# spawner1145/vae-tagger

Measured on AMD Instinct MI355X. Metric: images/sec encode+tag, 1024^2 bf16, higher is better.
Workload: dtype bf16

## Files before the change

include/vae_tagger_hip.h:

```cpp
#ifndef VAE_TAGGER_HIP_H
#define VAE_TAGGER_HIP_H

#include <stddef.h>
#include <stdint.h>

#ifdef __cplusplus
extern "C" {
#endif

typedef struct vt_context vt_context;

enum { VT_OK = 0, VT_ERR_INVALID = 1, VT_ERR_HIP = 2, VT_ERR_STATE = 3, VT_ERR_MISSING_WEIGHT = 4,
       VT_ERR_WORKSPACE = 5 };
enum { VT_F32 = 0, VT_BF16 = 1, VT_F16 = 2, VT_U8 = 3  };

const char* vt_version(void);
int vt_create(int device, vt_context** out);
void vt_destroy(vt_context* ctx);
const char* vt_last_error(const vt_context* ctx);

int vt_encoder_configure(vt_context* ctx, int in_channels, int latent_channels, const int* block_out_channels,
                         int n_blocks, int layers_per_block, int norm_num_groups, float scaling_factor,
                         int has_scaling_factor, float shift_factor, int has_shift_factor);
int vt_set_weight(vt_context* ctx, const char* name, const void* host_data, int dtype, const int64_t* shape,
// ... 60 lines not shown
                    uint64_t* row_stats_out , size_t row_stats_bytes, void* workspace, size_t workspace_bytes, void* stream);

typedef struct { const void* state; size_t state_bytes; long long capacity; long long n_seen; } vt_eval_source;
int vt_eval_export(vt_context* ctx, const void* state, size_t state_bytes, int N, int T, long long capacity, long long n_seen,
                   void* out_state, size_t out_bytes, long long out_capacity, void* stream);
int vt_eval_merge(vt_context* ctx, void* dst, size_t dst_bytes, int N, int T, long long dst_capacity, long long dst_n_seen,
                  const vt_eval_source* sources , int W, void* stream);

typedef struct { const void* state; size_t state_bytes; double alpha; double gamma; const double* class_weights ; } vt_loss_source;
size_t vt_loss_state_bytes(int N);
int vt_loss_reset(vt_context* ctx, void* state, size_t state_bytes, int N, double alpha, double gamma,
                  const double* class_weights , void* stream);
int vt_loss_update(vt_context* ctx, void* state, size_t state_bytes, int N, const float* logits ,
                   const void* labels , int labels_dtype , int B, void* stream);
int vt_loss_read(vt_context* ctx, const void* state, size_t state_bytes, int N, void* out, size_t out_bytes, void* stream);
int vt_loss_merge(vt_context* ctx, void* dst, size_t dst_bytes, int N, double alpha, double gamma,
                  const double* class_weights , const vt_loss_source* sources , int W, void* stream);

enum { VT_SAMPLE_GT = 0, VT_SAMPLE_GE = 1 };
size_t vt_sample_state_bytes(int T, long long capacity);
int vt_sample_reset(vt_context* ctx, void* state, size_t state_bytes, int T, const double* thresholds , int rule,
                    long long capacity, void* stream);
int vt_sample_update(vt_context* ctx, void* state, size_t state_bytes, int T, long long capacity, const float* probs ,
                     const void* labels , int labels_dtype , const uint32_t* true_extra ,
                     int B, int N, long long n_seen , void* stream);
int vt_sample_from_keys(vt_context* ctx, const void* eval_state, size_t eval_state_bytes, int N, int T_eval, long long capacity,
                        long long n_seen, const double* class_thresholds , int rule,
                        const uint32_t* true_extra , void* sample_state , size_t sample_state_bytes,
                        long long sample_capacity, void* stream);
size_t vt_sample_finish_bytes(int T);
int vt_sample_finish(vt_context* ctx, const void* state, size_t state_bytes, int T, long long capacity, long long n_seen, void* out,
                     size_t out_bytes, void* stream);
int vt_sample_read_rows(vt_context* ctx, const void* state, size_t state_bytes, int T, long long capacity, long long n_seen,
                        uint32_t* true_out , size_t true_bytes, uint32_t* rows_out , size_t rows_bytes,
                        void* stream);

double vt_encoder_flops(const vt_context* ctx, int H, int W);

enum { VT_HEAD_PARAM = 0, VT_HEAD_GRAD = 1, VT_HEAD_ADAM_M = 2, VT_HEAD_ADAM_V = 3, VT_HEAD_LOSS_RING = 4, VT_HEAD_NORM = 5 };
enum { VT_HEAD_LOSS_BCE = 0, VT_HEAD_LOSS_FOCAL = 1, VT_HEAD_LOSS_CLASS_BALANCED = 2 };
int vt_decoder_feature_dim(const vt_context* ctx);
int vt_decode_features(vt_context* ctx, const float* latent_nchw, int B, int h, int w, float* features_out , void* workspace,
                       size_t workspace_bytes, void* stream);
size_t vt_head_state_bytes(const vt_context* ctx);
size_t vt_head_workspace_bytes(const vt_context* ctx, int B);
int vt_head_init(vt_context* ctx, void* state, size_t state_bytes, void* stream);
int vt_head_forward(vt_context* ctx, const void* state, size_t state_bytes, const float* features, int B, float* logits_out, void* workspace,
                    size_t workspace_bytes, void* stream);
int vt_head_forward_backward(vt_context* ctx, void* state, size_t state_bytes, const float* features, const void* labels, int labels_dtype,
                             int B, int loss_kind, double focal_alpha, double focal_gamma, const float* class_weights, double loss_scale,
                             int train, const float* dropout_p , unsigned long long seed, unsigned long long step,
                             float* logits_out, unsigned char* masks_out, void* workspace, size_t workspace_bytes, void* stream);
int vt_head_clip(vt_context* ctx, void* state, size_t state_bytes, float max_norm, void* stream);
int vt_head_step(vt_context* ctx, void* state, size_t state_bytes, double lr, double beta1, double beta2, double eps, double weight_decay,
                 long long t, void* stream);
int vt_head_commit(vt_context* ctx, const void* state, size_t state_bytes, void* stream);
int vt_head_read(vt_context* ctx, const void* state, size_t state_bytes, int kind, const char* name, void* out, size_t out_bytes, void* stream);
int vt_head_write(vt_context* ctx, void* state, size_t state_bytes, int kind, const char* name, const void* src, size_t src_bytes,
                  void* stream);

enum { VT_FRONT_BN_MEAN = 6, VT_FRONT_BN_VAR = 7, VT_FRONT_BN_TRACKED = 8 };
size_t vt_front_state_bytes(const vt_context* ctx);
size_t vt_front_workspace_bytes(const vt_context* ctx, int B, int h, int w);
int vt_front_init(vt_context* ctx, void* state, size_t state_bytes, void* stream);
int vt_front_forward(vt_context* ctx, void* state, size_t state_bytes, const float* latent_nchw, int B, int h, int w, int train,
                     float attention_dropout, unsigned long long seed, unsigned long long step, float* features_out ,
                     unsigned char* mask_out, void* workspace, size_t workspace_bytes, void* stream);
int vt_front_backward(vt_context* ctx, void* state, size_t state_bytes, const float* latent_nchw, const float* d_features , int B,
                      int h, int w, float attention_dropout, unsigned long long seed, unsigned long long step, void* workspace,
                      size_t workspace_bytes, void* stream);
int vt_front_step(vt_context* ctx, void* state, size_t state_bytes, double lr, double beta1, double beta2, double eps, double weight_decay,
                  long long t, void* stream);
int vt_front_commit(vt_context* ctx, const void* state, size_t state_bytes, void* stream);
int vt_front_read(vt_context* ctx, const void* state, size_t state_bytes, int kind, const char* name, void* out, size_t out_bytes, void* stream);
int vt_front_write(vt_context* ctx, void* state, size_t state_bytes, int kind, const char* name, const void* src, size_t src_bytes,
                   void* stream);
int vt_head_forward_backward_dx(vt_context* ctx, void* state, size_t state_bytes, const float* features, const void* labels, int labels_dtype,
                                int B, int loss_kind, double focal_alpha, double focal_gamma, const float* class_weights, double loss_scale,
                                int train, const float* dropout_p , unsigned long long seed, unsigned long long step,
                                float* logits_out, unsigned char* masks_out, float* d_features , void* workspace,
                                size_t workspace_bytes, void* stream);
int vt_train_clip(vt_context* ctx, void* head_state, size_t head_state_bytes, void* front_state, size_t front_state_bytes, float max_norm,
                  void* stream);

size_t vt_cross_state_bytes(const vt_context* ctx);
size_t vt_cross_workspace_bytes(const vt_context* ctx, int B);
int vt_cross_init(vt_context* ctx, void* state, size_t state_bytes, void* stream);
int vt_cross_forward(vt_context* ctx, void* state, size_t state_bytes, const float* x_in , int B, float* features_out ,
                     void* workspace, size_t workspace_bytes, void* stream);
int vt_cross_backward(vt_context* ctx, void* state, size_t state_bytes, const float* x_in, const float* d_features , int B,
                      float* d_x_out , void* workspace, size_t workspace_bytes, void* stream);
int vt_cross_step(vt_context* ctx, void* state, size_t state_bytes, double lr, double beta1, double beta2, double eps, double weight_decay,
                  long long t, void* stream);
int vt_cross_commit(vt_context* ctx, const void* state, size_t state_bytes, void* stream);
int vt_cross_read(vt_context* ctx, const void* state, size_t state_bytes, int kind, const char* name, void* out, size_t out_bytes, void* stream);
int vt_cross_write(vt_context* ctx, void* state, size_t state_bytes, int kind, const char* name, const void* src, size_t src_bytes,
                   void* stream);
int vt_train_clip3(vt_context* ctx, void* head_state, size_t head_state_bytes, void* front_state, size_t front_state_bytes, void* cross_state,
                   size_t cross_state_bytes, float max_norm, void* stream);

size_t vt_head_grads_floats(const vt_context* ctx);
int vt_head_grads_export(vt_context* ctx, const void* state, size_t state_bytes, void* dst, size_t dst_bytes, void* stream);
int vt_head_grads_merge(vt_context* ctx, void* state, size_t state_bytes, const float* src, size_t stride_floats, int K, const double* weights,
                        void* stream);
size_t vt_front_grads_floats(const vt_context* ctx);
int vt_front_grads_export(vt_context* ctx, const void* state, size_t state_bytes, void* dst, size_t dst_bytes, void* stream);
int vt_front_grads_merge(vt_context* ctx, void* state, size_t state_bytes, const float* src, size_t stride_floats, int K, const double* weights,
                         void* stream);
size_t vt_cross_grads_floats(const vt_context* ctx);
int vt_cross_grads_export(vt_context* ctx, const void* state, size_t state_bytes, void* dst, size_t dst_bytes, void* stream);
int vt_cross_grads_merge(vt_context* ctx, void* state, size_t state_bytes, const float* src, size_t stride_floats, int K, const double* weights,
                         void* stream);

int vt_set_flag(vt_context* ctx, int flag, int value);

int vt_debug_trace(vt_context* ctx, int enable, unsigned long long* sums_out, int max_sums, int* n_out);
int vt_profile_num_configs(void);
int vt_profile_begin(vt_context* ctx);
int vt_profile_end(vt_context* ctx, int max_cfg, long long* launches, double* total_ms, double* total_flops,
                   const char** kernel_names);

int vt_image_decoder_configure(vt_context* ctx, int out_channels, int latent_channels, const int* block_out_channels, int n_blocks,
                               int layers_per_block, int groups, float scaling, int has_scaling, float shift, int has_shift);
int vt_image_decoder_finalize(vt_context* ctx);
size_t vt_decode_image_workspace_bytes(const vt_context* ctx, int B, int h, int w);
int vt_decode_image(vt_context* ctx, const float* z_nchw, int B, int h, int w, int unscale, float* image_out, size_t image_bytes,
                    void* workspace, size_t workspace_bytes, void* stream);

int vt_op_conv2d(vt_context* ctx, const void* x_bf16_nhwc, const void* w_bf16_ohwi, const float* bias,
                 const float* residual_f32, float* out_f32, void* out_bf16, int B, int Hin, int Win, int Cin,
                 int Cout, int ksize, int stride, int pad_lo, int pad_hi, void* stream);
int vt_op_norm_silu_conv3x3(vt_context* ctx, const void* x_nhwc, int x_dtype, const float* scale_shift,
                            const void* w_bf16_ohwi, const float* bias, const float* residual_f32, float* out_f32,
                            void* out_bf16, int B, int H, int W, int Cin, int Cout, void* stream);
size_t vt_op_conv2d_gn_workspace_bytes(int B, int Hout, int Wout, int Cout);
int vt_op_conv2d_gn(vt_context* ctx, const void* x_bf16_nhwc, const void* w_bf16_ohwi, const float* bias,
                    const float* residual_f32, float* out_f32, void* out_bf16, int B, int Hin, int Win, int Cin,
                    int Cout, int ksize, int stride, int pad_lo, int pad_hi, int groups, float eps, const float* gamma,
                    const float* beta, float* scale_shift_out, void* workspace, void* stream);
int vt_op_upsample2x_conv3x3(vt_context* ctx, const void* x_bf16_nhwc, const float* w_f32_oihw, const float* bias, float* out_f32,
                             int B, int h, int w, int C, void* stream);
int vt_op_upsample2x_conv3x3_gn(vt_context* ctx, const void* x_bf16_nhwc, const float* w_f32_oihw, const float* bias, float* out_f32,
                                int B, int h, int w, int C, int groups, float eps, const float* gamma, const float* beta,
                                float* scale_shift_out, void* stream);
size_t vt_op_conv3x3_fp8_workspace_bytes(int B, int H, int W, int Cin, int Cout);
int vt_op_conv3x3_fp8(vt_context* ctx, const float* x_f32_nhwc, const float* w_f32_oihw, const float* bias, const float* residual_f32,
                      float* out_f32, int B, int H, int W, int Cin, int Cout, int stride ,
                      void* workspace, void* stream);
int vt_op_gemm_nt(vt_context* ctx, const void* a_bf16, const void* b_bf16, const float* bias, float* out_f32,
                  void* out_bf16, int batch, int M, int N, int K, int lda, int ldb, int ldo, long long a_bs,
                  long long b_bs, long long o_bs, float alpha, int bias_per_row, void* stream);
int vt_op_conv_in(vt_context* ctx, const float* x_nchw, const float* w_oihw, const float* bias, float* out_f32,
                  void* out_bf16, int B, int H, int W, int Cout, void* workspace, void* stream);
size_t vt_op_groupnorm_workspace_bytes(int B, int HW, int C);
int vt_op_groupnorm(vt_context* ctx, const void* x, int x_dtype, int B, int HW, int C, int groups, float eps,
                    const float* gamma, const float* beta, int silu, void* y_bf16, void* workspace, void* stream);
int vt_op_softmax_rows(vt_context* ctx, const float* scores, void* probs_bf16, int rows, int n, int lds, int ldp,
                       void* stream);
size_t vt_op_attention_workspace_bytes(int B, int S, int C);
int vt_op_attention(vt_context* ctx, const void* x_bf16 , const float* residual_f32,
                    float* out_f32, int B, int S, int C, void* workspace, void* stream);

#ifdef __cplusplus
}
#endif
#endif
```

vae_tagger_amd/_lib.py:

```python
import ctypes
import os
import threading

_HERE = os.path.dirname(os.path.abspath(__file__))
LIB_PATH = os.environ.get("VAE_TAGGER_HIP_LIB") or os.path.join(_HERE, "csrc", "libvae_tagger_hip.so")

VT_F32, VT_BF16, VT_F16, VT_U8 = 0, 1, 2, 3
VT_STATUS_NONFINITE, VT_STATUS_FP8_SATURATED = 1, 2
ENCODE_MOMENTS, ENCODE_MODE, ENCODE_MODE_SCALED = 0, 1, 2
HEAD_PARAM, HEAD_GRAD, HEAD_ADAM_M, HEAD_ADAM_V, HEAD_LOSS_RING, HEAD_NORM = range(6)
FRONT_BN_MEAN, FRONT_BN_VAR, FRONT_BN_TRACKED = 6, 7, 8
HEAD_LOSS_KINDS = {"bce": 0, "focal": 1, "class_balanced": 2}
HEAD_RING = 256
VT_SAMPLE_GT, VT_SAMPLE_GE = 0, 1

_c = ctypes
_vp, _i, _f, _sz, _ll = _c.c_void_p, _c.c_int, _c.c_float, _c.c_size_t, _c.c_longlong


class ResizeItem(_c.Structure):
    _fields_ = [("src_hwc", _vp), ("src_h", _i), ("src_w", _i), ("crop_left", _i), ("crop_top", _i), ("crop_w", _i), ("crop_h", _i)]


class EvalSource(_c.Structure):
    _fields_ = [("state", _vp), ("state_bytes", _sz), ("capacity", _ll), ("n_seen", _ll)]


class LossSource(_c.Structure):
    _fields_ = [("state", _vp), ("state_bytes", _sz), ("alpha", _c.c_double), ("gamma", _c.c_double), ("class_weights", _vp)]


PROTOTYPES = {
    "vt_version": (_c.c_char_p, []),
    "vt_create": (_i, [_i, _c.POINTER(_vp)]),
    "vt_destroy": (None, [_vp]),
    "vt_last_error": (_c.c_char_p, [_vp]),
    "vt_encoder_configure": (_i, [_vp, _i, _i, _c.POINTER(_i), _i, _i, _i, _f, _i, _f, _i]),
    "vt_set_weight": (_i, [_vp, _c.c_char_p, _vp, _i, _c.POINTER(_c.c_int64), _i]),
    "vt_encoder_finalize": (_i, [_vp]),
    "vt_decoder_configure": (_i, [_vp, _i, _i, _i, _i, _i, _i, _i]),
    "vt_decoder_finalize": (_i, [_vp]),
    "vt_encode_workspace_bytes": (_sz, [_vp, _i, _i, _i]),
    "vt_encode": (_i, [_vp, _vp, _i, _i, _i, _i, _vp, _vp, _sz, _vp]),
    "vt_decode_workspace_bytes": (_sz, [_vp, _i, _i, _i]),
    "vt_decode_logits": (_i, [_vp, _vp, _i, _i, _i, _vp, _vp, _sz, _vp]),
    "vt_get_confidence": (_i, [_vp, _vp, _i, _i, _vp, _vp, _vp]),
    "vt_summarize_confidence": (_i, [_vp, _vp, _vp, _i, _i, _f, _i, _vp, _vp, _vp, _vp]),
    "vt_summarize_confidence_per_class": (_i, [_vp, _vp, _vp, _i, _i, _vp, _i, _vp, _vp, _vp, _vp]),
    "vt_status": (_i, [_vp, _i, _c.POINTER(_i), _vp]),
    "vt_status_async": (_i, [_vp, _i, _vp, _vp]),
    "vt_encode_tag_workspace_bytes": (_sz, [_vp, _i, _i, _i]),
    "vt_encode_tag": (_i, [_vp, _vp, _i, _i, _i, _vp, _vp, _vp, _sz, _vp]),
    "vt_preprocess_u8": (_i, [_vp, _vp, _i, _i, _i, _vp, _vp]),
    "vt_resize_workspace_bytes": (_sz, [_i, _i, _i, _i, _i]),
    "vt_resize_table": (_i, [_i, _i, _i, _c.POINTER(_i), _i]),
    "vt_resize_u8": (_i, [_vp, _vp, _i, _i, _i, _i, _i, _i, _vp, _i, _i, _i, _vp, _sz, _vp]),
    "vt_resize_batch_workspace_bytes": (_sz, [_c.POINTER(ResizeItem), _i, _i, _i, _i]),
    "vt_resize_normalize_batch": (_i, [_vp, _c.POINTER(ResizeItem), _i, _i, _i, _i, _vp, _sz, _vp, _sz, _vp, _sz, _vp]),
    "vt_eval_state_bytes": (_sz, [_i, _i, _ll]),
    "vt_eval_reset": (_i, [_vp, _vp, _sz, _i, _i, _c.POINTER(_c.c_double), _i, _ll, _vp]),
    "vt_eval_update": (_i, [_vp, _vp, _sz, _i, _i, _i, _ll, _vp, _vp, _i, _i, _ll, _vp]),
    "vt_eval_grow": (_i, [_vp, _vp, _sz, _ll, _vp, _sz, _ll, _i, _i, _ll, _vp]),
    "vt_eval_ap_workspace_bytes": (_sz, [_i, _ll]),
    "vt_eval_average_precision": (_i, [_vp, _vp, _sz, _i, _i, _ll, _ll, _vp, _sz, _vp, _vp, _sz, _vp]),
    "vt_eval_read_counts": (_i, [_vp, _vp, _sz, _i, _i, _ll, _vp, _sz, _vp, _sz, _vp, _sz, _vp]),
    "vt_eval_recount_workspace_bytes": (_sz, [_i, _ll]),
    "vt_eval_recount": (_i, [_vp, _vp, _sz, _i, _i, _ll, _ll, _vp, _vp, _sz, _vp, _sz, _vp, _sz, _vp]),
    "vt_eval_export": (_i, [_vp, _vp, _sz, _i, _i, _ll, _ll, _vp, _sz, _ll, _vp]),
    "vt_eval_merge": (_i, [_vp, _vp, _sz, _i, _i, _ll, _ll, _c.POINTER(EvalSource), _i, _vp]),
    "vt_loss_state_bytes": (_sz, [_i]),
    "vt_loss_reset": (_i, [_vp, _vp, _sz, _i, _c.c_double, _c.c_double, _vp, _vp]),
    "vt_loss_update": (_i, [_vp, _vp, _sz, _i, _vp, _vp, _i, _i, _vp]),
    "vt_loss_read": (_i, [_vp, _vp, _sz, _i, _vp, _sz, _vp]),
    "vt_loss_merge": (_i, [_vp, _vp, _sz, _i, _c.c_double, _c.c_double, _vp, _c.POINTER(LossSource), _i, _vp]),
    "vt_sample_state_bytes": (_sz, [_i, _ll]),
    "vt_sample_reset": (_i, [_vp, _vp, _sz, _i, _c.POINTER(_c.c_double), _i, _ll, _vp]),
    "vt_sample_update": (_i, [_vp, _vp, _sz, _i, _ll, _vp, _vp, _i, _vp, _i, _i, _ll, _vp]),
    "vt_sample_from_keys": (_i, [_vp, _vp, _sz, _i, _i, _ll, _ll, _vp, _i, _vp, _vp, _sz, _ll, _vp]),
    "vt_sample_finish_bytes": (_sz, [_i]),
    "vt_sample_finish": (_i, [_vp, _vp, _sz, _i, _ll, _ll, _vp, _sz, _vp]),
    "vt_sample_read_rows": (_i, [_vp, _vp, _sz, _i, _ll, _ll, _vp, _sz, _vp, _sz, _vp]),
    "vt_decoder_feature_dim": (_i, [_vp]),
    "vt_decode_features": (_i, [_vp, _vp, _i, _i, _i, _vp, _vp, _sz, _vp]),
    "vt_head_state_bytes": (_sz, [_vp]),
    "vt_head_workspace_bytes": (_sz, [_vp, _i]),
    "vt_head_init": (_i, [_vp, _vp, _sz, _vp]),
    "vt_head_forward": (_i, [_vp, _vp, _sz, _vp, _i, _vp, _vp, _sz, _vp]),
    "vt_head_forward_backward": (_i, [_vp, _vp, _sz, _vp, _vp, _i, _i, _i, _c.c_double, _c.c_double, _vp, _c.c_double, _i,
                                      _c.POINTER(_f), _c.c_ulonglong, _c.c_ulonglong, _vp, _vp, _vp, _sz, _vp]),
    "vt_head_clip": (_i, [_vp, _vp, _sz, _f, _vp]),
    "vt_head_step": (_i, [_vp, _vp, _sz, _c.c_double, _c.c_double, _c.c_double, _c.c_double, _c.c_double, _ll, _vp]),
    "vt_head_commit": (_i, [_vp, _vp, _sz, _vp]),
    "vt_head_read": (_i, [_vp, _vp, _sz, _i, _c.c_char_p, _vp, _sz, _vp]),
    "vt_head_write": (_i, [_vp, _vp, _sz, _i, _c.c_char_p, _vp, _sz, _vp]),
    "vt_front_state_bytes": (_sz, [_vp]),
    "vt_front_workspace_bytes": (_sz, [_vp, _i, _i, _i]),
    "vt_front_init": (_i, [_vp, _vp, _sz, _vp]),
    "vt_front_forward": (_i, [_vp, _vp, _sz, _vp, _i, _i, _i, _i, _f, _c.c_ulonglong, _c.c_ulonglong, _vp, _vp, _vp, _sz, _vp]),
    "vt_front_backward": (_i, [_vp, _vp, _sz, _vp, _vp, _i, _i, _i, _f, _c.c_ulonglong, _c.c_ulonglong, _vp, _sz, _vp]),
    "vt_front_step": (_i, [_vp, _vp, _sz, _c.c_double, _c.c_double, _c.c_double, _c.c_double, _c.c_double, _ll, _vp]),
    "vt_front_commit": (_i, [_vp, _vp, _sz, _vp]),
    "vt_front_read": (_i, [_vp, _vp, _sz, _i, _c.c_char_p, _vp, _sz, _vp]),
    "vt_front_write": (_i, [_vp, _vp, _sz, _i, _c.c_char_p, _vp, _sz, _vp]),
    "vt_head_forward_backward_dx": (_i, [_vp, _vp, _sz, _vp, _vp, _i, _i, _i, _c.c_double, _c.c_double, _vp, _c.c_double, _i,
                                         _c.POINTER(_f), _c.c_ulonglong, _c.c_ulonglong, _vp, _vp, _vp, _vp, _sz, _vp]),
    "vt_train_clip": (_i, [_vp, _vp, _sz, _vp, _sz, _f, _vp]),
    "vt_cross_state_bytes": (_sz, [_vp]),
    "vt_cross_workspace_bytes": (_sz, [_vp, _i]),
    "vt_cross_init": (_i, [_vp, _vp, _sz, _vp]),
    "vt_cross_forward": (_i, [_vp, _vp, _sz, _vp, _i, _vp, _vp, _sz, _vp]),
    "vt_cross_backward": (_i, [_vp, _vp, _sz, _vp, _vp, _i, _vp, _vp, _sz, _vp]),
    "vt_cross_step": (_i, [_vp, _vp, _sz, _c.c_double, _c.c_double, _c.c_double, _c.c_double, _c.c_double, _ll, _vp]),
    "vt_cross_commit": (_i, [_vp, _vp, _sz, _vp]),
    "vt_cross_read": (_i, [_vp, _vp, _sz, _i, _c.c_char_p, _vp, _sz, _vp]),
    "vt_cross_write": (_i, [_vp, _vp, _sz, _i, _c.c_char_p, _vp, _sz, _vp]),
    "vt_train_clip3": (_i, [_vp, _vp, _sz, _vp, _sz, _vp, _sz, _f, _vp]),
    "vt_head_grads_floats": (_sz, [_vp]),
    "vt_head_grads_export": (_i, [_vp, _vp, _sz, _vp, _sz, _vp]),
    "vt_head_grads_merge": (_i, [_vp, _vp, _sz, _vp, _sz, _i, _c.POINTER(_c.c_double), _vp]),
    "vt_front_grads_floats": (_sz, [_vp]),
    "vt_front_grads_export": (_i, [_vp, _vp, _sz, _vp, _sz, _vp]),
    "vt_front_grads_merge": (_i, [_vp, _vp, _sz, _vp, _sz, _i, _c.POINTER(_c.c_double), _vp]),
    "vt_cross_grads_floats": (_sz, [_vp]),
    "vt_cross_grads_export": (_i, [_vp, _vp, _sz, _vp, _sz, _vp]),
    "vt_cross_grads_merge": (_i, [_vp, _vp, _sz, _vp, _sz, _i, _c.POINTER(_c.c_double), _vp]),
    "vt_image_decoder_configure": (_i, [_vp, _i, _i, _c.POINTER(_i), _i, _i, _i, _f, _i, _f, _i]),
    "vt_image_decoder_finalize": (_i, [_vp]),
    "vt_decode_image_workspace_bytes": (_sz, [_vp, _i, _i, _i]),
    "vt_decode_image": (_i, [_vp, _vp, _i, _i, _i, _i, _vp, _sz, _vp, _sz, _vp]),
    "vt_encoder_flops":(_c.c_double, [_vp, _i, _i]),
    "vt_set_flag": (_i, [_vp, _i, _i]),
    "vt_debug_trace": (_i, [_vp, _i, _c.POINTER(_c.c_ulonglong), _i, _c.POINTER(_i)]),
    "vt_profile_num_configs": (_i, []),
    "vt_profile_begin": (_i, [_vp]),
    "vt_profile_end": (_i, [_vp, _i, _c.POINTER(_ll), _c.POINTER(_c.c_double), _c.POINTER(_c.c_double), _c.POINTER(_c.c_char_p)]),
    "vt_op_conv2d": (_i, [_vp, _vp, _vp, _vp, _vp, _vp, _vp, _i, _i, _i, _i, _i, _i, _i, _i, _i, _vp]),
    "vt_op_norm_silu_conv3x3": (_i, [_vp, _vp, _i, _vp, _vp, _vp, _vp, _vp, _vp, _i, _i, _i, _i, _i, _vp]),
    "vt_op_conv2d_gn_workspace_bytes": (_sz, [_i, _i, _i, _i]),
    "vt_op_conv2d_gn": (_i, [_vp, _vp, _vp, _vp, _vp, _vp, _vp, _i, _i, _i, _i, _i, _i, _i, _i, _i, _i, _f, _vp, _vp, _vp, _vp, _vp]),
    "vt_op_upsample2x_conv3x3": (_i, [_vp, _vp, _vp, _vp, _vp, _i, _i, _i, _i, _vp]),
    "vt_op_upsample2x_conv3x3_gn": (_i, [_vp, _vp, _vp, _vp, _vp, _i, _i, _i, _i, _i, _f, _vp, _vp, _vp, _vp]),
    "vt_op_conv3x3_fp8_workspace_bytes": (_sz, [_i, _i, _i, _i, _i]),
    "vt_op_conv3x3_fp8": (_i, [_vp, _vp, _vp, _vp, _vp, _vp, _i, _i, _i, _i, _i, _i, _vp, _vp]),
    "vt_op_gemm_nt": (_i, [_vp, _vp, _vp, _vp, _vp, _vp, _i, _i, _i, _i, _i, _i, _i, _ll, _ll, _ll, _f, _i, _vp]),
    "vt_op_conv_in": (_i, [_vp, _vp, _vp, _vp, _vp, _vp, _i, _i, _i, _i, _vp, _vp]),
    "vt_op_groupnorm_workspace_bytes": (_sz, [_i, _i, _i]),
    "vt_op_groupnorm": (_i, [_vp, _vp, _i, _i, _i, _i, _i, _f, _vp, _vp, _i, _vp, _vp, _vp]),
    "vt_op_softmax_rows": (_i, [_vp, _vp, _vp, _i, _i, _i, _i, _vp]),
    "vt_op_attention_workspace_bytes": (_sz, [_i, _i, _i]),
    "vt_op_attention": (_i, [_vp, _vp, _vp, _vp, _i, _i, _i, _vp, _vp]),
}

_lib = None
_lock = threading.Lock()


class VTError(RuntimeError):
    pass


def load():
    global _lib
    with _lock:
        if _lib is not None:
            return _lib
        if not os.path.exists(LIB_PATH):
            raise VTError(
                f"{LIB_PATH} not found: the HIP extension is not built. Run "
                f"`python -c 'import __graft_entry__ as g; g.build()'` or `make -C {os.path.dirname(LIB_PATH)}`. "
                "There is no CPU fallback.")
        lib = ctypes.CDLL(LIB_PATH)
        for name, (res, args) in PROTOTYPES.items():
            fn = getattr(lib, name)
            fn.restype = res
            fn.argtypes = args
        _lib = lib
        return lib


class Context:

    def __init__(self, device_index=0):
        self.lib = load()
        h = _vp()
        rc = self.lib.vt_create(int(device_index), ctypes.byref(h))
        if rc != 0 or not h.value:
            raise VTError(f"vt_create(device={device_index}) failed with code {rc} (no usable HIP device?)")
        self.handle = h
        self.device_index = int(device_index)

    def close(self):
        if getattr(self, "handle", None) is not None and self.handle.value:
            self.lib.vt_destroy(self.handle)
            self.handle = _vp()

    def __del__(self):
        try:
            self.close()
        except Exception:
            pass

    def check(self, rc, what):
        if rc != 0:
            msg = self.lib.vt_last_error(self.handle)
            raise VTError(f"{what} failed (code {rc}): {msg.decode('utf-8', 'replace') if msg else ''}")

    def call(self, name, *args):
        self.check(getattr(self.lib, name)(self.handle, *args), name)

    def status(self, clear=True, stream=None):
        v = _i(0)
        if stream is None:
            import torch
            stream = _vp(torch.cuda.current_stream(self.device_index).cuda_stream)
        self.call("vt_status", int(clear), ctypes.byref(v), stream)
        return v.value

    def set_weight(self, name, tensor):
        import torch
        t = tensor.detach().to("cpu")
        if t.dtype == torch.bfloat16:
            dt, t = VT_BF16, t.contiguous().view(torch.int16)
        elif t.dtype == torch.float16:
            dt, t = VT_F16, t.contiguous().view(torch.int16)
        else:
            dt, t = VT_F32, t.to(torch.float32).contiguous()
        shape = (ctypes.c_int64 * max(1, tensor.dim()))(*tensor.shape)
        self.call("vt_set_weight", name.encode("utf-8"), _vp(t.data_ptr()), dt, shape, tensor.dim())
```

vae_tagger_amd/csrc/capi.hip:

```cpp
#include <math.h>
#include <string.h>

#include "vt_context.h"
#include "vt_eval.h"

using namespace vt;

namespace {
__global__ void dbg_checksum_kernel(const unsigned int* __restrict__ p, long long n, unsigned long long* __restrict__ out) {
    unsigned long long acc = 0;
    for (long long i = (long long)blockIdx.x * blockDim.x + threadIdx.x; i < n; i += (long long)gridDim.x * blockDim.x) acc += (unsigned long long)p[i] * (unsigned long long)(i % 1021 + 1);
    atomicAdd(out, acc);
}
constexpr int DBG_SLOTS = 256;
}

void vt::dbg_sum(vt_context* c, const void* p, size_t bytes, hipStream_t s) {
    if (!c->dbg_on || !c->dbg || c->dbg_n >= DBG_SLOTS) return;
    hipLaunchKernelGGL(dbg_checksum_kernel, dim3(64), dim3(256), 0, s, (const unsigned int*)p, (long long)(bytes / 4), c->dbg + c->dbg_n);
    ++c->dbg_n;
}

extern "C" {

// ... 294 lines not shown
    return VT_OK;
}

size_t vt_eval_ap_workspace_bytes(int N, long long n_seen) {
    if (N <= 0 || n_seen <= 0 || (unsigned long long)N * (unsigned long long)n_seen > (unsigned long long)VT_EVAL_MICRO_LIMIT) return 0;
    return vt_eval_align((size_t)N * (size_t)n_seen * 8);
}

int vt_eval_average_precision(vt_context* c, void* state, size_t state_bytes, int N, int T, long long capacity, long long n_seen,
                              double* ap_out, size_t ap_bytes, double* micro_ap_out, void* workspace, size_t workspace_bytes, void* stream) {
    if (!c) return VT_ERR_INVALID;
    DeviceGuard guard(c);
    if (int r = eval_check_state(c, "vt_eval_average_precision", state, state_bytes, N, T, capacity)) return r;
    if (capacity <= 0) return c->fail(VT_ERR_STATE, "vt_eval_average_precision: the state keeps no keys (capacity 0)");
    if (n_seen <= 0 || n_seen > capacity) return c->fail(VT_ERR_INVALID, "vt_eval_average_precision: n_seen = %lld outside [1, capacity = %lld]", n_seen, capacity);
    if (!ap_out || ((uintptr_t)ap_out & 7)) return c->fail(VT_ERR_INVALID, "vt_eval_average_precision: ap_out is null or misaligned");
    if (ap_bytes < (size_t)N * 8) return c->fail(VT_ERR_WORKSPACE, "vt_eval_average_precision: ap_out holds %zu bytes, %zu needed", ap_bytes, (size_t)N * 8);
    if (micro_ap_out) {
        const size_t need = vt_eval_ap_workspace_bytes(N, n_seen);
        if (need == 0) return c->fail(VT_ERR_INVALID, "vt_eval_average_precision: micro AP runs on the device while n_seen * N < 2^31");
        if ((uintptr_t)micro_ap_out & 7) return c->fail(VT_ERR_INVALID, "vt_eval_average_precision: micro_ap_out is misaligned");
        if (!workspace || misaligned(workspace)) return c->fail(VT_ERR_INVALID, "vt_eval_average_precision: workspace is null or not 256-B aligned");
        if (workspace_bytes < need) return c->fail(VT_ERR_WORKSPACE, "vt_eval_average_precision: workspace holds %zu bytes, %zu needed", workspace_bytes, need);
    }
    HIPCK(c, vt_eval_launch_ap(state, vt_eval_layout(N, T, capacity), N, capacity, n_seen, ap_out, micro_ap_out, (unsigned long long*)workspace,
                               (hipStream_t)stream), "eval_average_precision");
    return VT_OK;
}

int vt_eval_read_counts(vt_context* c, const void* state, size_t state_bytes, int N, int T, long long capacity, uint32_t* counts_out,
                        size_t counts_bytes, uint32_t* support_out, size_t support_bytes, uint64_t* row_stats_out, size_t row_stats_bytes,
                        void* stream) {
    if (!c) return VT_ERR_INVALID;
    DeviceGuard guard(c);
    if (int r = eval_check_state(c, "vt_eval_read_counts", state, state_bytes, N, T, capacity)) return r;
    if (!counts_out || !support_out || !row_stats_out) return c->fail(VT_ERR_INVALID, "vt_eval_read_counts: null output");
    const size_t nc = (size_t)N * T * 2 * 4, ns = (size_t)N * 4, nr = 3 * 8;
    if (counts_bytes < nc || support_bytes < ns || row_stats_bytes < nr)
        return c->fail(VT_ERR_WORKSPACE, "vt_eval_read_counts: outputs hold %zu / %zu / %zu bytes, %zu / %zu / %zu needed", counts_bytes, support_bytes,
                       row_stats_bytes, nc, ns, nr);
    const EvalLayout l = vt_eval_layout(N, T, capacity);
    hipStream_t s = (hipStream_t)stream;
    const char* st = (const char*)state;
    HIPCK(c, hipMemcpyAsync(counts_out, st + l.counts, nc, hipMemcpyDefault, s), "eval_read counts");
    HIPCK(c, hipMemcpyAsync(support_out, st + l.support, ns, hipMemcpyDefault, s), "eval_read support");
    HIPCK(c, hipMemcpyAsync(row_stats_out, st + l.row_stats, nr, hipMemcpyDefault, s), "eval_read row_stats");
    return VT_OK;
}

size_t vt_eval_recount_workspace_bytes(int N, long long n_seen) {
    if (N <= 0 || n_seen < 0 || n_seen > VT_EVAL_MAX_N_SEEN) return 0;
    return vt_eval_recount_ws_bytes(N, n_seen);
}

int vt_eval_recount(vt_context* c, const void* state, size_t state_bytes, int N, int T, long long capacity, long long n_seen,
                    const double* class_thresholds, uint32_t* counts_out, size_t counts_bytes, uint64_t* row_stats_out,
                    size_t row_stats_bytes, void* workspace, size_t workspace_bytes, void* stream) {
    if (!c) return VT_ERR_INVALID;
    DeviceGuard guard(c);
    if (int r = eval_check_state(c, "vt_eval_recount", state, state_bytes, N, T, capacity)) return r;
    if (n_seen < 0 || n_seen > VT_EVAL_MAX_N_SEEN || n_seen > capacity)
        return c->fail(VT_ERR_INVALID, "vt_eval_recount: n_seen = %lld outside [0, capacity = %lld]%s", n_seen, capacity,
                       capacity == 0 ? " (the state keeps no keys)" : "");
    if (!class_thresholds || ((uintptr_t)class_thresholds & 7)) return c->fail(VT_ERR_INVALID, "vt_eval_recount: class_thresholds is null or misaligned");
    if (!counts_out || ((uintptr_t)counts_out & 3) || !row_stats_out || ((uintptr_t)row_stats_out & 7))
        return c->fail(VT_ERR_INVALID, "vt_eval_recount: an output is null or misaligned");
    if (!workspace || misaligned(workspace)) return c->fail(VT_ERR_INVALID, "vt_eval_recount: workspace is null or not 256-B aligned");
    const size_t nc = (size_t)N * 2 * 4, nr = 3 * 8, need = vt_eval_recount_ws_bytes(N, n_seen);
    if (counts_bytes < nc || row_stats_bytes < nr)
        return c->fail(VT_ERR_WORKSPACE, "vt_eval_recount: outputs hold %zu / %zu bytes, %zu / %zu needed", counts_bytes, row_stats_bytes, nc, nr);
    if (workspace_bytes < need) return c->fail(VT_ERR_WORKSPACE, "vt_eval_recount: workspace holds %zu bytes, %zu needed", workspace_bytes, need);
    HIPCK(c, vt_eval_launch_recount(state, vt_eval_layout(N, T, capacity), N, capacity, n_seen, class_thresholds, counts_out,
                                    (unsigned long long*)row_stats_out, workspace, (hipStream_t)stream), "eval_recount");
    return VT_OK;
}

namespace {
bool blocks_overlap(const void* a, size_t na, const void* b, size_t nb) {
    const uintptr_t pa = (uintptr_t)a, pb = (uintptr_t)b;
    return pa < pb + nb && pb < pa + na;
}
}

int vt_eval_export(vt_context* c, const void* state, size_t state_bytes, int N, int T, long long capacity, long long n_seen, void* out_state,
                   size_t out_bytes, long long out_capacity, void* stream) {
    if (!c) return VT_ERR_INVALID;
    DeviceGuard guard(c);
    if (int r = eval_check_state(c, "vt_eval_export (state)", state, state_bytes, N, T, capacity)) return r;
    if (int r = eval_check_state(c, "vt_eval_export (out)", out_state, out_bytes, N, T, out_capacity)) return r;
    if (n_seen < 0 || n_seen > VT_EVAL_MAX_N_SEEN || (capacity > 0 && n_seen > capacity))
        return c->fail(VT_ERR_INVALID, "vt_eval_export: n_seen = %lld outside [0, capacity = %lld]", n_seen, capacity);
    if (out_capacity != 0 && out_capacity < n_seen)
        return c->fail(VT_ERR_INVALID, "vt_eval_export: out_capacity = %lld is neither 0 nor >= n_seen = %lld", out_capacity, n_seen);
    if (out_capacity > 0 && capacity == 0 && n_seen > 0)
        return c->fail(VT_ERR_INVALID, "vt_eval_export: the state keeps no keys (capacity 0) but out_capacity = %lld", out_capacity);
    const EvalLayout l = vt_eval_layout(N, T, capacity), lo = vt_eval_layout(N, T, out_capacity);
    if (blocks_overlap(state, l.total, out_state, lo.total)) return c->fail(VT_ERR_INVALID, "vt_eval_export: out_state overlaps the state");
    HIPCK(c, vt_eval_launch_export(state, l, out_state, lo, N, capacity, n_seen, out_capacity, c->eval_merge_vec, (hipStream_t)stream), "eval_export");
    return VT_OK;
}

int vt_eval_merge(vt_context* c, void* dst, size_t dst_bytes, int N, int T, long long dst_capacity, long long dst_n_seen,
                  const vt_eval_source* sources, int W, void* stream) {
    if (!c) return VT_ERR_INVALID;
    DeviceGuard guard(c);
    if (int r = eval_check_state(c, "vt_eval_merge (dst)", dst, dst_bytes, N, T, dst_capacity)) return r;
    if (!sources || W < 1 || W > VT_EVAL_MAX_MERGE) return c->fail(VT_ERR_INVALID, "vt_eval_merge: null sources or W = %d outside [1, %d]", W, VT_EVAL_MAX_MERGE);
    if (dst_n_seen < 0 || dst_n_seen > VT_EVAL_MAX_N_SEEN || (dst_capacity > 0 && dst_n_seen > dst_capacity))
        return c->fail(VT_ERR_INVALID, "vt_eval_merge: dst_n_seen = %lld outside [0, capacity = %lld]", dst_n_seen, dst_capacity);
    const EvalLayout l = vt_eval_layout(N, T, dst_capacity);
    EvalMergeArg a;
    a.W = W;
    long long total = dst_n_seen;
    for (int w = 0; w < W; ++w) {
        const vt_eval_source& s = sources[w];
        if (int r = eval_check_state(c, "vt_eval_merge (source)", s.state, s.state_bytes, N, T, s.capacity)) return r;
        if (s.n_seen < 0 || s.n_seen > VT_EVAL_MAX_N_SEEN || (s.capacity > 0 && s.n_seen > s.capacity))
            return c->fail(VT_ERR_INVALID, "vt_eval_merge: source %d has n_seen = %lld outside [0, capacity = %lld]", w, s.n_seen, s.capacity);
        if (blocks_overlap(dst, l.total, s.state, vt_eval_layout(N, T, s.capacity).total))
            return c->fail(VT_ERR_INVALID, "vt_eval_merge: source %d is dst or overlaps it", w);
        if (dst_capacity > 0 && s.capacity == 0 && s.n_seen > 0)
            return c->fail(VT_ERR_INVALID, "vt_eval_merge: source %d keeps no keys (capacity 0) for its %lld samples, dst does", w, s.n_seen);
        a.src[w] = EvalMergeSrc{(const char*)s.state, s.capacity, s.n_seen, s.n_seen, total};
        total += s.n_seen;
        if (total > VT_EVAL_MAX_N_SEEN) return c->fail(VT_ERR_INVALID, "vt_eval_merge: %lld samples in all, 2^31 or more", total);
    }
    if (dst_capacity > 0 && total > dst_capacity)
        return c->fail(VT_ERR_INVALID, "vt_eval_merge: dst_n_seen + the sources' samples = %lld exceeds the capacity %lld", total, dst_capacity);
    HIPCK(c, vt_eval_launch_merge(dst, l, N, dst_capacity, a, c->eval_merge_vec, (hipStream_t)stream), "eval_merge");
    return VT_OK;
}

int vt_set_flag(vt_context* c, int flag, int value) {
    if (!c) return VT_ERR_INVALID;
    if (flag == 0) { c->use_halo_conv = value != 0; return VT_OK; }
    if (flag == 1) { c->fuse_gn_stats = value != 0; return VT_OK; }
    if (flag == 2) { c->fuse_gn_apply = value != 0; return VT_OK; }
    if (flag == 3) { c->halo_occ2 = value < 0 ? 0 : (value > 4 ? 4 : value); return VT_OK; }
    if (flag == 4) { c->res_fp16 = value != 0; return VT_OK; }
    if (flag == 5) { c->conv_in_mfma = value != 0; return VT_OK; }
    if (flag == 6) { c->gemm_short = value != 0; return VT_OK; }
    if (flag == 8) { c->fuse_shortcut = value != 0; return VT_OK; }
    if (flag == 9) { c->attn_qk_kernel = value != 0; return VT_OK; }
    if (flag == 10) { c->pv_stream = value != 0; return VT_OK; }
    if (flag == 11) { c->fp8 = value != 0; return VT_OK; }
    if (flag == 16) { if ((value & 3) == 3 || value < 0 || value > 7) return c->fail(VT_ERR_INVALID, "vt_set_flag(16): tile shape 0..2 (+4: every layer)"); c->fp8_tile = value; return VT_OK; }
    if (flag == 12) { c->attn_pv_kernel = value != 0; return VT_OK; }
    if (flag == 17) { c->attn_proj_kernel = value != 0; return VT_OK; }
    if (flag == 18) { c->f16_ops = value != 0; return VT_OK; }
    if (flag == 19) { c->s2_planar = value != 0; return VT_OK; }
    if (flag == 21) { c->eval_merge_vec = value != 0; return VT_OK; }
    if (flag == 20) { c->conv_out_halo = value != 0; return VT_OK; }
    if (flag == 22) { c->up2_literal = value != 0; return VT_OK; }
    if (flag == 13) { c->s2_halo = value != 0; return VT_OK; }
    if (flag == 14) { c->attn_fp8 = value != 0; return VT_OK; }
    if (flag == 15) { c->proj_fp8 = value != 0; return VT_OK; }
    if (flag == 7) {
        if (value < 0 || value > 2) return c->fail(VT_ERR_INVALID, "vt_set_flag(7): value %d not in 0..2", value);
        c->attn_mode = value;
        return VT_OK;
    }
    return c->fail(VT_ERR_INVALID, "vt_set_flag: unknown flag %d", flag);
}

int vt_profile_num_configs(void) { return VT_NUM_PROF_SLOTS; }

int vt_preprocess_u8(vt_context* c, const uint8_t* in_hwc, int B, int H, int W, float* out_nchw, void* stream) {
    if (!c) return VT_ERR_INVALID;
    DeviceGuard guard(c);
    HIPCK(c, vt_launch_preprocess_u8(in_hwc, out_nchw, B, H, W, (hipStream_t)stream), "vt_preprocess_u8");
    return VT_OK;
}

namespace {
constexpr int RS_BITS = 32 - 8 - 2;
double rs_filter(int kind, double x) {
    if (kind == 0) {
        if (x < 0.0) x = -x;
        return x < 1.0 ? 1.0 - x : 0.0;
    }
    if (-3.0 <= x && x < 3.0) {
        auto sinc = [](double v) { if (v == 0.0) return 1.0; v *= M_PI; return sin(v) / v; };
        return sinc(x) * sinc(x / 3);
    }
    return 0.0;
}
}
extern "C++" {
namespace vt {
int rs_ksize(int in_size, int out_size, int kind) {
    double fs = (double)in_size / out_size;
    if (fs < 1.0) fs = 1.0;
    return (int)ceil((kind == 0 ? 1.0 : 3.0) * fs) * 2 + 1;
}
void rs_table(int in_size, int out_size, int kind, int* tab) {
    const double scale = (double)in_size / out_size;
    double filterscale = scale < 1.0 ? 1.0 : scale;
    const double support = (kind == 0 ? 1.0 : 3.0) * filterscale, ss = 1.0 / filterscale;
    const int ksize = (int)ceil(support) * 2 + 1;
    std::vector<double> w(ksize);
    for (int xx = 0; xx < out_size; ++xx) {
        const double center = (xx + 0.5) * scale;
        int xmin = (int)(center - support + 0.5);
        if (xmin < 0) xmin = 0;
        int xmax = (int)(center + support + 0.5);
        if (xmax > in_size) xmax = in_size;
        xmax -= xmin;
        double ww = 0.0;
        for (int x = 0; x < xmax; ++x) { w[x] = rs_filter(kind, (x + xmin - center + 0.5) * ss); ww += w[x]; }
        int* t = tab + (size_t)xx * (2 + ksize);
        t[0] = xmin; t[1] = xmax;
        for (int x = 0; x < ksize; ++x) {
            double v = x < xmax ? w[x] : 0.0;
            if (x < xmax && ww != 0.0) v /= ww;
            t[2 + x] = v < 0 ? (int)(-0.5 + v * (1 << RS_BITS)) : (int)(0.5 + v * (1 << RS_BITS));
        }
    }
}
}
}
namespace {
struct RsPlan { int kh, kv; size_t tab_h, tab_v, tmp, total; };
RsPlan rs_plan(int crop_h, int crop_w, int dst_h, int dst_w, int kind) {
    RsPlan p{};
    const bool nh = dst_w != crop_w, nv = dst_h != crop_h;
    p.kh = nh ? rs_ksize(crop_w, dst_w, kind) : 0;
    p.kv = nv ? rs_ksize(crop_h, dst_h, kind) : 0;
    p.tab_h = nh ? (size_t)dst_w * (2 + p.kh) : 0;
    p.tab_v = nv ? (size_t)dst_h * (2 + p.kv) : 0;
    p.tmp = (nh && nv) ? (size_t)crop_h * dst_w * 3 : ((nv && !nh) ? (size_t)crop_h * crop_w * 3 : 0);
    p.total = align_up((p.tab_h + p.tab_v) * 4) + align_up(p.tmp);
    return p;
}
}

int vt_resize_table(int in_size, int out_size, int filter, int* table_out, int table_ints) {
    if (in_size <= 0 || out_size <= 0 || (filter != 0 && filter != 1)) return -1;
    const int ks = rs_ksize(in_size, out_size, filter);
    if (!table_out) return ks;
    if ((long long)table_ints < (long long)out_size * (2 + ks)) return -1;
    rs_table(in_size, out_size, filter, table_out);
    return ks;
}

size_t vt_resize_workspace_bytes(int crop_h, int crop_w, int dst_h, int dst_w, int filter) {
    if (crop_h <= 0 || crop_w <= 0 || dst_h <= 0 || dst_w <= 0 || (filter != 0 && filter != 1)) return 0;
    return rs_plan(crop_h, crop_w, dst_h, dst_w, filter).total + 256;
}

int vt_resize_u8(vt_context* c, const uint8_t* src_hwc, int src_h, int src_w, int crop_left, int crop_top, int crop_w, int crop_h,
                 uint8_t* dst_hwc, int dst_h, int dst_w, int filter, void* workspace, size_t workspace_bytes, void* stream) {
    if (!c) return VT_ERR_INVALID;
    if (!src_hwc || !dst_hwc || (filter != 0 && filter != 1) || crop_w <= 0 || crop_h <= 0 || dst_w <= 0 || dst_h <= 0 ||
        crop_left < 0 || crop_top < 0 || crop_left + crop_w > src_w || crop_top + crop_h > src_h)
        return c->fail(VT_ERR_INVALID, "vt_resize_u8: bad argument");
    DeviceGuard guard(c);
    const RsPlan p = rs_plan(crop_h, crop_w, dst_h, dst_w, filter);
    char* ws = (char*)(((uintptr_t)workspace + 255) & ~(uintptr_t)255);
    if (p.total && (!workspace || workspace_bytes < p.total + (size_t)(ws - (char*)workspace)))
        return c->fail(VT_ERR_WORKSPACE, "vt_resize_u8: workspace %zu < required %zu", workspace_bytes, p.total + 256);
    hipStream_t s = (hipStream_t)stream;
    int* tab = (int*)ws;
    const size_t ints = p.tab_h + p.tab_v;
    if (ints) {
        if (!c->rs_event) HIPCK(c, hipEventCreateWithFlags(&c->rs_event, hipEventDisableTiming), "hipEventCreate");
        else HIPCK(c, hipEventSynchronize(c->rs_event), "hipEventSynchronize");
        if (c->rs_host_ints < ints) {
            if (c->rs_host) (void)hipHostFree(c->rs_host);
            c->rs_host = nullptr; c->rs_host_ints = 0;
            HIPCK(c, hipHostMalloc((void**)&c->rs_host, ints * 4, hipHostMallocDefault), "hipHostMalloc");
            c->rs_host_ints = ints;
        }
        if (p.tab_h) rs_table(crop_w, dst_w, filter, c->rs_host);
        if (p.tab_v) rs_table(crop_h, dst_h, filter, c->rs_host + p.tab_h);
        HIPCK(c, hipMemcpyAsync(tab, c->rs_host, ints * 4, hipMemcpyHostToDevice, s), "hipMemcpyAsync(tables)");
        HIPCK(c, hipEventRecord(c->rs_event, s), "hipEventRecord");
    }
    unsigned char* tmp = p.tmp ? (unsigned char*)(ws + align_up(ints * 4)) : nullptr;
    HIPCK(c, vt_launch_resize_u8(src_hwc, src_h, src_w, crop_left, crop_top, crop_w, crop_h, dst_hwc, dst_h, dst_w,
                                 p.tab_h ? tab : nullptr, p.kh, p.tab_v ? tab + p.tab_h : nullptr, p.kv, tmp, s), "vt_resize_u8");
    return VT_OK;
}

int vt_debug_trace(vt_context* c, int enable, unsigned long long* sums_out, int max_sums, int* n_out) {
    if (!c) return VT_ERR_INVALID;
    DeviceGuard guard(c);
    if (enable) {
        if (!c->dbg) HIPCK(c, hipMalloc((void**)&c->dbg, DBG_SLOTS * 8), "hipMalloc(debug trace)");
        HIPCK(c, hipMemset(c->dbg, 0, DBG_SLOTS * 8), "hipMemset(debug trace)");
        c->dbg_n = 0; c->dbg_on = true;
        return VT_OK;
    }
    c->dbg_on = false;
    HIPCK(c, hipDeviceSynchronize(), "hipDeviceSynchronize");
    const int n = c->dbg_n < max_sums ? c->dbg_n : max_sums;
    if (sums_out && n > 0) HIPCK(c, hipMemcpy(sums_out, c->dbg, (size_t)n * 8, hipMemcpyDeviceToHost), "hipMemcpy(debug trace)");
    if (n_out) *n_out = n;
    return VT_OK;
}

int vt_profile_begin(vt_context* c) {
    if (!c) return VT_ERR_INVALID;
    c->prof.clear(); c->events_used = 0; c->profiling = true;
    return VT_OK;
}

// ... 19 lines not shown
```

vae_tagger_amd/csrc/encoder.hip:

```cpp
#include <algorithm>

#include "vt_context.h"

namespace vt {

int launch_gemm(vt_context* c, const ConvGemmArgs& a_in, hipStream_t s, const char* what) {
    ConvGemmArgs a = a_in;
    a.short_tiles = c->gemm_short;
    if (!c->profiling || a.gate) { HIPCK(c, vt_launch_conv_gemm(a, s), what); return VT_OK; }
    const int n = a.Cout < a.Wrows ? a.Cout : a.Wrows;
    return profiled(c, s, vt_conv_gemm_config(a), 2.0 * a.batch * (double)a.Hout * a.Wout * n * (double)(a.ksize * a.ksize) * a.Cin, what,
                    [&] { return vt_launch_conv_gemm(a, s); });
}

int launch_halo(vt_context* c, const Conv3x3Args& a_in, hipStream_t s, const char* what) {
    Conv3x3Args a = a_in;
    a.occ2 = c->halo_occ2;
    if (!c->profiling) { HIPCK(c, vt_launch_conv3x3_halo(a, s), what); return VT_OK; }
    return profiled(c, s, vt_conv3x3_halo_config(a), 2.0 * a.batch * (double)a.H * a.W * a.Cout * (9.0 * a.Cin + (a.scX ? a.scCin : 0)), what,
                    [&] { return vt_launch_conv3x3_halo(a, s); });
}

int launch_halo_fp8(vt_context* c, const Conv3x3Fp8Args& a, hipStream_t s, const char* what) {
    return profiled(c, s, a.Cin <= 128 ? VT_PROF_HALO_FP8_C128 : VT_PROF_HALO_FP8,
                    2.0 * a.batch * (double)a.H * a.W * a.Cout * (9.0 * a.Cin + (a.scX ? a.scCin : 0)), what, [&] { return vt_launch_conv3x3_halo_fp8(a, s); });
}


int run_gn(vt_context* c, const void* x, int xdt , int B, int HW, const NormW& n, int groups, int silu, bf16_t* y,
           GnState& g, hipStream_t s, bool out_fp8, bool out_f16 ) {
    const float o8 = out_fp8 ? FP8_ACT_SCALE : 0.f;
    int parts = g.parts;
    if (parts == 0) HIPCK(c, vt_launch_gn_stats(x, xdt, B, HW, n.c, groups, g.partial, &parts, s), "gn_stats");
    g.parts = 0;
    HIPCK(c, vt_launch_gn_finalize(g.partial, parts, B, n.c, groups, 1e-6f, n.g, n.b, g.ss, s, c->status), "gn_finalize");
    dbg_sum(c, g.partial, (size_t)B * parts * groups * 3 * 4, s);
    dbg_sum(c, g.ss, (size_t)B * n.c * 2 * 4, s);
    const double bytes = (double)B * HW * n.c * ((xdt == 1 ? 4.0 : 2.0) + (out_fp8 ? 1.0 : 2.0));
    return profiled(c, s, VT_PROF_GN_APPLY, bytes, "gn_apply", [&] { return vt_launch_gn_apply(x, xdt, g.ss, y, B, HW, n.c, silu, s, o8, c->status, out_f16); });
}

bool conv_f16(const vt_context* c, const ConvW& w, int stride, bool has_sc) {
    if (!c->f16_ops || c->fp8 || w.k != 3) return false;
    if (stride == 2) return c->s2_halo && w.wp2_16 != nullptr;
    return c->use_halo_conv && w.wp && w.wp16 && !c->fuse_gn_apply && vt_conv3x3_halo_f16_supported(w.cout, c->halo_occ2, has_sc ? 1 : 0);
}

namespace {

struct ConvCall {
    const ConvW& w; const bf16_t* x; int B, Hin, Win, stride, pad, Hout, Wout; bf16_t* o16; hipStream_t s; const ConvOpts& o;
    const float* res32; const f16_t* res16; float* o32; f16_t* oh16;
    int cpg; bool fuse;
    double flops() const { return 2.0 * B * (double)Hout * Wout * w.cout * 9.0 * w.cin; }
};

int conv_s2_fp8(vt_context* c, const ConvCall& k) {
    const ConvW& w = k.w;
    Conv3x3S2Fp8Args h{};
    h.X = (const unsigned char*)k.x; h.Wp = w.wp8s2; h.mult = w.mult8g; h.bias = w.b; h.res = k.res32;
    h.out_f32 = k.o32; h.out_f16 = k.oh16; h.out_bf16 = k.o16; h.zeros = c->zeros;
    h.batch = k.B; h.H = k.Hin; h.W = k.Win; h.Cin = w.cin; h.Cout = w.cout; h.x_planar = k.o.planar;
    if (k.fuse) { h.gn_partial = k.o.gn->partial; h.gn_cpg = k.cpg; k.o.gn->parts = vt_conv3x3_s2_fp8_tiles(k.Hout, k.Wout); }
    return profiled(c, k.s, VT_PROF_S2_HALO_FP8, k.flops(), "conv3x3_s2_fp8", [&] { return vt_launch_conv3x3_s2_fp8(h, k.s); });
}

int conv_gemm_fp8(vt_context* c, const ConvCall& k) {
    const ConvW& w = k.w;
    ConvGemmArgs a{};
    a.X = k.x; a.W = (const bf16_t*)w.w8g; a.f8 = 1; a.col_scale = w.mult8g;
    a.bias = w.b; a.res = k.res32; a.res_f16 = k.res16; a.out_f32 = k.o32; a.out_f16 = k.oh16; a.out_bf16 = k.o16; a.zeros = c->zeros;
    a.Hin = k.Hin; a.Win = k.Win; a.Hout = k.Hout; a.Wout = k.Wout; a.Cin = w.cin; a.Cout = w.cout; a.Wrows = w.cout;
    a.ksize = 3; a.stride = 2; a.pad = k.pad;
    a.ldx = w.cin; a.ldw = 9 * w.cin; a.ldo = w.cout; a.ldr = w.cout;
    a.x_bs = (long long)k.Hin * k.Win * w.cin; a.w_bs = 0; a.o_bs = (long long)k.Hout * k.Wout * w.cout; a.r_bs = a.o_bs;
    a.batch = k.B; a.alpha = 1.f; a.bias_mode = 1; a.out_mode = 0; a.short_tiles = c->gemm_short;
    if (k.fuse && w.cout > 32 && (w.cout % (w.cout <= 128 ? 128 : 256)) == 0) {
        a.gn_partial = k.o.gn->partial; a.gn_cpg = k.cpg; k.o.gn->parts = vt_conv_gemm_ptiles_of(a);
    }
    return profiled(c, k.s, VT_PROF_GEMM_FP8, k.flops(), "conv_gemm_fp8", [&] { return vt_launch_conv_gemm(a, k.s); });
}

int conv_halo_fp8(vt_context* c, const ConvCall& k) {
    const ConvW& w = k.w; const ScFuse* sc = k.o.sc;
    Conv3x3Fp8Args h{};
    h.X = (const unsigned char*)k.x; h.Wp = w.wp8; h.mult = w.mult8; h.bias = w.b; h.res = k.res32; h.res_f16 = k.res16;
    h.out_f32 = k.o32; h.out_f16 = k.oh16; h.out_bf16 = k.o.o16_e4m3 ? nullptr : k.o16; h.zeros = c->zeros;
    if (k.o.o16_e4m3) { h.out_e4m3 = (unsigned char*)k.o16; h.out_e4m3_scale = FP8_RES_SCALE; h.status = c->status; h.out8_planar = k.o.planar; }
    else if (k.o.planar) return c->fail(VT_ERR_STATE, "internal: planar bf16 copy requested from the fp8 conv");
    h.batch = k.B; h.H = k.Hin; h.W = k.Win; h.Cin = w.cin; h.Cout = w.cout;
    if (sc) { h.scX = sc->x; h.scW = sc->wp8; h.scCin = sc->cin; h.bias = sc->bias; }
    h.shape = (w.cin <= 128 || (c->fp8_tile & 4)) ? (c->fp8_tile & 3) : 0;
    if (k.fuse) { h.gn_partial = k.o.gn->partial; h.gn_cpg = k.cpg; k.o.gn->parts = vt_conv3x3_halo_fp8_tiles_shape(k.Hin, k.Win, h.shape); }
    return launch_halo_fp8(c, h, k.s, "conv3x3_halo_fp8");
}

int conv_s2(vt_context* c, const ConvCall& k) {
    const ConvW& w = k.w;
    Conv3x3S2Args h{};
    h.X = k.x; h.Wp = k.o.x_f16 ? w.wp2_16 : w.wp2; h.bias = w.b; h.res = k.res32; h.out_f32 = k.o32; h.out_f16 = k.oh16; h.out_bf16 = k.o16; h.zeros = c->zeros;
    h.batch = k.B; h.H = k.Hin; h.W = k.Win; h.Cin = w.cin; h.Cout = w.cout; h.f16 = k.o.x_f16; h.out16_f16 = k.o.o16_f16; h.x_planar = k.o.planar;
    if (k.fuse) { h.gn_partial = k.o.gn->partial; h.gn_cpg = k.cpg; k.o.gn->parts = vt_conv3x3_s2_tiles(k.Hout, k.Wout); }
    return profiled(c, k.s, VT_PROF_S2_HALO, k.flops(), "conv3x3_s2", [&] { return vt_launch_conv3x3_s2(h, k.s); });
}

int conv_halo(vt_context* c, const ConvCall& k) {
    const ConvW& w = k.w; const ConvOpts& o = k.o;
    Conv3x3Args h{};
    h.X = o.xnorm_f32 ? nullptr : k.x; h.Xf32 = o.xnorm_f32; h.scale_shift = o.ss;
    h.Wp = o.x_f16 ? w.wp16 : w.wp; h.bias = w.b; h.res = k.res32; h.res_f16 = k.res16; h.out_f32 = k.o32; h.out_f16 = k.oh16; h.out_bf16 = k.o16; h.zeros = c->zeros;
    h.batch = k.B; h.H = k.Hin; h.W = k.Win; h.Cin = w.cin; h.Cout = w.cout; h.f16 = o.x_f16; h.out16_f16 = o.o16_f16; h.out16_planar = o.planar;
    if (o.sc) { h.scX = o.sc->x; h.scW = o.x_f16 ? o.sc->wp16 : o.sc->wp; h.scCin = o.sc->cin; h.bias = o.sc->bias; }
    if (k.fuse) { h.gn_partial = o.gn->partial; h.gn_cpg = k.cpg; o.gn->parts = vt_conv3x3_halo_tiles(k.Hin, k.Win, w.cout, o.ss ? (o.xnorm_f32 ? 1 : 2) : 0, c->halo_occ2, o.sc != nullptr); }
    VTCK(launch_halo(c, h, k.s, "conv3x3_halo"));
    if (c->dbg_on) {
        const size_t ne = (size_t)k.B * k.Hin * k.Win * w.cout;
        if (k.oh16) dbg_sum(c, k.oh16, ne * 2, k.s); else if (k.o32) dbg_sum(c, k.o32, ne * 4, k.s); else if (k.o16) dbg_sum(c, k.o16, ne * 2, k.s);
    }
    return VT_OK;
}

int conv_gemm(vt_context* c, const ConvCall& k) {
    const ConvW& w = k.w;
    ConvGemmArgs a{};
    a.X = k.x; a.W = w.w; a.bias = w.b; a.res = k.res32; a.res_f16 = k.res16; a.out_f32 = k.o32; a.out_f16 = k.oh16; a.out_bf16 = k.o16; a.zeros = c->zeros;
    a.Hin = k.Hin; a.Win = k.Win; a.Hout = k.Hout; a.Wout = k.Wout; a.Cin = w.cin; a.Cout = w.cout; a.Wrows = w.cout;
    a.ksize = w.k; a.stride = k.stride; a.pad = k.pad;
    a.ldx = w.cin; a.ldw = w.k * w.k * w.cin; a.ldo = w.cout; a.ldr = w.cout;
    a.x_bs = (long long)k.Hin * k.Win * w.cin; a.w_bs = 0; a.o_bs = (long long)k.Hout * k.Wout * w.cout; a.r_bs = a.o_bs;
    a.batch = k.B; a.alpha = 1.f; a.bias_mode = 1; a.out_mode = 0;
    if (k.fuse && w.cout > 32 && (w.cout % (w.cout <= 128 ? 128 : 256)) == 0) {
        a.short_tiles = c->gemm_short;
        a.gn_partial = k.o.gn->partial; a.gn_cpg = k.cpg; k.o.gn->parts = vt_conv_gemm_ptiles_of(a);
    }
    return launch_gemm(c, a, k.s, "conv_gemm");
}

}

int run_conv(vt_context* c, const ConvW& w, const bf16_t* x, int B, int Hin, int Win, int stride, int pad, int Hout, int Wout,
             const void* res, void* oh, bf16_t* o16, hipStream_t s, const ConvOpts& o) {
    const int cpg = w.cout / o.groups;
    const ConvCall k{w, x, B, Hin, Win, stride, pad, Hout, Wout, o16, s, o,
                     o.rdt == 1 ? (const float*)res : nullptr, o.rdt == 2 ? (const f16_t*)res : nullptr, o.rdt == 1 ? (float*)oh : nullptr, o.rdt == 2 ? (f16_t*)oh : nullptr,
                     cpg, o.gn && c->fuse_gn_stats && (cpg == 4 || cpg == 8 || cpg == 16)};
    if (o.gn) o.gn->parts = 0;
    if (o.x_fp8 && stride == 2) {
        if (!w.w8g || w.k != 3 || o.ss || o.sc || o.o16_e4m3) return c->fail(VT_ERR_STATE, "internal: fp8 operands requested for a conv the fp8 GEMM cannot run");
        if (c->s2_halo && w.wp8s2 && pad == 0 && Hout == Hin / 2 && Wout == Win / 2 && !k.res16) return conv_s2_fp8(c, k);
        return conv_gemm_fp8(c, k);
    }
    if (o.x_fp8) {
        if (!w.wp8 || w.k != 3 || stride != 1 || pad != 1 || o.ss || (o.sc && !o.sc->wp8)) return c->fail(VT_ERR_STATE, "internal: fp8 operands requested for a conv the fp8 kernel cannot run");
        return conv_halo_fp8(c, k);
    }
    if (c->s2_halo && w.wp2 && w.k == 3 && stride == 2 && pad == 0 && Hout == Hin / 2 && Wout == Win / 2 && !k.res16 && !o.ss && !o.sc && !o.xnorm_f32) return conv_s2(c, k);
    if (c->use_halo_conv && w.wp && w.k == 3 && stride == 1 && pad == 1 && Hout == Hin && Wout == Win) return conv_halo(c, k);
    if (o.ss || o.sc) return c->fail(VT_ERR_STATE, "internal: fused norm / shortcut requested for a conv the halo kernel cannot run");
    if (o.x_f16 || o.o16_f16 || o.planar) return c->fail(VT_ERR_STATE, "internal: fp16 operands / a planar layout requested for a conv on the generic GEMM");
    return conv_gemm(c, k);
}

static bool norm_conv_fusable(const vt_context* c, const ConvW& w, int cin) {
    return c->fuse_gn_apply && c->use_halo_conv && w.wp && w.k == 3 && cin * 8 <= 8192;
}

int run_norm_conv(vt_context* c, const NormW& n, const ConvW& w, const void* x, int xdt, int B, int H, int W,
                  int groups, bf16_t* act, const void* res, void* oh, bf16_t* o16, GnState& gn, bool want_stats,
                  hipStream_t s, int rdt, const NormConvOpts& nc) {
    const ScFuse* sc = nc.sc;
    const bool f8 = c->fp8 && w.wp8 && w.k == 3 && (!sc || sc->wp8);
    if (nc.o16_e4m3 && !f8) return c->fail(VT_ERR_STATE, "internal: e4m3 output requested from a bf16 conv");
    ConvOpts o;
    o.gn = want_stats ? &gn : nullptr; o.groups = groups; o.rdt = rdt;
    if (f8 || xdt == 2 || !norm_conv_fusable(c, w, n.c)) {
        const bool h16 = !f8 && conv_f16(c, w, 1, sc != nullptr) && (!sc || sc->x_f16);
        if (sc && sc->x_f16 && !h16) return c->fail(VT_ERR_STATE, "internal: fp16 shortcut input for a bf16 conv");
        VTCK(run_gn(c, x, xdt, B, H * W, n, groups, 1, act, gn, s, f8, h16));
        o.sc = sc; o.x_fp8 = f8; o.o16_e4m3 = nc.o16_e4m3; o.x_f16 = h16; o.o16_f16 = nc.o16_f16; o.planar = nc.o16_planar;
        return run_conv(c, w, act, B, H, W, 1, 1, H, W, res, oh, o16, s, o);
    }
    if (nc.o16_planar) return c->fail(VT_ERR_STATE, "internal: planar copy requested from the fused-norm staging path");
    if (sc) return c->fail(VT_ERR_STATE, "internal: fused shortcut with the fused-norm staging");
    int parts = gn.parts;
    if (parts == 0) HIPCK(c, vt_launch_gn_stats(x, xdt, B, H * W, n.c, groups, gn.partial, &parts, s), "gn_stats");
    gn.parts = 0;
    HIPCK(c, vt_launch_gn_finalize(gn.partial, parts, B, n.c, groups, 1e-6f, n.g, n.b, gn.ss, s, c->status), "gn_finalize");
    o.xnorm_f32 = xdt == 1 ? (const float*)x : nullptr; o.ss = gn.ss;
    return run_conv(c, w, xdt == 0 ? (const bf16_t*)x : nullptr, B, H, W, 1, 1, H, W, res, oh, o16, s, o);
}

namespace {

struct EncPlan {
    size_t max_elems = 0;
    int max_c = 0;
    int max_chunks = 0;
    int hl = 0, wl = 0;
    size_t total = 0;
};
constexpr size_t SLACK = 4096;

EncPlan plan_encoder(const EncoderW& e, int B, int H, int W) {
    EncPlan p;
    int h = H, w = W;
    auto note = [&](int hh, int ww, int ch) {
        p.max_elems = std::max(p.max_elems, (size_t)hh * ww * ch);
        p.max_c = std::max(p.max_c, ch);
        p.max_chunks = std::max({p.max_chunks, vt_gn_max_chunks(hh * ww, ch), vt_conv_gemm_ptiles(hh * ww, ch), vt_conv3x3_halo_tiles_max(hh, ww),
                                 vt_conv_in_parts(hh, ww), vt_conv_in_mfma_parts(hh, ww), vt_conv3x3_halo_fp8_tiles(hh, ww),
                                 vt_conv3x3_s2_tiles(hh, ww), vt_conv3x3_s2_fp8_tiles(hh, ww)});
    };
    note(h, w, e.block_out[0]);
    for (size_t i = 0; i < e.block_out.size(); ++i) {
        note(h, w, e.block_out[i]);
        if (i + 1 < e.block_out.size()) { h /= 2; w /= 2; note(h, w, e.block_out[i]); }
    }
    p.hl = h; p.wl = w;
    const int S = h * w, C = e.block_out.back();
    p.max_chunks = std::max(p.max_chunks, vt_attn_linear_parts(S));
    p.total = 3 * align_up(p.max_elems * B * 4 + SLACK) + 3 * align_up(p.max_elems * B * 2 + SLACK) +
              align_up((size_t)B * p.max_chunks * e.groups * 3 * 4) + align_up((size_t)B * p.max_c * 2 * 4) +
              attn_scratch_bytes(B, S, C) + ALIGN;
    return p;
}

struct BlockOut {
    bool only16 = false;
    bool e4m3 = false;
    bool f16 = false, planar = false;
};

struct EncRun {
    vt_context* c; const EncoderW& e; int B; hipStream_t s;
    int rdt;
    void* f32[3]; bf16_t* b16[3];
    GnState gn; AttnScratch as;
    int cur = 0;
    bf16_t *act, *tmid, *hb;
    int h, w;
    const bf16_t* h16 = nullptr;
    bool h16_is_f16 = false;

    EncRun(vt_context* c_, const EncPlan& p, int B_, int H, int W, void* ws, hipStream_t s_)
        : c(c_), e(c_->enc), B(B_), s(s_), rdt(c_->res_fp16 ? 2 : 1), h(H), w(W) {
        char* q = (char*)ws;
        for (int i = 0; i < 3; ++i) { f32[i] = (void*)q; q += align_up(p.max_elems * B * 4 + SLACK); }
        for (int i = 0; i < 3; ++i) { b16[i] = (bf16_t*)q; q += align_up(p.max_elems * B * 2 + SLACK); }
        gn.partial = (float*)q; q += align_up((size_t)B * p.max_chunks * e.groups * 3 * 4);
        gn.ss = (float*)q; q += align_up((size_t)B * p.max_c * 2 * 4);
        as = carve_attn(q, B, p.hl * p.wl, e.block_out.back());
        act = b16[0]; tmid = b16[1]; hb = b16[2];
    }

    int conv_in(const float* x) {
        const int cpg0 = e.block_out[0] / e.groups;
        const bool fuse0 = c->fuse_gn_stats && (cpg0 % 4) == 0;
        int parts = 0;
        float* o32 = rdt == 1 ? (float*)f32[cur] : nullptr;
        f16_t* oh = rdt == 2 ? (f16_t*)f32[cur] : nullptr;
        if (c->conv_in_mfma && e.conv_in_wpk) {
            HIPCK(c, vt_launch_conv_in_mfma(x, e.conv_in_wpk, e.conv_in_b, o32, nullptr, oh, fuse0 ? gn.partial : nullptr, &parts,
                                            B, h, w, s), "conv_in_mfma");
        } else {
            HIPCK(c, vt_launch_conv_in(x, e.conv_in_w, e.conv_in_b, o32, nullptr, oh, fuse0 ? gn.partial : nullptr, cpg0, &parts,
                                       B, h, w, e.block_out[0], s), "conv_in");
        }
        gn.parts = fuse0 ? parts : 0;
        return VT_OK;
    }

    bool fuse_sc(const ResnetW& rw) const {
        return c->fuse_shortcut && rw.sc_wp && c->use_halo_conv && rw.c2.wp && !c->fuse_gn_apply && (!(c->fp8 && rw.c2.wp8) || rw.sc_wp8);
    }

    int resnet(const ResnetW& rw, const bf16_t* h16_for_shortcut, const BlockOut& out = BlockOut()) {
        const int nxt = (cur + 1) % 3, scb = (cur + 2) % 3;
        const void* res = f32[cur];
        const ScFuse scf{h16_for_shortcut, rw.sc_wp, rw.b_c2sc, rw.cin, rw.sc_wp8, rw.sc_wp16, h16_is_f16};
        NormConvOpts c2;
        if (rw.has_sc) {
            if (fuse_sc(rw)) {
                c2.sc = &scf; res = nullptr;
            } else {
                ConvOpts o; o.rdt = rdt;
                VTCK(run_conv(c, rw.sc, h16_for_shortcut, B, h, w, 1, 0, h, w, nullptr, f32[scb], nullptr, s, o));
                res = f32[scb];
            }
        }
        const bool c1h = rdt == 2;
        const int c1dt = c1h ? 2 : 0;
        VTCK(run_norm_conv(c, rw.n1, rw.c1, f32[cur], rdt, B, h, w, e.groups, act, nullptr, c1h ? (void*)tmid : nullptr,
                           c1h ? nullptr : tmid, gn, true, s, rdt));
        if (out.only16) {
            c2.o16_e4m3 = out.e4m3; c2.o16_f16 = out.f16; c2.o16_planar = out.planar;
            return run_norm_conv(c, rw.n2, rw.c2, tmid, c1dt, B, h, w, e.groups, act, res, nullptr, hb, gn, false, s, rdt, c2);
        }
        VTCK(run_norm_conv(c, rw.n2, rw.c2, tmid, c1dt, B, h, w, e.groups, act, res, f32[nxt], nullptr, gn, true, s, rdt, c2));
        cur = nxt;
        return VT_OK;
    }

    int stage(size_t i) {
        const StageW& st = e.stages[i];
        BlockOut hbo;
        for (size_t j = 0; j < st.res.size(); ++j) {
            const ResnetW& rw = st.res[j];
            const bool last = j + 1 == st.res.size();
            if (rw.has_sc && !h16) return c->fail(VT_ERR_STATE, "internal: shortcut conv without a bf16 input");
            BlockOut out;
            out.only16 = last && st.has_down;
            out.e4m3 = out.only16 && c->fp8 && st.down.w8g && rw.c2.wp8 && !rw.has_sc;
            out.f16 = out.only16 && !out.e4m3 && conv_f16(c, st.down, 2, false);
            out.planar = out.only16 && c->s2_planar && c->s2_halo && !c->fuse_gn_apply &&
                         (out.e4m3 ? st.down.wp8s2 != nullptr : (st.down.wp2 != nullptr && c->use_halo_conv && rw.c2.wp && !(c->fp8 && rw.c2.wp8)));
            VTCK(resnet(rw, h16, out));
            if (last) hbo = out;
            h16 = out.only16 ? hb : nullptr; h16_is_f16 = false;
        }
        if (!st.has_down) return VT_OK;
        const int ho = h / 2, wo = w / 2;
        const int nxt = (cur + 1) % 3;
        const ResnetW* next = (i + 1 < e.stages.size() && e.stages[i + 1].res[0].has_sc) ? &e.stages[i + 1].res[0] : nullptr;
        bf16_t* copy = !next ? nullptr : (fuse_sc(*next) ? (bf16_t*)f32[(nxt + 2) % 3] : tmid);
        const bool copy16 = copy && fuse_sc(*next) && conv_f16(c, next->c2, 1, true) && c->s2_halo && st.down.wp2 && !hbo.e4m3;
        ConvOpts o;
        o.gn = &gn; o.groups = e.groups; o.rdt = rdt; o.x_fp8 = hbo.e4m3; o.x_f16 = hbo.f16; o.o16_f16 = copy16; o.planar = hbo.planar;
        VTCK(run_conv(c, st.down, hb, B, h, w, 2, 0, ho, wo, nullptr, f32[nxt], copy, s, o));
        h16 = copy; h16_is_f16 = copy16;
        cur = nxt; h = ho; w = wo;
        return VT_OK;
    }

    int mid_attention() {
        const int S = h * w, nxt = (cur + 1) % 3;
        const bool tok8 = attn_proj_is_fp8(c, e.attn, S, e.attn.c);
        VTCK(run_gn(c, f32[cur], rdt, B, S, e.attn.gn, e.groups, 0, act, gn, s, tok8));
        VTCK(run_attention(c, e.attn, act, f32[cur], f32[nxt], B, S, as, s, &gn, e.groups, rdt, tok8));
        cur = nxt;
        return VT_OK;
    }

    int conv_out(int mode, float* latent) {
        const ConvW& cw = e.conv_out;
        const bool out16 = cw.cout <= 32 && cw.w16 && c->f16_ops && !c->fp8;
        VTCK(run_gn(c, f32[cur], rdt, B, h * w, e.norm_out, e.groups, 1, act, gn, s, false, out16));
        const int keep = mode == 0 ? 2 * e.latent : e.latent;
        const float post_scale = (mode == 2 && e.has_scaling) ? e.scaling : 1.f, post_shift = (mode == 2 && e.has_shift) ? e.shift : 0.f;
        if (c->conv_out_halo && cw.wpo && cw.k == 3 && keep <= cw.cout) {
            ConvOutArgs o{};
            o.X = act; o.Wp = out16 ? cw.wpo16 : cw.wpo; o.f16 = out16; o.bias = cw.b; o.out = latent; o.zeros = c->zeros;
            o.batch = B; o.H = h; o.W = w; o.Cin = cw.cin; o.Cout = cw.cout; o.keep = keep;
            o.post_scale = post_scale; o.post_shift = post_shift;
            return profiled(c, s, VT_PROF_CONV_OUT, 2.0 * B * (double)h * w * cw.cout * 9.0 * cw.cin, "conv_out_halo", [&] { return vt_launch_conv_out_halo(o, s); });
        }
        ConvGemmArgs a{};
        a.X = act; a.W = out16 ? cw.w16 : cw.w; a.f16 = out16; a.bias = cw.b; a.out_f32 = latent; a.zeros = c->zeros;
        a.Hin = a.Hout = h; a.Win = a.Wout = w; a.Cin = cw.cin; a.Cout = cw.cout; a.Wrows = cw.cout;
        a.ksize = 3; a.stride = 1; a.pad = 1; a.ldx = cw.cin; a.ldw = 9 * cw.cin; a.ldo = cw.cout;
        a.cout_keep = keep;
        a.x_bs = (long long)h * w * cw.cin; a.o_bs = (long long)a.cout_keep * h * w; a.batch = B; a.alpha = 1.f;
        a.bias_mode = 1; a.out_mode = 1;
        a.post_scale = post_scale; a.post_shift = post_shift;
        return launch_gemm(c, a, s, "conv_out");
    }
};

}
}

using namespace vt;

extern "C" {

int vt_encoder_configure(vt_context* c, int in_ch, int latent, const int* block_out, int n_blocks, int layers,
                         int groups, float scaling, int has_scaling, float shift, int has_shift) {
    if (!c) return VT_ERR_INVALID;
    if (in_ch != 3) return c->fail(VT_ERR_INVALID, "in_channels must be 3 (got %d)", in_ch);
    if (!block_out || n_blocks < 1 || n_blocks > 8 || layers < 1 || layers > 8 || latent < 1 || groups < 1)
        return c->fail(VT_ERR_INVALID, "bad encoder configuration");
    EncoderW& e = c->enc;
    { DeviceGuard guard(c); c->free_allocs(c->enc_allocs); }
    e = EncoderW();
    e.in_ch = in_ch; e.latent = latent; e.layers = layers; e.groups = groups;
    e.block_out.assign(block_out, block_out + n_blocks);
    for (int ch : e.block_out) {
        if (ch % groups || ch % 64 || ch > 2048) return c->fail(VT_ERR_INVALID, "block_out_channels entries must be multiples of 64 and of norm_num_groups (got %d)", ch);
        const int cpg = ch / groups;
        if (cpg < 2 || (cpg & (cpg - 1)) || (256 % (ch / 8))) return c->fail(VT_ERR_INVALID, "unsupported channels/groups combination %d/%d", ch, groups);
    }
    if (2 * latent > 32 || (2 * latent) % 4) return c->fail(VT_ERR_INVALID, "latent_channels must be <= 16 and even");
    e.scaling = scaling; e.has_scaling = has_scaling != 0; e.shift = shift; e.has_shift = has_shift != 0;
    e.configured = true;
    return VT_OK;
}

size_t vt_encode_workspace_bytes(const vt_context* c, int B, int H, int W) {
    if (!c || !c->enc.configured || B <= 0 || H < 8 || W < 8) return 0;
    return plan_encoder(c->enc, B, H, W).total;
}

double vt_encoder_flops(const vt_context* c, int H, int W) {
    if (!c || !c->enc.configured) return 0.0;
    const EncoderW& e = c->enc;
    double f = 2.0 * H * W * 27 * e.block_out[0];
    int h = H, w = W, ci = e.block_out[0];
    for (size_t i = 0; i < e.block_out.size(); ++i) {
        const int co = e.block_out[i];
        for (int j = 0; j < e.layers; ++j) {
            f += 2.0 * h * w * 9 * ci * co + 2.0 * h * w * 9 * co * co;
            if (ci != co) f += 2.0 * h * w * ci * co;
            ci = co;
        }
        if (i + 1 < e.block_out.size()) { h /= 2; w /= 2; f += 2.0 * h * w * 9 * co * co; }
    }
    const double s = (double)h * w, C = ci;
    f += 4 * (2.0 * s * 9 * C * C) + 4 * (2.0 * s * C * C) + 2 * (2.0 * s * s * C) + 2.0 * s * 9 * C * 2 * e.latent;
    return f;
}

int vt_encode(vt_context* c, const float* x, int B, int H, int W, int mode, float* latent, void* ws, size_t ws_bytes,
              void* stream) {
    if (!c) return VT_ERR_INVALID;
    DeviceGuard guard(c);
    const EncoderW& e = c->enc;
    if (!e.finalized) return c->fail(VT_ERR_STATE, "encoder weights not finalized");
    if (!x || !latent || !ws || B <= 0) return c->fail(VT_ERR_INVALID, "vt_encode: null buffer or B <= 0");
    if (mode < 0 || mode > 2) return c->fail(VT_ERR_INVALID, "vt_encode: mode must be 0 (moments), 1 (mode) or 2 (mode*scale+shift)");
    const int nd = (int)e.block_out.size() - 1;
    if ((H >> nd) < 1 || (W >> nd) < 1) return c->fail(VT_ERR_INVALID, "vt_encode: image %dx%d too small", H, W);
    const EncPlan p = plan_encoder(e, B, H, W);
    if (ws_bytes < p.total) return c->fail(VT_ERR_WORKSPACE, "vt_encode: workspace %zu < required %zu", ws_bytes, p.total);
    if (((uintptr_t)ws) % ALIGN) return c->fail(VT_ERR_INVALID, "vt_encode: workspace must be 256-B aligned");
    EncRun run(c, p, B, H, W, ws, (hipStream_t)stream);
    VTCK(run.conv_in(x));
    for (size_t i = 0; i < e.stages.size(); ++i) VTCK(run.stage(i));
    VTCK(run.resnet(e.mid0, nullptr));
    VTCK(run.mid_attention());
    VTCK(run.resnet(e.mid1, nullptr));
    return run.conv_out(mode, latent);
}

size_t vt_encode_tag_workspace_bytes(const vt_context* c, int B, int H, int W) {
    if (!c || !c->enc.configured || !c->dec_configured || B <= 0 || H < 8 || W < 8) return 0;
    const EncPlan p = plan_encoder(c->enc, B, H, W);
    const size_t lat_bytes = align_up((size_t)B * c->enc.latent * p.hl * p.wl * 4);
// ... 21 lines not shown
```

vae_tagger_amd/csrc/misc_kernels.hip:

```cpp
#include <type_traits>

#include "vt_common.h"
#include "vt_kernels.h"

namespace {

constexpr int CI_PIX = 64, CI_ROWS = 16;
__global__ __launch_bounds__(256) VT_NO_PACKED_F32 void conv_in_kernel(const float* __restrict__ x, const float* __restrict__ wp,
                                                      const float* __restrict__ bias, float* __restrict__ o32,
                                                      bf16_t* __restrict__ o16, f16_t* __restrict__ oh,
                                                      float* __restrict__ gn_partial,
                                                      int gn_cpg, int H, int W, int Cout) {
    extern __shared__ __attribute__((aligned(16))) float sm[];
    constexpr int RW = CI_PIX + 2, RH = CI_ROWS + 2;
    float* sw = sm;
    float* sin = sm + 27 * Cout;
    float* red = sin + 3 * RH * RW;
    const int tid = threadIdx.x;
    const int b = blockIdx.z, y0 = blockIdx.y * CI_ROWS, x0 = blockIdx.x * CI_PIX;
    for (int i = tid; i < 27 * Cout; i += 256) sw[i] = wp[i];
    for (int i = tid; i < 3 * RH * RW; i += 256) {
        const int c = i / (RH * RW), r = (i / RW) % RH, xx = i % RW;
        const int iy = y0 - 1 + r, ix = x0 - 1 + xx;
        float v = 0.f;
        if (iy >= 0 && iy < H && ix >= 0 && ix < W) v = x[(((long long)b * 3 + c) * H + iy) * W + ix];
        sin[i] = v;
    }
    __syncthreads();
    const int cgi = tid & 15, ps = tid >> 4;
    for (int cg = cgi; cg * 8 < Cout; cg += 16) {
        const f32x4 b0 = *(const f32x4*)(bias + cg * 8), b1 = *(const f32x4*)(bias + cg * 8 + 4);
        float s0 = 0.f, ss0 = 0.f, s1 = 0.f, ss1 = 0.f;
        int cnt = 0;
        for (int row = 0; row < CI_ROWS; ++row) {
            const int y = y0 + row;
            if (y >= H) break;
            float acc[4][8];
#pragma unroll
            for (int p = 0; p < 4; ++p) {
                acc[p][0] = b0[0]; acc[p][1] = b0[1]; acc[p][2] = b0[2]; acc[p][3] = b0[3];
                acc[p][4] = b1[0]; acc[p][5] = b1[1]; acc[p][6] = b1[2]; acc[p][7] = b1[3];
            }
#pragma unroll
            for (int c = 0; c < 3; ++c)
#pragma unroll
                for (int ky = 0; ky < 3; ++ky) {
                    float in6[6];
#pragma unroll
                    for (int i = 0; i < 6; ++i) in6[i] = sin[(c * RH + row + ky) * RW + ps * 4 + i];
#pragma unroll
                    for (int kx = 0; kx < 3; ++kx) {
                        const float* wr = sw + (c * 9 + ky * 3 + kx) * Cout + cg * 8;
                        const f32x4 w0 = *(const f32x4*)wr, w1 = *(const f32x4*)(wr + 4);
#pragma unroll
                        for (int p = 0; p < 4; ++p) {
                            const float v = in6[p + kx];
                            acc[p][0] = fmaf(v, w0[0], acc[p][0]); acc[p][1] = fmaf(v, w0[1], acc[p][1]);
                            acc[p][2] = fmaf(v, w0[2], acc[p][2]); acc[p][3] = fmaf(v, w0[3], acc[p][3]);
                            acc[p][4] = fmaf(v, w1[0], acc[p][4]); acc[p][5] = fmaf(v, w1[1], acc[p][5]);
                            acc[p][6] = fmaf(v, w1[2], acc[p][6]); acc[p][7] = fmaf(v, w1[3], acc[p][7]);
                        }
                    }
                }
#pragma unroll
            for (int p = 0; p < 4; ++p) {
                const int px = x0 + ps * 4 + p;
                if (px >= W) continue;
                const long long o = (((long long)b * H + y) * W + px) * Cout + cg * 8;
                if (o32) {
                    *(f32x4*)(o32 + o) = f32x4{acc[p][0], acc[p][1], acc[p][2], acc[p][3]};
                    *(f32x4*)(o32 + o + 4) = f32x4{acc[p][4], acc[p][5], acc[p][6], acc[p][7]};
                }
                if (o16) {
                    bf16x8 h;
#pragma unroll
                    for (int i = 0; i < 8; ++i) h[i] = (bf16_t)acc[p][i];
                    *(bf16x8*)(o16 + o) = h;
                }
                if (oh) {
                    typedef _Float16 f16x8 __attribute__((ext_vector_type(8)));
                    f16x8 h;
#pragma unroll
                    for (int i = 0; i < 8; ++i) h[i] = (f16_t)acc[p][i];
                    *(f16x8*)(oh + o) = h;
                }
#pragma unroll
                for (int i = 0; i < 4; ++i) {
                    const float d0 = acc[p][i] - b0[0], d1 = acc[p][4 + i] - b1[0];
                    s0 += d0; ss0 = fmaf(d0, d0, ss0); s1 += d1; ss1 = fmaf(d1, d1, ss1);
                }
                ++cnt;
            }
        }
        if (gn_partial) {
            const float n = 4.0f * (float)cnt;
            float* r0 = red + ((cg * 2 + 0) * 16 + ps) * 3;
            float* r1 = red + ((cg * 2 + 1) * 16 + ps) * 3;
            const float m0 = cnt ? s0 / n : 0.f, m1 = cnt ? s1 / n : 0.f;
            r0[0] = n; r0[1] = b0[0] + m0; r0[2] = cnt ? fmaxf(ss0 - s0 * m0, 0.f) : 0.f;
            r1[0] = n; r1[1] = b1[0] + m1; r1[2] = cnt ? fmaxf(ss1 - s1 * m1, 0.f) : 0.f;
        }
    }
    if (gn_partial) {
        __syncthreads();
        const int G = Cout / gn_cpg, hpg = gn_cpg >> 2;
        if (tid < G) {
            float n = 0.f, mean = 0.f, m2 = 0.f;
            for (int hh = 0; hh < hpg; ++hh)
                for (int q = 0; q < 16; ++q) {
                    const float* r = red + ((tid * hpg + hh) * 16 + q) * 3;
                    vt_chan_merge(n, mean, m2, r[0], r[1], r[2]);
                }
            const int part = blockIdx.y * gridDim.x + blockIdx.x, nparts = gridDim.x * gridDim.y;
            float* o = gn_partial + (((long long)b * nparts + part) * G + tid) * 3;
            o[0] = n; o[1] = mean; o[2] = m2;
        }
    }
}

constexpr int CM_ROWS = 8, CM_PIX = 64;
#ifndef CONV_IN_OCC
#define CONV_IN_OCC 3
#endif
#ifndef CONV_IN_UNROLL
#define CONV_IN_UNROLL 1
#endif
__global__ __launch_bounds__(256, CONV_IN_OCC) void conv_in_mfma_kernel(const float* __restrict__ x, const bf16_t* __restrict__ wpk,
                                                           const float* __restrict__ bias, float* __restrict__ o32,
                                                           bf16_t* __restrict__ o16, f16_t* __restrict__ oh,
                                                           float* __restrict__ gn_partial, int H, int W) {
    constexpr int RW = CM_PIX + 2, RH = CM_ROWS + 2, C = 128;
    __shared__ __attribute__((aligned(16))) float sin[3 * RH * RW];
    __shared__ __attribute__((aligned(16))) char stgbuf[4 * 4096];
    __shared__ __attribute__((aligned(16))) char wlds[128 * 64];
    float (*red)[32][3] = (float (*)[32][3])sin;
    const int tid = threadIdx.x, lane = tid & 63, wave = tid >> 6;
    const int b = blockIdx.z, y0 = blockIdx.y * CM_ROWS, x0 = blockIdx.x * CM_PIX;
    for (int i = tid; i < 3 * RH * RW; i += 256) {
        const int c = i / (RH * RW), r = (i / RW) % RH, xx = i % RW;
        const int iy = y0 - 1 + r, ix = x0 - 1 + xx;
        float v = 0.f;
        if (iy >= 0 && iy < H && ix >= 0 && ix < W) v = x[(((long long)b * 3 + c) * H + iy) * W + ix];
        sin[i] = v;
    }
    for (int q = tid; q < 512; q += 256) {
        const int row = q >> 2, ch = q & 3;
        *(bf16x8*)(wlds + row * 64 + ((ch ^ ((row >> 2) & 3)) << 4)) = *(const bf16x8*)(wpk + C * 32 + row * 32 + ch * 8);
    }
    const int fr = lane & 15, fq = lane >> 4;
    int offb[8];
#pragma unroll
    for (int r = 0; r < 8; ++r) {
        const int k = fq * 8 + r, kk = k < 27 ? k : 0;
        const int ci = kk / 9, ky = (kk - ci * 9) / 3, kx = kk - ci * 9 - ky * 3;
        offb[r] = ((ci * RH + ky) * RW + kx) * 4;
    }
    bf16x8 wh[8];
#pragma unroll
    for (int i = 0; i < 8; ++i) wh[i] = *(const bf16x8*)(wpk + (i * 16 + fr) * 32 + fq * 8);
    const char* const wlp = wlds + fr * 64 + ((fq ^ ((fr >> 2) & 3)) << 4);
    float piv[8];
#pragma unroll
    for (int i = 0; i < 8; ++i) piv[i] = bias[64 * (i >> 2) + 16 * fq + 4 * (i & 3)];
    float gs[8], gss[8];
#pragma unroll
    for (int i = 0; i < 8; ++i) gs[i] = gss[i] = 0.f;
    int cnt = 0;
    __syncthreads();
    typedef unsigned u32x4 __attribute__((ext_vector_type(4)));
    typedef _Float16 f16x8 __attribute__((ext_vector_type(8)));
    char* const stg = stgbuf + wave * 4096;
    const f32x4 zero4 = {0.f, 0.f, 0.f, 0.f};
#pragma unroll CONV_IN_UNROLL
    for (int t = 0; t < 8; ++t) {
        const int p = wave * 128 + t * 16 + fr;
        const char* pb = (const char*)sin + ((p >> 6) * RW + (p & 63)) * 4;
        float v[8];
#pragma unroll
        for (int r = 0; r < 8; ++r) v[r] = *(const float*)(pb + offb[r]);
        if (fq == 3) { v[3] = v[4] = v[5] = 1.f; v[6] = v[7] = 0.f; }
        bf16x8 xh, xl;
#pragma unroll
        for (int r = 0; r < 8; ++r) {
            xh[r] = (bf16_t)v[r];
            xl[r] = (bf16_t)(v[r] - (float)xh[r]);
        }
        const int y = y0 + (p >> 6), xx = x0 + (p & 63);
        const bool ok = y < H && xx < W;
        const long long o = (((long long)b * H + y) * W + xx) * C + 16 * fq;
        f32x4 acc[8];
#pragma unroll
        for (int i = 0; i < 8; ++i) acc[i] = __builtin_amdgcn_mfma_f32_16x16x32_bf16(wh[i], xl, zero4, 0, 0, 0);
#pragma unroll
        for (int i = 0; i < 8; ++i) acc[i] = __builtin_amdgcn_mfma_f32_16x16x32_bf16(wh[i], xh, acc[i], 0, 0, 0);
#pragma unroll
        for (int i = 0; i < 8; ++i)
            acc[i] = __builtin_amdgcn_mfma_f32_16x16x32_bf16(*(const bf16x8*)(wlp + i * 1024), xh, acc[i], 0, 0, 0);
        if (ok && o32) {
#pragma unroll
            for (int hh = 0; hh < 2; ++hh)
#pragma unroll
                for (int i = 0; i < 4; ++i) *(f32x4*)(o32 + o + 64 * hh + 4 * i) = acc[hh * 4 + i];
        }
#pragma unroll
        for (int pass = 0; pass < 2; ++pass) {
            char* outp = pass == 0 ? (char*)oh : (char*)o16;
            if (!outp) continue;
#pragma unroll
            for (int hh = 0; hh < 2; ++hh)
#pragma unroll
                for (int i = 0; i < 4; i += 2) {
                    char* d = stg + fr * 256 + (((hh * 8 + fq * 2 + (i >> 1)) ^ fr) << 4);
                    if (pass == 0) {
                        f16x8 h;
#pragma unroll
                        for (int r = 0; r < 4; ++r) { h[r] = (f16_t)acc[hh * 4 + i][r]; h[4 + r] = (f16_t)acc[hh * 4 + i + 1][r]; }
                        *(f16x8*)d = h;
                    } else {
                        bf16x8 h;
#pragma unroll
                        for (int r = 0; r < 4; ++r) { h[r] = (bf16_t)acc[hh * 4 + i][r]; h[4 + r] = (bf16_t)acc[hh * 4 + i + 1][r]; }
                        *(bf16x8*)d = h;
                    }
                }
            asm volatile("" ::: "memory");
            const int p0 = wave * 128 + t * 16;
            const int ty = y0 + (p0 >> 6), tx = x0 + (p0 & 63);
#pragma unroll
            for (int q = 0; q < 4; ++q) {
                const int px = q * 4 + (lane >> 4), ch = lane & 15;
                const u32x4 v4 = *(const u32x4*)(stg + px * 256 + ((ch ^ px) << 4));
                if (ty < H && tx + px < W) {
#ifdef CONV_IN_NT
                    __builtin_nontemporal_store(v4, (u32x4*)(outp + ((((long long)b * H + ty) * W + tx + px) * C) * 2 + ch * 16));
#else
                    *(u32x4*)(outp + ((((long long)b * H + ty) * W + tx + px) * C) * 2 + ch * 16) = v4;
#endif
                }
            }
            asm volatile("" ::: "memory");
        }
        if (ok) {
#pragma unroll
            for (int i = 0; i < 8; ++i)
#pragma unroll
                for (int r = 0; r < 4; ++r) { const float d = acc[i][r] - piv[i]; gs[i] += d; gss[i] = fmaf(d, d, gss[i]); }
            ++cnt;
        }
    }
    if (gn_partial) {
        __syncthreads();
        const float n = vt_row16_sum(4.0f * (float)cnt);
#pragma unroll
        for (int i = 0; i < 8; ++i) {
            const float s1 = vt_row16_sum(gs[i]), s2 = vt_row16_sum(gss[i]);
            if (fr == 0) {
                const int g = 16 * (i >> 2) + 4 * fq + (i & 3);
                const float ms = n > 0.f ? s1 / n : 0.f;
                red[wave][g][0] = n; red[wave][g][1] = piv[i] + ms; red[wave][g][2] = n > 0.f ? fmaxf(s2 - s1 * ms, 0.f) : 0.f;
            }
        }
        __syncthreads();
        if (tid < 32) {
            float nn = 0.f, mean = 0.f, m2 = 0.f;
            for (int w = 0; w < 4; ++w) vt_chan_merge(nn, mean, m2, red[w][tid][0], red[w][tid][1], red[w][tid][2]);
            const int part = blockIdx.y * gridDim.x + blockIdx.x, nparts = gridDim.x * gridDim.y;
            float* o = gn_partial + (((long long)b * nparts + part) * 32 + tid) * 3;
            o[0] = nn; o[1] = mean; o[2] = m2;
        }
    }
}

template <typename T> __device__ __forceinline__ float sm_ld(const T* p, long long i) { return (float)p[i]; }

template <typename T>
__global__ __launch_bounds__(256) void softmax_rows_kernel(const T* __restrict__ s, bf16_t* __restrict__ p, int n,
                                                           int lds, int ldp) {
    __shared__ float red[8];
    const long long row = blockIdx.x;
    const T* sr = s + row * lds;
    bf16_t* pr = p + row * ldp;
    const int tid = threadIdx.x, lane = tid & 63, wv = tid >> 6;
    float m = -INFINITY;
    for (int i = tid; i < n; i += 256) m = fmaxf(m, sm_ld(sr, i));
    m = wave_max(m);
    if (lane == 0) red[wv] = m;
    __syncthreads();
    m = fmaxf(fmaxf(red[0], red[1]), fmaxf(red[2], red[3]));
    float sum = 0.f;
    for (int i = tid; i < n; i += 256) sum += __expf(sm_ld(sr, i) - m);
    sum = wave_sum(sum);
    if (lane == 0) red[4 + wv] = sum;
    __syncthreads();
    sum = (red[4] + red[5]) + (red[6] + red[7]);
    const float inv = 1.0f / sum;
    for (int i = tid; i < ldp; i += 256) pr[i] = (bf16_t)(i < n ? __expf(sm_ld(sr, i) - m) * inv : 0.f);
}

template <typename T, int NV>
__global__ __launch_bounds__(256) void softmax_rows_cached_kernel(const T* __restrict__ s, bf16_t* __restrict__ p,
                                                                  int n, int lds, int ldp) {
    __shared__ float red[8];
    const long long row = blockIdx.x;
    const T* sr = s + row * lds;
    bf16_t* pr = p + row * ldp;
    const int tid = threadIdx.x, lane = tid & 63, wv = tid >> 6;
    f32x4 v[NV];
    float m = -INFINITY;
#pragma unroll
    for (int k = 0; k < NV; ++k) {
        const int i = (k * 256 + tid) * 4;
        if (i + 3 < n) {
            if constexpr (sizeof(T) == 4) v[k] = *(const f32x4*)(sr + i);
            else { const f16x4 h = *(const f16x4*)(sr + i); v[k] = f32x4{(float)h[0], (float)h[1], (float)h[2], (float)h[3]}; }
        } else {
#pragma unroll
            for (int r = 0; r < 4; ++r) v[k][r] = (i + r < n) ? sm_ld(sr, i + r) : -INFINITY;
        }
        m = fmaxf(m, fmaxf(fmaxf(v[k][0], v[k][1]), fmaxf(v[k][2], v[k][3])));
    }
    m = wave_max(m);
    if (lane == 0) red[wv] = m;
    __syncthreads();
    m = fmaxf(fmaxf(red[0], red[1]), fmaxf(red[2], red[3]));
    float sum = 0.f;
#pragma unroll
    for (int k = 0; k < NV; ++k) {
#pragma unroll
        for (int r = 0; r < 4; ++r) { v[k][r] = __expf(v[k][r] - m); sum += v[k][r]; }
    }
    sum = wave_sum(sum);
    if (lane == 0) red[4 + wv] = sum;
    __syncthreads();
    sum = (red[4] + red[5]) + (red[6] + red[7]);
    const float inv = 1.0f / sum;
#pragma unroll
    for (int k = 0; k < NV; ++k) {
        const int i = (k * 256 + tid) * 4;
        if (i < ldp) {
            bf16x4 h;
#pragma unroll
            for (int r = 0; r < 4; ++r) h[r] = (bf16_t)(v[k][r] * inv);
            *(bf16x4*)(pr + i) = h;
        }
    }
}

__global__ __launch_bounds__(256) void preprocess_u8_kernel(const unsigned char* __restrict__ in, float* __restrict__ out,
                                                            long long HW) {
    const int b = blockIdx.y;
    const long long p = (long long)blockIdx.x * 256 + threadIdx.x;
    if (p >= HW) return;
    const unsigned char* src = in + ((long long)b * HW + p) * 3;
#pragma unroll
    for (int c = 0; c < 3; ++c) {
        const float v = __fdiv_rn((float)src[c], 255.0f);
        out[((long long)b * 3 + c) * HW + p] = (v - 0.5f) / 0.5f;
    }
}

constexpr int RS_PRECISION_BITS = 32 - 8 - 2;
__device__ __forceinline__ unsigned char rs_clip8(int v) {
    v >>= RS_PRECISION_BITS;
    return (unsigned char)(v < 0 ? 0 : (v > 255 ? 255 : v));
}
__global__ __launch_bounds__(256) void resize_h_kernel(const unsigned char* __restrict__ src, int src_w, int left, int top,
                                                       const int* __restrict__ tab, int ksize, unsigned char* __restrict__ out,
                                                       int rows, int out_w) {
    const int xx = blockIdx.x * 256 + threadIdx.x, y = blockIdx.y;
    if (xx >= out_w || y >= rows) return;
    const int* t = tab + (long long)xx * (2 + ksize);
    const int x0 = t[0], n = t[1];
    const unsigned char* p = src + ((long long)(top + y) * src_w + left + x0) * 3;
    int a0 = 1 << (RS_PRECISION_BITS - 1), a1 = a0, a2 = a0;
    for (int k = 0; k < n; ++k) {
        const int c = t[2 + k];
        a0 += p[3 * k] * c; a1 += p[3 * k + 1] * c; a2 += p[3 * k + 2] * c;
    }
    unsigned char* o = out + ((long long)y * out_w + xx) * 3;
    o[0] = rs_clip8(a0); o[1] = rs_clip8(a1); o[2] = rs_clip8(a2);
}
__global__ __launch_bounds__(256) void resize_v_kernel(const unsigned char* __restrict__ in, const int* __restrict__ tab, int ksize,
                                                       unsigned char* __restrict__ out, int w, int out_h) {
    const int xx = blockIdx.x * 256 + threadIdx.x, yy = blockIdx.y;
    if (xx >= w || yy >= out_h) return;
    const int* t = tab + (long long)yy * (2 + ksize);
    const int y0 = t[0], n = t[1];
    const unsigned char* p = in + ((long long)y0 * w + xx) * 3;
    int a0 = 1 << (RS_PRECISION_BITS - 1), a1 = a0, a2 = a0;
    for (int k = 0; k < n; ++k) {
        const int c = t[2 + k];
        const unsigned char* q = p + (long long)k * w * 3;
        a0 += q[0] * c; a1 += q[1] * c; a2 += q[2] * c;
    }
    unsigned char* o = out + ((long long)yy * w + xx) * 3;
    o[0] = rs_clip8(a0); o[1] = rs_clip8(a1); o[2] = rs_clip8(a2);
}
__global__ __launch_bounds__(256) void crop_copy_kernel(const unsigned char* __restrict__ src, int src_w, int left, int top,
                                                        unsigned char* __restrict__ out, int rows, int w) {
    const int i = blockIdx.x * 256 + threadIdx.x, y = blockIdx.y;
    if (i >= w * 3 || y >= rows) return;
    out[(long long)y * w * 3 + i] = src[((long long)(top + y) * src_w + left) * 3 + i];
}

}

hipError_t vt_launch_preprocess_u8(const unsigned char* in_hwc, float* out_nchw, int B, int H, int W, hipStream_t s) {
    if (!in_hwc || !out_nchw || B <= 0 || H <= 0 || W <= 0) return hipErrorInvalidValue;
    const long long HW = (long long)H * W;
    hipLaunchKernelGGL(preprocess_u8_kernel, dim3((unsigned)((HW + 255) / 256), B), dim3(256), 0, s, in_hwc, out_nchw, HW);
    return hipGetLastError();
}

hipError_t vt_launch_resize_u8(const unsigned char* src, int src_h, int src_w, int left, int top, int crop_w, int crop_h,
                               unsigned char* dst, int dst_h, int dst_w, const int* tab_h, int ksize_h, const int* tab_v,
                               int ksize_v, unsigned char* tmp, hipStream_t s) {
    if (!src || !dst || left < 0 || top < 0 || crop_w <= 0 || crop_h <= 0 || left + crop_w > src_w || top + crop_h > src_h ||
        dst_h <= 0 || dst_w <= 0 || dst_h > 65535 || crop_h > 65535)
        return hipErrorInvalidValue;
    const bool need_h = dst_w != crop_w, need_v = dst_h != crop_h;
    if ((need_h && !tab_h) || (need_v && !tab_v) || (need_h && need_v && !tmp)) return hipErrorInvalidValue;
    if (!need_h && !need_v) {
        hipLaunchKernelGGL(crop_copy_kernel, dim3((crop_w * 3 + 255) / 256, crop_h), dim3(256), 0, s, src, src_w, left, top, dst, crop_h, crop_w);
        return hipGetLastError();
    }
    if (need_h) {
        unsigned char* o = need_v ? tmp : dst;
        hipLaunchKernelGGL(resize_h_kernel, dim3((dst_w + 255) / 256, crop_h), dim3(256), 0, s, src, src_w, left, top, tab_h, ksize_h, o, crop_h, dst_w);
        if (need_v) hipLaunchKernelGGL(resize_v_kernel, dim3((dst_w + 255) / 256, dst_h), dim3(256), 0, s, tmp, tab_v, ksize_v, dst, dst_w, dst_h);
    } else {
        if (!tmp) return hipErrorInvalidValue;
        hipLaunchKernelGGL(crop_copy_kernel, dim3((crop_w * 3 + 255) / 256, crop_h), dim3(256), 0, s, src, src_w, left, top, tmp, crop_h, crop_w);
        hipLaunchKernelGGL(resize_v_kernel, dim3((dst_w + 255) / 256, dst_h), dim3(256), 0, s, tmp, tab_v, ksize_v, dst, dst_w, dst_h);
    }
    return hipGetLastError();
}

hipError_t vt_launch_conv_in(const float* x, const float* wp, const float* bias, float* o32, bf16_t* o16, f16_t* oh,
                             float* gn_partial, int gn_cpg, int* gn_parts, int B, int H, int W, int Cout, hipStream_t s) {
    if (!x || !wp || !bias || (!o32 && !o16 && !oh) || B <= 0 || H <= 0 || W <= 0 || Cout <= 0 || (Cout % 8))
        return hipErrorInvalidValue;
    if (gn_partial && ((gn_cpg % 4) || gn_cpg <= 0 || (Cout % gn_cpg) || Cout / gn_cpg > 256)) return hipErrorInvalidValue;
    const size_t smem = (size_t)(27 * Cout + 3 * (CI_ROWS + 2) * (CI_PIX + 2) + (Cout / 4) * 16 * 3) * sizeof(float);
    if (smem > 64 * 1024) return hipErrorInvalidValue;
    dim3 grid((W + CI_PIX - 1) / CI_PIX, (H + CI_ROWS - 1) / CI_ROWS, B);
    if (gn_parts) *gn_parts = grid.x * grid.y;
    hipLaunchKernelGGL(conv_in_kernel, grid, dim3(256), smem, s, x, wp, bias, o32, o16, oh, gn_partial, gn_cpg, H, W, Cout);
    return hipGetLastError();
}

hipError_t vt_launch_conv_in_mfma(const float* x, const bf16_t* wpk, const float* bias, float* o32, bf16_t* o16, f16_t* oh,
                                  float* gn_partial, int* gn_parts, int B, int H, int W, hipStream_t s) {
    if (!x || !wpk || !bias || (!o32 && !o16 && !oh) || B <= 0 || H <= 0 || W <= 0) return hipErrorInvalidValue;
    dim3 grid((W + CM_PIX - 1) / CM_PIX, (H + CM_ROWS - 1) / CM_ROWS, B);
    if (gn_parts) *gn_parts = grid.x * grid.y;
    hipLaunchKernelGGL(conv_in_mfma_kernel, grid, dim3(256), 0, s, x, wpk, bias, o32, o16, oh, gn_partial, H, W);
    return hipGetLastError();
}
int vt_conv_in_mfma_parts(int H, int W) { return ((W + CM_PIX - 1) / CM_PIX) * ((H + CM_ROWS - 1) / CM_ROWS); }

int vt_conv_in_parts(int H, int W) { return ((W + CI_PIX - 1) / CI_PIX) * ((H + CI_ROWS - 1) / CI_ROWS); }

template <int NV>
__global__ __launch_bounds__(256) void softmax_rows_f16x8_kernel(const f16_t* __restrict__ s, bf16_t* __restrict__ p,
                                                                 int n, int lds, int ldp) {
    typedef _Float16 f16x8 __attribute__((ext_vector_type(8)));
    __shared__ float red[8];
    const long long row = blockIdx.x;
    const f16_t* sr = s + row * lds;
    bf16_t* pr = p + row * ldp;
    const int tid = threadIdx.x, lane = tid & 63, wv = tid >> 6;
    float v[NV][8];
    float m = -INFINITY;
#pragma unroll
    for (int k = 0; k < NV; ++k) {
        const int i = (k * 256 + tid) * 8;
        if (i + 7 < n) {
            const f16x8 h = *(const f16x8*)(sr + i);
#pragma unroll
            for (int r = 0; r < 8; ++r) v[k][r] = (float)h[r];
        } else {
#pragma unroll
            for (int r = 0; r < 8; ++r) v[k][r] = (i + r < n) ? (float)sr[i + r] : -INFINITY;
        }
#pragma unroll
        for (int r = 0; r < 8; ++r) m = fmaxf(m, v[k][r]);
    }
    m = wave_max(m);
    if (lane == 0) red[wv] = m;
    __syncthreads();
    m = fmaxf(fmaxf(red[0], red[1]), fmaxf(red[2], red[3]));
    float sum = 0.f;
#pragma unroll
    for (int k = 0; k < NV; ++k)
#pragma unroll
        for (int r = 0; r < 8; ++r) { v[k][r] = __expf(v[k][r] - m); sum += v[k][r]; }
    sum = wave_sum(sum);
    if (lane == 0) red[4 + wv] = sum;
    __syncthreads();
    sum = (red[4] + red[5]) + (red[6] + red[7]);
    const float inv = 1.0f / sum;
#pragma unroll
    for (int k = 0; k < NV; ++k) {
        const int i = (k * 256 + tid) * 8;
        if (i < ldp) {
            bf16x8 h;
#pragma unroll
            for (int r = 0; r < 8; ++r) h[r] = (bf16_t)(v[k][r] * inv);
            *(bf16x8*)(pr + i) = h;
        }
    }
}

template <typename T>
static hipError_t softmax_dispatch(const T* scores, bf16_t* probs, long long rows, int n, int lds, int ldp, hipStream_t s) {
    const bool vec = (lds % 4 == 0) && (ldp % 4 == 0) && (((uintptr_t)scores) % 16 == 0) && (((uintptr_t)probs) % 8 == 0);
    const int need = (ldp + 1023) / 1024;
    const dim3 grid((unsigned)rows);
#define SMX(NV) hipLaunchKernelGGL((softmax_rows_cached_kernel<T, NV>), grid, dim3(256), 0, s, scores, probs, n, lds, ldp)
    if (vec && need <= 1) SMX(1);
    else if (vec && need <= 2) SMX(2);
    else if (vec && need <= 4) SMX(4);
    else if (vec && need <= 8) SMX(8);
    else if (vec && need <= 16) SMX(16);
    else hipLaunchKernelGGL((softmax_rows_kernel<T>), grid, dim3(256), 0, s, scores, probs, n, lds, ldp);
#undef SMX
    return hipGetLastError();
}

hipError_t vt_launch_softmax_rows(const void* scores, int scores_f16, bf16_t* probs, long long rows, int n, int lds, int ldp,
                                  hipStream_t s) {
    if (!scores || !probs || rows <= 0 || rows > 0x7fffffffLL || n <= 0 || lds < n || ldp < n) return hipErrorInvalidValue;
    if (scores_f16 && (lds % 8 == 0) && (ldp % 8 == 0) && (((uintptr_t)scores) % 16 == 0) && (((uintptr_t)probs) % 16 == 0) &&
        ldp <= 8 * 2048) {
        const int need = (ldp + 2047) / 2048;
        const dim3 grid((unsigned)rows);
#define SMH(NV) hipLaunchKernelGGL((softmax_rows_f16x8_kernel<NV>), grid, dim3(256), 0, s, (const f16_t*)scores, probs, n, lds, ldp)
        if (need <= 1) SMH(1); else if (need <= 2) SMH(2); else if (need <= 4) SMH(4); else SMH(8);
#undef SMH
        return hipGetLastError();
    }
    return scores_f16 ? softmax_dispatch((const f16_t*)scores, probs, rows, n, lds, ldp, s)
                      : softmax_dispatch((const float*)scores, probs, rows, n, lds, ldp, s);
}

namespace {

__global__ __launch_bounds__(256) void attn_row_norms_kernel(const bf16_t* __restrict__ qk, long long rows, int C,
                                                             float* __restrict__ qn, float* __restrict__ kn, float* __restrict__ sd) {
    const long long row = (long long)blockIdx.x * 4 + (threadIdx.x >> 6);
    if (row >= rows) return;
    const int lane = threadIdx.x & 63;
    const bf16_t* q = qk + row * 2 * C;
    float a = 0.f, b = 0.f, d = 0.f;
    for (int c = lane * 8; c < C; c += 512) {
        const bf16x8 qv = *(const bf16x8*)(q + c), kv = *(const bf16x8*)(q + C + c);
#pragma unroll
        for (int r = 0; r < 8; ++r) {
            const float x = (float)qv[r], y = (float)kv[r];
            a += x * x; b += y * y; d += x * y;
        }
    }
#pragma unroll
    for (int o = 32; o > 0; o >>= 1) { a += __shfl_xor(a, o); b += __shfl_xor(b, o); d += __shfl_xor(d, o); }
    if (lane == 0) { qn[row] = a; kn[row] = b; sd[row] = d; }
}

__global__ __launch_bounds__(256) VT_NO_PACKED_F32 void attn_row_norms_fp8_kernel(const bf16_t* __restrict__ qk, long long rows, int C, float scale,
                                                                 unsigned char* __restrict__ qk8, float* __restrict__ qn,
                                                                 float* __restrict__ kn, float* __restrict__ sd, int* __restrict__ status) {
    const long long row = (long long)blockIdx.x * 4 + (threadIdx.x >> 6);
    if (row >= rows) return;
    const int lane = threadIdx.x & 63;
    const bf16_t* q = qk + row * 2 * C;
    unsigned char* o = qk8 + row * 2 * C;
    const float inv = 1.0f / scale;
    float a = 0.f, b = 0.f, d = 0.f, amax = 0.f;
    typedef float f32x2 __attribute__((ext_vector_type(2)));
    for (int c = lane * 8; c < C; c += 512) {
        const bf16x8 qv = *(const bf16x8*)(q + c), kv = *(const bf16x8*)(q + C + c);
        int qw[2] = {0, 0}, kw[2] = {0, 0};
        auto pair = [&](auto p_tag) {
            constexpr int P = decltype(p_tag)::value;
            constexpr bool HI = (P & 1) != 0;
            float x0 = (float)qv[2 * P] * scale, x1 = (float)qv[2 * P + 1] * scale, y0 = (float)kv[2 * P] * scale, y1 = (float)kv[2 * P + 1] * scale;
            amax = fmaxf(fmaxf(fabsf(x0), fabsf(x1)), fmaxf(fmaxf(fabsf(y0), fabsf(y1)), amax));
            x0 = __builtin_amdgcn_fmed3f(x0, -448.f, 448.f); x1 = __builtin_amdgcn_fmed3f(x1, -448.f, 448.f);
            y0 = __builtin_amdgcn_fmed3f(y0, -448.f, 448.f); y1 = __builtin_amdgcn_fmed3f(y1, -448.f, 448.f);
            qw[P >> 1] = __builtin_amdgcn_cvt_pk_fp8_f32(x0, x1, qw[P >> 1], HI);
            kw[P >> 1] = __builtin_amdgcn_cvt_pk_fp8_f32(y0, y1, kw[P >> 1], HI);
            const f32x2 xq = __builtin_amdgcn_cvt_pk_f32_fp8(qw[P >> 1], HI), yq = __builtin_amdgcn_cvt_pk_f32_fp8(kw[P >> 1], HI);
            const float u0 = xq[0] * inv, u1 = xq[1] * inv, w0 = yq[0] * inv, w1 = yq[1] * inv;
            a += u0 * u0 + u1 * u1; b += w0 * w0 + w1 * w1; d += u0 * w0 + u1 * w1;
        };
        pair(std::integral_constant<int, 0>{}); pair(std::integral_constant<int, 1>{});
        pair(std::integral_constant<int, 2>{}); pair(std::integral_constant<int, 3>{});
        *(int2*)(o + c) = make_int2(qw[0], qw[1]);
        *(int2*)(o + C + c) = make_int2(kw[0], kw[1]);
    }
#pragma unroll
    for (int off = 32; off > 0; off >>= 1) { a += __shfl_xor(a, off); b += __shfl_xor(b, off); d += __shfl_xor(d, off); }
    if (lane == 0) { qn[row] = a; kn[row] = b; sd[row] = d; }
    if (status && amax > 448.f) atomicOr(status, 2);
}

__global__ __launch_bounds__(1024) void attn_shift_kernel(const float* __restrict__ qn, const float* __restrict__ kn,
                                                          const float* __restrict__ sd, int S, float alpha, float max_gap,
                                                          float* __restrict__ shift, int* __restrict__ flags, int group) {
    __shared__ float red[16];
// ... 69 lines not shown
```

vae_tagger_amd/csrc/ops.hip:

```cpp
#include <algorithm>

#include "vt_context.h"

using namespace vt;

namespace {

int ensure_op_scratch(vt_context* c, size_t bytes) {
    if (c->op_scratch_bytes >= bytes) return VT_OK;
    if (c->op_scratch) (void)hipFree(c->op_scratch);
    c->op_scratch = nullptr; c->op_scratch_bytes = 0;
    HIPCK(c, hipMalloc(&c->op_scratch, bytes), "hipMalloc(op scratch)");
    c->op_scratch_bytes = bytes;
    return VT_OK;
}

template <class V>
hipError_t to_device(void* dst, const std::vector<V>& v) { return hipMemcpy(dst, v.data(), v.size() * sizeof(V), hipMemcpyHostToDevice); }

}

extern "C" {

int vt_op_conv2d(vt_context* c, const void* x, const void* w, const float* bias, const float* res, float* o32, void* o16,
// ... 68 lines not shown
    if (c->use_halo_conv && ksize == 3 && stride == 1 && pad_lo == 1 && pad_hi == 1 && vt_conv3x3_halo_supported(Cin, Cout)) {
        VTCK(ensure_op_scratch(c, (size_t)Cout * 9 * Cin * 2));
        HIPCK(c, vt_launch_repack_ohwi_to_halo(cw.w, (bf16_t*)c->op_scratch, Cin, Cout, s), "repack");
        cw.wp = (const bf16_t*)c->op_scratch;
    }
    if (!bias) return c->fail(VT_ERR_INVALID, "vt_op_conv2d_gn: bias required");
    GnState gn; gn.partial = (float*)ws;
    ConvOpts o; o.gn = &gn; o.groups = groups;
    const int saved = c->fuse_gn_stats; c->fuse_gn_stats = 1;
    int r = run_conv(c, cw, (const bf16_t*)x, B, Hin, Win, stride, pad_lo, Hout, Wout, res, o32, (bf16_t*)o16, s, o);
    c->fuse_gn_stats = saved;
    if (r) return r;
    if (gn.parts == 0) return c->fail(VT_ERR_INVALID, "vt_op_conv2d_gn: this shape has no stats epilogue");
    HIPCK(c, vt_launch_gn_finalize(gn.partial, gn.parts, B, Cout, groups, eps, gamma, beta, scale_shift, s), "gn_finalize");
    return VT_OK;
}

static int op_upsample2x_conv3x3(vt_context* c, const void* x, const float* w, const float* bias, float* o32, int B, int h, int wd, int C,
                                 int groups, float eps, const float* gamma, const float* beta, float* scale_shift, hipStream_t s) {
    if (!x || !w || !o32) return c->fail(VT_ERR_INVALID, "vt_op_upsample2x_conv3x3: null buffer");
    if (B <= 0 || h <= 0 || wd <= 0 || C < 8 || (C % 8)) return c->fail(VT_ERR_INVALID, "vt_op_upsample2x_conv3x3: bad shape");
    if ((long long)B * h * wd * C >= (1LL << 29)) return c->fail(VT_ERR_INVALID, "vt_op_upsample2x_conv3x3: tensor too large for the operator entry");
    const bool f16 = c->f16_ops != 0;
    const bool want_gn = scale_shift != nullptr;
    const bool folded = !c->up2_literal && vt_conv3x3_up2_supported(C, C);
    const int cpg = want_gn ? C / groups : 0;
    const int parts_max = std::max({vt_conv3x3_up2_tiles(h, wd), vt_conv3x3_halo_tiles_max(2 * h, 2 * wd), vt_conv_gemm_ptiles(4 * h * wd, C)});
    const size_t gn_bytes = want_gn ? align_up((size_t)B * parts_max * groups * 3 * 4) : 0;
    const size_t w_bytes = align_up((size_t)C * C * 16 * 2), up_bytes = align_up((size_t)B * 4 * h * wd * C * 2);
    VTCK(ensure_op_scratch(c, gn_bytes + w_bytes + (folded ? 0 : up_bytes)));
    char* p = (char*)c->op_scratch;
    GnState gn; gn.partial = (float*)p; p += gn_bytes;
    bf16_t* wp = (bf16_t*)p; p += w_bytes;
    if (folded) {
        HIPCK(c, vt_launch_pack_up2(w, f16 ? nullptr : wp, f16 ? (f16_t*)wp : nullptr, C, C, s), "pack_up2");
        ConvUp2Args a{};
        a.X = (const bf16_t*)x; a.Wp = wp; a.bias = bias; a.out_f32 = o32; a.zeros = c->zeros; a.batch = B; a.H = h; a.W = wd; a.Cin = C; a.Cout = C; a.f16 = f16;
        if (want_gn) { a.gn_partial = gn.partial; a.gn_cpg = cpg; gn.parts = vt_conv3x3_up2_tiles(h, wd); }
        HIPCK(c, vt_launch_conv3x3_up2(a, s), "conv3x3_up2");
    } else {
        bf16_t* up = (bf16_t*)p;
        const bool halo = c->use_halo_conv && vt_conv3x3_halo_supported(C, C);
        if (f16 && !(halo && vt_conv3x3_halo_f16_supported(C, c->halo_occ2, 0)))
            return c->fail(VT_ERR_INVALID, "vt_op_upsample2x_conv3x3: the literal route has no fp16-operand kernel for %d channels", C);
        HIPCK(c, vt_launch_upsample2x_nhwc16(x, up, B, h, wd, C, s), "upsample2x");
        HIPCK(c, vt_launch_pack_f32_oihw(w, wp, C, C, halo ? 1 : 0, f16, s), "pack_f32_oihw");
        ConvW cw; cw.cin = C; cw.cout = C; cw.k = 3; cw.b = bias;
        if (halo) { cw.wp = wp; cw.wp16 = wp; } else cw.w = wp;
        ConvOpts o; o.x_f16 = f16; o.groups = want_gn ? groups : 32; o.gn = want_gn ? &gn : nullptr;
        const int saved = c->fuse_gn_stats; c->fuse_gn_stats = 1;
        const int r = run_conv(c, cw, up, B, 2 * h, 2 * wd, 1, 1, 2 * h, 2 * wd, nullptr, o32, nullptr, s, o);
        c->fuse_gn_stats = saved;
        if (r) return r;
    }
    if (want_gn) {
        if (gn.parts == 0) return c->fail(VT_ERR_INVALID, "vt_op_upsample2x_conv3x3_gn: this shape has no stats epilogue");
        HIPCK(c, vt_launch_gn_finalize(gn.partial, gn.parts, B, C, groups, eps, gamma, beta, scale_shift, s), "gn_finalize");
    }
    return VT_OK;
}

int vt_op_upsample2x_conv3x3(vt_context* c, const void* x, const float* w_oihw, const float* bias, float* o32, int B, int h, int w, int C,
                             void* stream) {
    if (!c) return VT_ERR_INVALID;
    DeviceGuard guard(c);
    return op_upsample2x_conv3x3(c, x, w_oihw, bias, o32, B, h, w, C, 0, 0.f, nullptr, nullptr, nullptr, (hipStream_t)stream);
}

int vt_op_upsample2x_conv3x3_gn(vt_context* c, const void* x, const float* w_oihw, const float* bias, float* o32, int B, int h, int w, int C,
                                int groups, float eps, const float* gamma, const float* beta, float* scale_shift, void* stream) {
    if (!c) return VT_ERR_INVALID;
    DeviceGuard guard(c);
    if (!gamma || !beta || !scale_shift || !bias || groups < 1 || groups > 64 || C % groups) return c->fail(VT_ERR_INVALID, "vt_op_upsample2x_conv3x3_gn: bad argument");
    const int cpg = C / groups;
    if (cpg != 4 && cpg != 8 && cpg != 16) return c->fail(VT_ERR_INVALID, "vt_op_upsample2x_conv3x3_gn: channels per group must be 4, 8 or 16");
    return op_upsample2x_conv3x3(c, x, w_oihw, bias, o32, B, h, w, C, groups, eps, gamma, beta, scale_shift, (hipStream_t)stream);
}

size_t vt_op_conv3x3_fp8_workspace_bytes(int B, int H, int W, int Cin, int Cout) {
    if (B <= 0 || H <= 0 || W <= 0 || !vt_conv3x3_halo_fp8_supported(Cin, Cout)) return 0;
    return align_up((size_t)B * H * W * Cin) + align_up((size_t)B * Cin * 8) + align_up((size_t)Cout * 9 * Cin) + align_up((size_t)Cout * 4) + ALIGN;
}

int vt_op_conv3x3_fp8(vt_context* c, const float* x_nhwc, const float* w_oihw, const float* bias, const float* res, float* o32,
                      int B, int H, int W, int Cin, int Cout, int stride, void* ws, void* stream) {
    if (!c) return VT_ERR_INVALID;
    DeviceGuard guard(c);
    if (!x_nhwc || !w_oihw || !o32 || !ws || ((uintptr_t)ws % ALIGN)) return c->fail(VT_ERR_INVALID, "vt_op_conv3x3_fp8: bad buffer");
    if (vt_op_conv3x3_fp8_workspace_bytes(B, H, W, Cin, Cout) == 0 || (stride != 1 && stride != 2)) return c->fail(VT_ERR_INVALID, "vt_op_conv3x3_fp8: unsupported shape");
    hipStream_t s = (hipStream_t)stream;
    char* p = (char*)ws;
    unsigned char* x8 = (unsigned char*)p; p += align_up((size_t)B * H * W * Cin);
    float* ss = (float*)p; p += align_up((size_t)B * Cin * 8);
    unsigned char* w8 = (unsigned char*)p; p += align_up((size_t)Cout * 9 * Cin);
    float* mult = (float*)p;
    std::vector<float> hw((size_t)Cout * 9 * Cin), hss((size_t)B * Cin * 2);
    HIPCK(c, hipMemcpy(hw.data(), w_oihw, hw.size() * 4, hipMemcpyDeviceToHost), "vt_op_conv3x3_fp8 copy");
    const bool s2_kernel = stride == 2 && c->s2_halo && vt_conv3x3_s2_fp8_supported(Cin, Cout);
    const ConvE4m3 pk = pack_conv_e4m3(hw.data(), Cout, Cin, s2_kernel);
    for (size_t i = 0; i < hss.size(); i += 2) { hss[i] = 1.f; hss[i + 1] = 0.f; }
    HIPCK(c, to_device(ss, hss), "vt_op_conv3x3_fp8 copy");
    if (stride == 2) {
        HIPCK(c, to_device(w8, s2_kernel ? pk.wp8s2 : pk.w8g), "vt_op_conv3x3_fp8 copy");
        HIPCK(c, to_device(mult, pk.mult8g), "vt_op_conv3x3_fp8 copy");
        HIPCK(c, vt_launch_gn_apply(x_nhwc, 1, ss, x8, B, H * W, Cin, 0, s, FP8_RES_SCALE), "vt_op_conv3x3_fp8 quantise");
        ConvW cw; cw.cin = Cin; cw.cout = Cout; cw.k = 3; cw.w8g = w8; cw.mult8g = mult; cw.b = bias;
        if (s2_kernel) cw.wp8s2 = w8;
        ConvOpts o; o.x_fp8 = true;
        return run_conv(c, cw, (const bf16_t*)x8, B, H, W, 2, 0, H / 2, W / 2, res, o32, nullptr, s, o);
    }
    HIPCK(c, to_device(w8, pk.wp8), "vt_op_conv3x3_fp8 copy");
    HIPCK(c, to_device(mult, pk.mult8), "vt_op_conv3x3_fp8 copy");
    HIPCK(c, vt_launch_gn_apply(x_nhwc, 1, ss, x8, B, H * W, Cin, 0, s, FP8_ACT_SCALE), "vt_op_conv3x3_fp8 quantise");
    Conv3x3Fp8Args h{};
    h.X = x8; h.Wp = w8; h.mult = mult; h.bias = bias; h.res = res; h.out_f32 = o32; h.zeros = c->zeros;
    h.batch = B; h.H = H; h.W = W; h.Cin = Cin; h.Cout = Cout;
    h.shape = (Cin <= 128 || (c->fp8_tile & 4)) ? (c->fp8_tile & 3) : 0;
    return launch_halo_fp8(c, h, s, "vt_op_conv3x3_fp8");
}

int vt_op_gemm_nt(vt_context* c, const void* A, const void* Bm, const float* bias, float* o32, void* o16, int batch, int M,
                  int N, int K, int lda, int ldb, int ldo, long long a_bs, long long b_bs, long long o_bs, float alpha,
                  int bias_per_row, void* stream) {
    if (!c) return VT_ERR_INVALID;
    DeviceGuard guard(c);
    if (!A || !Bm || (!o32 && !o16)) return c->fail(VT_ERR_INVALID, "vt_op_gemm_nt: null buffer");
    ConvGemmArgs a{};
    a.X = (const bf16_t*)A; a.W = (const bf16_t*)Bm; a.bias = bias; a.out_f32 = o32; a.out_bf16 = (bf16_t*)o16; a.zeros = c->zeros;
    a.Hin = a.Hout = 1; a.Win = a.Wout = M; a.Cin = K; a.Cout = N; a.Wrows = N; a.ksize = 1; a.stride = 1; a.pad = 0;
    a.ldx = lda; a.ldw = ldb; a.ldo = ldo; a.x_bs = a_bs; a.w_bs = b_bs; a.o_bs = o_bs; a.batch = batch; a.alpha = alpha;
    a.bias_mode = bias ? (bias_per_row ? 2 : 1) : 0;
    return launch_gemm(c, a, (hipStream_t)stream, "vt_op_gemm_nt");
}

int vt_op_conv_in(vt_context* c, const float* x, const float* w_oihw, const float* bias, float* o32, void* o16, int B,
                  int H, int W, int Cout, void* ws, void* stream) {
    if (!c) return VT_ERR_INVALID;
    DeviceGuard guard(c);
    if (!x || !w_oihw || !bias || !ws) return c->fail(VT_ERR_INVALID, "vt_op_conv_in: null buffer");
    std::vector<float> hw((size_t)Cout * 27);
    HIPCK(c, hipMemcpy(hw.data(), w_oihw, hw.size() * 4, hipMemcpyDeviceToHost), "vt_op_conv_in copy");
    if (Cout == 128 && c->conv_in_mfma) {
        std::vector<float> hb(128);
        HIPCK(c, hipMemcpy(hb.data(), bias, 128 * 4, hipMemcpyDeviceToHost), "vt_op_conv_in copy");
        HIPCK(c, to_device(ws, pack_conv_in_mfma(hw.data(), hb.data())), "vt_op_conv_in copy");
        HIPCK(c, vt_launch_conv_in_mfma(x, (const bf16_t*)ws, bias, o32, (bf16_t*)o16, nullptr, nullptr, nullptr, B, H, W, (hipStream_t)stream), "vt_op_conv_in");
        return VT_OK;
    }
    HIPCK(c, to_device(ws, pack_conv_in(hw.data(), Cout)), "vt_op_conv_in copy");
    HIPCK(c, vt_launch_conv_in(x, (const float*)ws, bias, o32, (bf16_t*)o16, nullptr, nullptr, 0, nullptr, B, H, W, Cout, (hipStream_t)stream), "vt_op_conv_in");
    return VT_OK;
}

size_t vt_op_groupnorm_workspace_bytes(int B, int HW, int C) {
    if (B <= 0 || HW <= 0 || C < 8 || (C % 8)) return 0;
    return align_up((size_t)B * vt_gn_max_chunks(HW, C) * 64 * 3 * 4) + align_up((size_t)B * C * 2 * 4);
}

int vt_op_groupnorm(vt_context* c, const void* x, int x_dtype, int B, int HW, int C, int groups, float eps,
                    const float* gamma, const float* beta, int silu, void* y, void* ws, void* stream) {
    if (!c) return VT_ERR_INVALID;
    DeviceGuard guard(c);
    if (!x || !gamma || !beta || !y || !ws) return c->fail(VT_ERR_INVALID, "vt_op_groupnorm: null buffer");
    if (x_dtype != VT_F32 && x_dtype != VT_BF16 && x_dtype != VT_F16) return c->fail(VT_ERR_INVALID, "vt_op_groupnorm: dtype must be f32, bf16 or f16");
    if (groups > 64) return c->fail(VT_ERR_INVALID, "vt_op_groupnorm: groups > 64");
    hipStream_t s = (hipStream_t)stream;
    float* partial = (float*)ws;
    float* ss = (float*)((char*)ws + align_up((size_t)B * vt_gn_max_chunks(HW, C) * 64 * 3 * 4));
    int nchunks = 0;
    const int f = x_dtype == VT_F32 ? 1 : (x_dtype == VT_F16 ? 2 : 0);
    HIPCK(c, vt_launch_gn_stats(x, f, B, HW, C, groups, partial, &nchunks, s), "gn_stats");
    HIPCK(c, vt_launch_gn_finalize(partial, nchunks, B, C, groups, eps, gamma, beta, ss, s), "gn_finalize");
    HIPCK(c, vt_launch_gn_apply(x, f, ss, (bf16_t*)y, B, HW, C, silu, s), "gn_apply");
    return VT_OK;
}

int vt_op_softmax_rows(vt_context* c, const float* scores, void* probs, int rows, int n, int lds, int ldp, void* stream) {
    if (!c) return VT_ERR_INVALID;
    DeviceGuard guard(c);
    HIPCK(c, vt_launch_softmax_rows(scores, 0, (bf16_t*)probs, rows, n, lds, ldp, (hipStream_t)stream), "vt_op_softmax_rows");
    return VT_OK;
}

}
```

vae_tagger_amd/csrc/vt_context.h:

```cpp
#pragma once
#include <hip/hip_runtime.h>
#include <stdarg.h>
#include <stdio.h>

#include <array>
#include <map>
#include <string>
#include <vector>

#include "../../include/vae_tagger_hip.h"
#include "vt_decoder.h"
#include "vt_kernels.h"

namespace vt {

struct HostTensor {
    std::vector<float> v;
    std::vector<int64_t> shape;
    int64_t numel() const { int64_t n = 1; for (auto d : shape) n *= d; return n; }
};

struct ConvW {
    const bf16_t* w = nullptr; const bf16_t* wp = nullptr; const float* b = nullptr; int cin = 0, cout = 0, k = 0;
    const bf16_t* wp2 = nullptr;
    const bf16_t* wpo = nullptr; const bf16_t* wpo16 = nullptr;
    const bf16_t* w16 = nullptr; const bf16_t* wp16 = nullptr; const bf16_t* wp2_16 = nullptr;
    const unsigned char* wp8 = nullptr; const float* mult8 = nullptr;
    const unsigned char* w8g = nullptr; const float* mult8g = nullptr;
    const unsigned char* wp8s2 = nullptr;
};
struct NormW { const float* g = nullptr; const float* b = nullptr; int c = 0; };
struct ResnetW {
    NormW n1, n2; ConvW c1, c2, sc; bool has_sc = false; int cin = 0, cout = 0;
    const bf16_t* sc_wp = nullptr; const float* b_c2sc = nullptr;
    const bf16_t* sc_wp16 = nullptr;
    const bf16_t* sc_wp8 = nullptr;
};
struct AttnW { NormW gn; const bf16_t *wqk = nullptr, *wv = nullptr, *wo = nullptr; const float *bqk = nullptr, *bv = nullptr, *bo = nullptr; int c = 0;
               const unsigned char *wqk8 = nullptr, *wv8 = nullptr; float sqk = 1.f, sv = 1.f; };
struct StageW { std::vector<ResnetW> res; bool has_down = false; ConvW down; };

struct EncoderW {
    bool configured = false, finalized = false;
    int in_ch = 3, latent = 16, layers = 2, groups = 32;
    std::vector<int> block_out;
    float scaling = 1.f, shift = 0.f;
    bool has_scaling = false, has_shift = false;
    const bf16_t* conv_in_wpk = nullptr;
    const float* conv_in_w = nullptr;
    const float* conv_in_b = nullptr;
    std::vector<StageW> stages;
    ResnetW mid0, mid1;
    AttnW attn;
    NormW norm_out;
    ConvW conv_out;
};

struct UpBlockW {
    std::vector<ResnetW> res; bool has_up = false;
    ConvW up;
    const bf16_t* up_wp = nullptr; const bf16_t* up_wp16 = nullptr;
};
struct ImageDecoderW {
    bool configured = false, finalized = false;
    int out_ch = 3, latent = 16, layers = 2, groups = 32;
    std::vector<int> block_out;
    float scaling = 1.f, shift = 0.f;
    bool has_scaling = false, has_shift = false;
    ConvW conv_in;
    int conv_in_cin() const { return (latent + 31) / 32 * 32; }
    ResnetW mid0, mid1;
    AttnW attn;
    std::vector<UpBlockW> ups;
    NormW norm_out;
    ConvW conv_out;
};

constexpr float FP8_ACT_SCALE = 8.0f;
constexpr float FP8_RES_SCALE = 1.0f;

constexpr size_t ALIGN = 256;
inline size_t align_up(size_t x) { return (x + ALIGN - 1) / ALIGN * ALIGN; }

}

struct vt_context {
    int device = 0;
    std::string err;
    std::map<std::string, vt::HostTensor> weights;
    std::vector<void*> enc_allocs, dec_allocs, imgdec_allocs;
    vt::ImageDecoderW imgdec;
    std::vector<void*>* cur_allocs = &enc_allocs;
    bool pack_fp8 = true;
    void* zeros = nullptr;
    int* status = nullptr;
    vt::EncoderW enc;
    DecoderWeights dec;
    bool dec_configured = false, dec_finalized = false;
    int use_halo_conv = 1;
    int fuse_gn_stats = 1;
    int fuse_gn_apply = 0;
    int res_fp16 = 1;
    int attn_mode = 0;
    int fuse_shortcut = 1;
    int pv_stream = 1;
    int attn_qk_kernel = 1;
    int attn_pv_kernel = 1;
    int fp8 = 0;
    int halo_occ2 = 3;
    int gemm_short = 1;
    int proj_fp8 = 1;
    int attn_fp8 = 1;
    unsigned long long* dbg = nullptr; int dbg_n = 0; bool dbg_on = false;
    int conv_out_halo = 1;
    int s2_planar = 1;
    int eval_merge_vec = 1;
    int f16_ops = 0;
    int attn_proj_kernel = 1;
    int fp8_tile = 0;
    int up2_literal = 0;
    int s2_halo = 1;
    int* rs_host = nullptr; size_t rs_host_ints = 0; hipEvent_t rs_event = nullptr;
    struct RsRingSlot { void* host = nullptr; size_t bytes = 0; hipEvent_t ev = nullptr; bool used = false; };
    static constexpr int RS_RING = 4;
    RsRingSlot rs_ring[RS_RING];
    unsigned rs_ring_next = 0;
    std::map<std::array<int, 4>, std::vector<int>> rs_tables;
    int conv_in_mfma = 1;
    void* op_scratch = nullptr; size_t op_scratch_bytes = 0;

    struct ProfRec { hipEvent_t e0, e1; double flops; int cfg; };
    bool profiling = false;
    std::vector<ProfRec> prof;
    std::vector<hipEvent_t> event_pool;
    size_t events_used = 0;
    hipEvent_t next_event() {
        if (events_used == event_pool.size()) {
            hipEvent_t e = nullptr;
            if (hipEventCreate(&e) != hipSuccess) return nullptr;
            event_pool.push_back(e);
        }
        return event_pool[events_used++];
    }

    int fail(int code, const char* fmt, ...) {
        char buf[512];
        va_list ap; va_start(ap, fmt); vsnprintf(buf, sizeof buf, fmt, ap); va_end(ap);
        err = buf;
        return code;
    }
    int hipfail(hipError_t e, const char* what) { return fail(VT_ERR_HIP, "%s: %s", what, hipGetErrorString(e)); }

    void* upload(const void* host, size_t bytes) {
        void* d = nullptr;
        if (hipMalloc(&d, bytes ? bytes : 16) != hipSuccess) return nullptr;
        cur_allocs->push_back(d);
        if (bytes && hipMemcpy(d, host, bytes, hipMemcpyHostToDevice) != hipSuccess) return nullptr;
        return d;
    }
    void free_allocs(std::vector<void*>& v) {
        for (void* p : v) (void)hipFree(p);
        v.clear();
    }
    const vt::HostTensor* find(const std::string& k) const {
        auto it = weights.find(k);
        return it == weights.end() ? nullptr : &it->second;
    }
};

namespace vt {

struct DeviceGuard {
    int prev = -1, dev;
    explicit DeviceGuard(const vt_context* c) : dev(c->device) {
        if (hipGetDevice(&prev) != hipSuccess) prev = -1;
        if (prev != dev) (void)hipSetDevice(dev);
    }
    ~DeviceGuard() { if (prev >= 0 && prev != dev) (void)hipSetDevice(prev); }
};

#define HIPCK(ctx, e, what) do { hipError_t _e = (e); if (_e != hipSuccess) return (ctx)->hipfail(_e, what); } while (0)
#define VTCK(e) do { const int _r = (e); if (_r) return _r; } while (0)

template <class Launch>
int profiled(vt_context* c, hipStream_t s, int slot, double count, const char* what, Launch&& launch) {
    if (!c->profiling) { HIPCK(c, launch(), what); return VT_OK; }
    vt_context::ProfRec r;
    r.e0 = c->next_event(); r.e1 = c->next_event();
    if (!r.e0 || !r.e1) return c->fail(VT_ERR_HIP, "event pool exhausted");
    r.flops = count; r.cfg = slot;
    HIPCK(c, hipEventRecord(r.e0, s), "hipEventRecord");
    HIPCK(c, launch(), what);
    HIPCK(c, hipEventRecord(r.e1, s), "hipEventRecord");
    c->prof.push_back(r);
    return VT_OK;
}

float bf2f(uint16_t h);
float h2f(uint16_t h);
std::vector<float> pack_conv_in(const float* w_o27, int cout);
std::vector<uint16_t> pack_conv_in_mfma(const float* w_o27, const float* bias);
struct ConvE4m3 {
    std::vector<uint8_t> wp8;  std::vector<float> mult8;
    std::vector<uint8_t> w8g;  std::vector<float> mult8g;
    std::vector<uint8_t> wp8s2;
};
ConvE4m3 pack_conv_e4m3(const float* w_oihw, int cout, int cin, bool s2_layout);

int rs_ksize(int in_size, int out_size, int kind);
void rs_table(int in_size, int out_size, int kind, int* tab);

void dbg_sum(vt_context* c, const void* p, size_t bytes, hipStream_t s);

struct GnState {
    float* partial = nullptr; float* ss = nullptr;
    int parts = 0;
};
struct ScFuse { const bf16_t* x; const bf16_t* wp; const float* bias; int cin; const bf16_t* wp8; const bf16_t* wp16;
                bool x_f16;
};
struct ConvOpts {
    GnState* gn = nullptr;
    int groups = 32;
    const float* xnorm_f32 = nullptr; const float* ss = nullptr;
    int rdt = 1;
    const ScFuse* sc = nullptr;
    bool x_fp8 = false, o16_e4m3 = false;
    bool x_f16 = false;
    bool o16_f16 = false;
    bool planar = false;
};
int launch_gemm(vt_context* c, const ConvGemmArgs& a, hipStream_t s, const char* what);
int launch_halo(vt_context* c, const Conv3x3Args& a, hipStream_t s, const char* what);
int launch_halo_fp8(vt_context* c, const Conv3x3Fp8Args& a, hipStream_t s, const char* what);
int run_conv(vt_context* c, const ConvW& w, const bf16_t* x, int B, int Hin, int Win, int stride, int pad, int Hout, int Wout,
             const void* res, void* oh, bf16_t* o16, hipStream_t s, const ConvOpts& o = ConvOpts());
int run_gn(vt_context* c, const void* x, int xdt, int B, int HW, const NormW& n, int groups, int silu, bf16_t* y, GnState& g, hipStream_t s,
           bool out_fp8 = false, bool out_f16 = false);
bool conv_f16(const vt_context* c, const ConvW& w, int stride, bool has_sc);
struct NormConvOpts { const ScFuse* sc = nullptr; bool o16_e4m3 = false, o16_f16 = false, o16_planar = false; };
int run_norm_conv(vt_context* c, const NormW& n, const ConvW& w, const void* x, int xdt, int B, int H, int W, int groups, bf16_t* act,
                  const void* res, void* oh, bf16_t* o16, GnState& gn, bool want_stats, hipStream_t s, int rdt, const NormConvOpts& nc = NormConvOpts());

struct AttnScratch {
    bf16_t* qk; bf16_t* vt; f16_t* scores; bf16_t* probs; bf16_t* o;
    unsigned char* qk8; unsigned char* vt8;
    unsigned char* x8; float* ident;
    float* qn; float* kn; float* sd; float* shift; float* rinv; float* part; int* flags;
    int group;
};
size_t attn_scratch_bytes(int B, int S, int C);
AttnScratch carve_attn(char* p, int B, int S, int C);
bool attn_proj_is_fp8(const vt_context* c, const AttnW& w, int S, int C);
int run_attention(vt_context* c, const AttnW& w, const bf16_t* x16, const void* res, void* out, int B, int S, const AttnScratch& sc,
                  hipStream_t s, GnState* gn = nullptr, int groups = 32, int rdt = 1, bool x_e4m3 = false);

}
```

vae_tagger_amd/csrc/vt_kernels.h:

```cpp
#pragma once
#include <hip/hip_runtime.h>
#include "vt_common.h"

struct ConvGemmArgs {
    const bf16_t* X;
    const bf16_t* W;
    const float* bias;
    const float* res;
    const f16_t* res_f16;
    float* out_f32;
    bf16_t* out_bf16;
    f16_t* out_f16;
    const void* zeros;
    float* gn_partial;
    int Hin, Win, Hout, Wout;
    int Cin, Cout;
    int Wrows;
    int ksize, stride, pad;
    int ldx, ldw, ldo, ldr;
    long long x_bs, w_bs, o_bs, r_bs;
    int batch;
    float alpha;
    int bias_mode;
    int out_mode;
// ... 100 lines not shown
struct AttnPv8Args {
    const unsigned char* P8; long long p_bs;
    const unsigned char* vt8; int ldv; long long vt_bs;
    int kext;
    bf16_t* o; int ldo; long long o_bs;
    float out_scale;
    const int* gate; int gate_expect;
    int S, C, batch;
    const void* zeros;
};
bool vt_attn_fp8_supported(int S, int C);
__host__ __device__ inline long long vt_attn_p8_slab_stride(int S) { return (long long)((S + 127) / 128) * 4096 + 2304; }
long long vt_attn_p8_bytes(int S);
hipError_t vt_launch_attn_qk_fp8(const AttnQk8Args& a, hipStream_t s);
hipError_t vt_launch_attn_pv_fp8(const AttnPv8Args& a, hipStream_t s);
hipError_t vt_launch_attn_vt_to_fp8(const bf16_t* vt, long long vt_bs, int ldv, unsigned char* v8, long long v8_bs, int ld8, int S, int kext,
                                    int C, int batch, float scale, int* status, hipStream_t s);
hipError_t vt_launch_attn_row_norms_fp8(const bf16_t* qk, long long rows, int C, float scale, unsigned char* qk8, float* qn, float* kn, float* sd,
                                        int* status, hipStream_t s);

struct Conv3x3Args {
    const bf16_t* X;
    const float* Xf32;
    const float* scale_shift;
    const bf16_t* Wp;
    const float* bias;
    const float* res;
    const f16_t* res_f16;
    float* out_f32;
    bf16_t* out_bf16;
    f16_t* out_f16;
    const void* zeros;
    float* gn_partial;
    int gn_cpg;
    int batch, H, W, Cin, Cout;
    const bf16_t* scX;
    const bf16_t* scW;
    int scCin;
    int occ2;
    int f16;
    int out16_f16;
    int out16_planar;
    int tiles_x, ctiles, per_img, ptiles;
    unsigned long long m_per_img, m_ctiles, m_tiles_x;
};
int vt_conv3x3_halo_tiles(int H, int W, int Cout, int xt, int occ2, int has_sc);
int vt_conv3x3_halo_tiles_max(int H, int W);
int vt_conv_gemm_ptiles(int HWo, int Cout);
int vt_conv_gemm_ptiles_of(const ConvGemmArgs& a);
bool vt_conv3x3_halo_supported(int Cin, int Cout);
bool vt_conv3x3_halo_f16_supported(int Cout, int occ2, int has_sc);
int vt_conv3x3_halo_config(const Conv3x3Args& a);
hipError_t vt_launch_conv3x3_halo(const Conv3x3Args& a, hipStream_t s);
hipError_t vt_launch_repack_ohwi_to_halo(const bf16_t* w_ohwi, bf16_t* wp, int Cin, int Cout, hipStream_t s);

struct ConvUp2Args {
    const bf16_t* X;
    const bf16_t* Wp;
    const float* bias;
    float* out_f32; f16_t* out_f16;
    bf16_t* out_16; int out16_f16;
    const void* zeros;
    float* gn_partial; int gn_cpg;
    int batch, H, W, Cin, Cout;
    int f16;
    int tiles_x, ptiles, ctiles;
};
bool vt_conv3x3_up2_supported(int Cin, int Cout);
int vt_conv3x3_up2_tiles(int H, int W);
hipError_t vt_launch_conv3x3_up2(const ConvUp2Args& a, hipStream_t s);
hipError_t vt_launch_pack_up2(const float* w_oihw, bf16_t* wp_bf16, f16_t* wp_f16, int Cin, int Cout, hipStream_t s);
hipError_t vt_launch_pack_f32_oihw(const float* w_oihw, bf16_t* dst, int Cin, int Cout, int layout, int f16, hipStream_t s);
hipError_t vt_launch_upsample2x_nhwc16(const void* x, void* y, int B, int H, int W, int C, hipStream_t s);

struct Conv3x3S2Args {
    const bf16_t* X;
    const bf16_t* Wp;
    const float* bias;
    const float* res;
    float* out_f32; bf16_t* out_bf16; f16_t* out_f16;
    const void* zeros;
    float* gn_partial; int gn_cpg;
    int batch, H, W, Cin, Cout;
    int f16, out16_f16;
    int x_planar;
    int Ho, Wo, tiles_x, ctiles, per_img, ptiles;
    unsigned long long m_per_img, m_ctiles, m_tiles_x;
};
bool vt_conv3x3_s2_supported(int Cin, int Cout);
int vt_conv3x3_s2_tiles(int Ho, int Wo);
hipError_t vt_launch_conv3x3_s2(const Conv3x3S2Args& a, hipStream_t s);
hipError_t vt_launch_repack_ohwi_to_s2(const bf16_t* w_ohwi, bf16_t* wp, int Cin, int Cout, hipStream_t s);

struct Conv3x3S2Fp8Args {
    const unsigned char* X;
    const unsigned char* Wp;
    const float* mult;
    const float* bias;
    const float* res;
    float* out_f32; bf16_t* out_bf16; f16_t* out_f16;
    const void* zeros;
    float* gn_partial; int gn_cpg;
    int batch, H, W, Cin, Cout;
    int x_planar;
    int Ho, Wo, tiles_x, ctiles, per_img, ptiles;
    unsigned long long m_per_img, m_ctiles, m_tiles_x;
};
bool vt_conv3x3_s2_fp8_supported(int Cin, int Cout);
int vt_conv3x3_s2_fp8_tiles(int Ho, int Wo);
hipError_t vt_launch_conv3x3_s2_fp8(const Conv3x3S2Fp8Args& a, hipStream_t s);

struct Conv3x3Fp8Args {
    const unsigned char* X;
    const unsigned char* Wp;
    const float* mult;
    const float* bias;
    const float* res; const f16_t* res_f16;
    float* out_f32; bf16_t* out_bf16; f16_t* out_f16;
    unsigned char* out_e4m3; float out_e4m3_scale;
    int out8_planar;
    int* status;
    const void* zeros;
    float* gn_partial; int gn_cpg;
    int batch, H, W, Cin, Cout;
    const bf16_t* scX; const bf16_t* scW; int scCin;
    int shape;
    int tiles_x, ctiles, per_img, ptiles;
    unsigned long long m_per_img, m_ctiles, m_tiles_x;
};
bool vt_conv3x3_halo_fp8_supported(int Cin, int Cout);
int vt_conv3x3_halo_fp8_tiles(int H, int W);
int vt_conv3x3_halo_fp8_tiles_shape(int H, int W, int shape);
int vt_halo_fp8_row_of_cout(int cout_local );
hipError_t vt_launch_conv3x3_halo_fp8(const Conv3x3Fp8Args& a, hipStream_t s);

struct ConvOutArgs {
    const bf16_t* X;
    const bf16_t* Wp;
    const float* bias;
    float* out;
    const void* zeros;
    int batch, H, W, Cin, Cout, keep;
    float post_scale, post_shift;
    int f16;
};
bool vt_conv_out_halo_supported(int Cin, int Cout);
hipError_t vt_launch_conv_out_halo(const ConvOutArgs& a, hipStream_t s);

hipError_t vt_launch_conv_in(const float* x_nchw, const float* w_packed , const float* bias,
                             float* out_f32, bf16_t* out_bf16, f16_t* out_f16, float* gn_partial, int gn_cpg, int* gn_parts,
                             int B, int H, int W, int Cout, hipStream_t s);
int vt_conv_in_parts(int H, int W);
hipError_t vt_launch_conv_in_mfma(const float* x_nchw, const bf16_t* wpk, const float* bias, float* out_f32, bf16_t* out_bf16,
                                  f16_t* out_f16, float* gn_partial, int* gn_parts, int B, int H, int W, hipStream_t s);
int vt_conv_in_mfma_parts(int H, int W);

hipError_t vt_launch_gn_stats(const void* x, int x_dtype, int B, int HW, int C, int groups,
                              float* partial, int* nchunks_out, hipStream_t s);
hipError_t vt_launch_gn_finalize(const float* partial , int nparts, int B, int C, int groups,
                                 float eps, const float* gamma, const float* beta, float* scale_shift ,
                                 hipStream_t s, int* status = nullptr );
int vt_gn_max_chunks(int HW, int C);
hipError_t vt_launch_gn_apply(const void* x, int x_dtype, const float* scale_shift, void* y, int B, int HW,
                              int C, int silu, hipStream_t s, float out_fp8_scale = 0.f,
                              int* status = nullptr ,
                              int out_f16 = 0 );

hipError_t vt_launch_preprocess_u8(const unsigned char* in_hwc, float* out_nchw, int B, int H, int W, hipStream_t s);
hipError_t vt_launch_resize_u8(const unsigned char* src, int src_h, int src_w, int left, int top, int crop_w, int crop_h,
                               unsigned char* dst, int dst_h, int dst_w, const int* tab_h, int ksize_h, const int* tab_v,
                               int ksize_v, unsigned char* tmp, hipStream_t s);

hipError_t vt_launch_attn_row_norms(const bf16_t* qk, long long rows, int C, float* qn, float* kn, float* sd, hipStream_t s);
hipError_t vt_launch_attn_shift(const float* qn, const float* kn, const float* sd, int images, int S, float alpha, float max_gap,
                                float* shift, int* flags, int group, hipStream_t s);
hipError_t vt_launch_attn_row_reduce(const float* part, int slots, long long row_bs, int S, int batch, int op, float* out,
                                     const int* gate, int gate_expect, hipStream_t s);
hipError_t vt_launch_softmax_rows(const void* scores, int scores_f16, bf16_t* probs, long long rows, int n, int lds,
                                  int ldp, hipStream_t s);

struct DecoderWeights;
```

Measured before the change: 217.5.

## Fuse conv_in with first GroupNorm+SiLU via stats-only pass and recompute-apply pass

Runs the 3-channel conv_in twice: once computing only GroupNorm statistics with no output store, then again emitting both the raw fp16 residual and the normalized SiLU activation directly. This drops the separate gn_apply pass over the full-resolution 128-channel activation, and with it the read-back of that tensor. The conv_in kernel is also restructured to process horizontal strips of tiles with double-buffered, vectorized halo loads. The cost is recomputing the cheap conv and higher LDS use per block. Adds an op entry point and a flag to toggle the path.

```diff
diff --git a/include/vae_tagger_hip.h b/include/vae_tagger_hip.h
--- a/include/vae_tagger_hip.h
+++ b/include/vae_tagger_hip.h
@@ -236,6 +236,10 @@
                   long long b_bs, long long o_bs, float alpha, int bias_per_row, void* stream);
 int vt_op_conv_in(vt_context* ctx, const float* x_nchw, const float* w_oihw, const float* bias, float* out_f32,
                   void* out_bf16, int B, int H, int W, int Cout, void* workspace, void* stream);
+size_t vt_op_conv_in_norm_workspace_bytes(int B, int H, int W);
+int vt_op_conv_in_norm(vt_context* ctx, const float* x_nchw, const float* w_oihw, const float* bias, const float* gamma, const float* beta,
+                       int groups, float eps, int fused, void* x0_out_f16, void* a1_out_16, int a1_is_f16, int B, int H, int W,
+                       void* workspace, size_t workspace_bytes, void* stream);
 size_t vt_op_groupnorm_workspace_bytes(int B, int HW, int C);
 int vt_op_groupnorm(vt_context* ctx, const void* x, int x_dtype, int B, int HW, int C, int groups, float eps,
                     const float* gamma, const float* beta, int silu, void* y_bf16, void* workspace, void* stream);
diff --git a/vae_tagger_amd/_lib.py b/vae_tagger_amd/_lib.py
--- a/vae_tagger_amd/_lib.py
+++ b/vae_tagger_amd/_lib.py
@@ -144,6 +144,8 @@
     "vt_op_conv3x3_fp8": (_i, [_vp, _vp, _vp, _vp, _vp, _vp, _i, _i, _i, _i, _i, _i, _vp, _vp]),
     "vt_op_gemm_nt": (_i, [_vp, _vp, _vp, _vp, _vp, _vp, _i, _i, _i, _i, _i, _i, _i, _ll, _ll, _ll, _f, _i, _vp]),
     "vt_op_conv_in": (_i, [_vp, _vp, _vp, _vp, _vp, _vp, _i, _i, _i, _i, _vp, _vp]),
+    "vt_op_conv_in_norm_workspace_bytes": (_sz, [_i, _i, _i]),
+    "vt_op_conv_in_norm": (_i, [_vp, _vp, _vp, _vp, _vp, _vp, _i, _f, _i, _vp, _vp, _i, _i, _i, _i, _vp, _sz, _vp]),
     "vt_op_groupnorm_workspace_bytes": (_sz, [_i, _i, _i]),
     "vt_op_groupnorm": (_i, [_vp, _vp, _i, _i, _i, _i, _i, _f, _vp, _vp, _i, _vp, _vp, _vp]),
     "vt_op_softmax_rows": (_i, [_vp, _vp, _vp, _i, _i, _i, _i, _vp]),
diff --git a/vae_tagger_amd/csrc/capi.hip b/vae_tagger_amd/csrc/capi.hip
--- a/vae_tagger_amd/csrc/capi.hip
+++ b/vae_tagger_amd/csrc/capi.hip
@@ -470,6 +470,7 @@
     if (flag == 21) { c->eval_merge_vec = value != 0; return VT_OK; }
     if (flag == 20) { c->conv_out_halo = value != 0; return VT_OK; }
     if (flag == 22) { c->up2_literal = value != 0; return VT_OK; }
+    if (flag == 23) { c->conv_in_norm = value != 0; return VT_OK; }
     if (flag == 13) { c->s2_halo = value != 0; return VT_OK; }
     if (flag == 14) { c->attn_fp8 = value != 0; return VT_OK; }
     if (flag == 15) { c->proj_fp8 = value != 0; return VT_OK; }
diff --git a/vae_tagger_amd/csrc/encoder.hip b/vae_tagger_amd/csrc/encoder.hip
--- a/vae_tagger_amd/csrc/encoder.hip
+++ b/vae_tagger_amd/csrc/encoder.hip
@@ -173,10 +173,11 @@
     if (nc.o16_e4m3 && !f8) return c->fail(VT_ERR_STATE, "internal: e4m3 output requested from a bf16 conv");
     ConvOpts o;
     o.gn = want_stats ? &gn : nullptr; o.groups = groups; o.rdt = rdt;
+    if (nc.act_ready && (f8 || xdt != 2)) return c->fail(VT_ERR_STATE, "internal: a ready-made operand for a conv that wants another one");
     if (f8 || xdt == 2 || !norm_conv_fusable(c, w, n.c)) {
         const bool h16 = !f8 && conv_f16(c, w, 1, sc != nullptr) && (!sc || sc->x_f16);
         if (sc && sc->x_f16 && !h16) return c->fail(VT_ERR_STATE, "internal: fp16 shortcut input for a bf16 conv");
-        VTCK(run_gn(c, x, xdt, B, H * W, n, groups, 1, act, gn, s, f8, h16));
+        if (!nc.act_ready) VTCK(run_gn(c, x, xdt, B, H * W, n, groups, 1, act, gn, s, f8, h16));
         o.sc = sc; o.x_fp8 = f8; o.o16_e4m3 = nc.o16_e4m3; o.x_f16 = h16; o.o16_f16 = nc.o16_f16; o.planar = nc.o16_planar;
         return run_conv(c, w, act, B, H, W, 1, 1, H, W, res, oh, o16, s, o);
     }
@@ -239,6 +240,7 @@
     int cur = 0;
     bf16_t *act, *tmid, *hb;
     int h, w;
+    bool act_ready = false;
     const bf16_t* h16 = nullptr;
     bool h16_is_f16 = false;
 
@@ -259,6 +261,21 @@
         int parts = 0;
         float* o32 = rdt == 1 ? (float*)f32[cur] : nullptr;
         f16_t* oh = rdt == 2 ? (f16_t*)f32[cur] : nullptr;
+        const ResnetW& r0 = e.stages[0].res[0];
+        if (c->conv_in_norm && c->conv_in_mfma && e.conv_in_wpk && fuse0 && rdt == 2 && !c->fp8 && !c->fuse_gn_apply && !r0.has_sc &&
+            r0.n1.c == 128 && e.groups == 32) {
+            const NormW& n = r0.n1;
+            HIPCK(c, vt_launch_conv_in_mfma(x, e.conv_in_wpk, e.conv_in_b, nullptr, nullptr, nullptr, gn.partial, &parts, B, h, w, s), "conv_in_mfma (statistics)");
+            HIPCK(c, vt_launch_gn_finalize(gn.partial, parts, B, n.c, e.groups, 1e-6f, n.g, n.b, gn.ss, s, c->status), "gn_finalize");
+            dbg_sum(c, gn.partial, (size_t)B * parts * e.groups * 3 * 4, s);
+            dbg_sum(c, gn.ss, (size_t)B * n.c * 2 * 4, s);
+            const int apply = conv_f16(c, r0.c1, 1, false) ? 2 : 1;
+            const double bytes = (double)B * h * w * (3 * 4.0 + n.c * (2.0 + 2.0));
+            VTCK(profiled(c, s, VT_PROF_GN_APPLY, bytes, "conv_in_norm",
+                          [&] { return vt_launch_conv_in_mfma(x, e.conv_in_wpk, e.conv_in_b, nullptr, act, oh, nullptr, nullptr, B, h, w, s, gn.ss, apply); }));
+            gn.parts = 0; act_ready = true;
+            return VT_OK;
+        }
         if (c->conv_in_mfma && e.conv_in_wpk) {
             HIPCK(c, vt_launch_conv_in_mfma(x, e.conv_in_wpk, e.conv_in_b, o32, nullptr, oh, fuse0 ? gn.partial : nullptr, &parts,
                                             B, h, w, s), "conv_in_mfma");
@@ -290,8 +307,10 @@
         }
         const bool c1h = rdt == 2;
         const int c1dt = c1h ? 2 : 0;
+        NormConvOpts c1;
+        c1.act_ready = act_ready; act_ready = false;
         VTCK(run_norm_conv(c, rw.n1, rw.c1, f32[cur], rdt, B, h, w, e.groups, act, nullptr, c1h ? (void*)tmid : nullptr,
-                           c1h ? nullptr : tmid, gn, true, s, rdt));
+                           c1h ? nullptr : tmid, gn, true, s, rdt, c1));
         if (out.only16) {
             c2.o16_e4m3 = out.e4m3; c2.o16_f16 = out.f16; c2.o16_planar = out.planar;
             return run_norm_conv(c, rw.n2, rw.c2, tmid, c1dt, B, h, w, e.groups, act, res, nullptr, hb, gn, false, s, rdt, c2);
diff --git a/vae_tagger_amd/csrc/misc_kernels.hip b/vae_tagger_amd/csrc/misc_kernels.hip
--- a/vae_tagger_amd/csrc/misc_kernels.hip
+++ b/vae_tagger_amd/csrc/misc_kernels.hip
@@ -119,30 +119,75 @@
 }
 
 constexpr int CM_ROWS = 8, CM_PIX = 64;
+constexpr int CM_RW = 72, CM_RH = CM_ROWS + 2, CM_COL0 = 3;
 #ifndef CONV_IN_OCC
 #define CONV_IN_OCC 3
 #endif
 #ifndef CONV_IN_UNROLL
 #define CONV_IN_UNROLL 1
 #endif
+#ifndef CONV_IN_STRIP
+#define CONV_IN_STRIP 4
+#endif
+template <bool STORE, int APPLY, bool STATS>
 __global__ __launch_bounds__(256, CONV_IN_OCC) void conv_in_mfma_kernel(const float* __restrict__ x, const bf16_t* __restrict__ wpk,
                                                            const float* __restrict__ bias, float* __restrict__ o32,
-                                                           bf16_t* __restrict__ o16, f16_t* __restrict__ oh,
-                                                           float* __restrict__ gn_partial, int H, int W) {
-    constexpr int RW = CM_PIX + 2, RH = CM_ROWS + 2, C = 128;
-    __shared__ __attribute__((aligned(16))) float sin[3 * RH * RW];
-    __shared__ __attribute__((aligned(16))) char stgbuf[4 * 4096];
+                                                           void* __restrict__ o16, f16_t* __restrict__ oh,
+                                                           float* __restrict__ gn_partial, const float* __restrict__ scale_shift,
+                                                           int H, int W, int tiles_x, int strip) {
+    constexpr int RW = CM_RW, RH = CM_RH, C = 128, HALO = 3 * RH * RW, NSEG = 3 * RH * 16, NEDGE = 3 * RH * 2;
+    static_assert(STORE || APPLY == 0, "the applied output is a store");
+    __shared__ __attribute__((aligned(16))) float sin[2 * HALO];
+    __shared__ __attribute__((aligned(16))) char stgbuf[STORE ? 4 * 4096 : 16];
     __shared__ __attribute__((aligned(16))) char wlds[128 * 64];
-    float (*red)[32][3] = (float (*)[32][3])sin;
+    __shared__ float red[STATS ? 2 : 1][4][32][3];
     const int tid = threadIdx.x, lane = tid & 63, wave = tid >> 6;
-    const int b = blockIdx.z, y0 = blockIdx.y * CM_ROWS, x0 = blockIdx.x * CM_PIX;
-    for (int i = tid; i < 3 * RH * RW; i += 256) {
-        const int c = i / (RH * RW), r = (i / RW) % RH, xx = i % RW;
-        const int iy = y0 - 1 + r, ix = x0 - 1 + xx;
-        float v = 0.f;
-        if (iy >= 0 && iy < H && ix >= 0 && ix < W) v = x[(((long long)b * 3 + c) * H + iy) * W + ix];
-        sin[i] = v;
-    }
+    const int b = blockIdx.z, y0 = blockIdx.y * CM_ROWS;
+    const int t0 = blockIdx.x * strip, ntile = min(strip, tiles_x - t0);
+    const bool vec = (W & 3) == 0 && (((uintptr_t)x) & 15) == 0;
+    const float* const xb = x + (long long)b * 3 * H * W;
+    int rowo[2]; bool rowok[2]; int segx[2], ldso[2];
+#pragma unroll
+    for (int j = 0; j < 2; ++j) {
+        const int sl = min(tid + 256 * j, NSEG - 1), row = sl >> 4, ch = row / RH, r = row - ch * RH, iy = y0 - 1 + r;
+        rowok[j] = tid + 256 * j < NSEG && iy >= 0 && iy < H;
+        rowo[j] = (ch * H + (rowok[j] ? iy : 0)) * W;
+        segx[j] = (sl & 15) * 4;
+        ldso[j] = row * RW + CM_COL0 + 1 + segx[j];
+    }
+    const int erow = min(tid, NEDGE - 1) >> 1, ech = erow / RH, eiy = y0 - 1 + (erow - ech * RH), edx = (tid & 1) ? CM_PIX : -1;
+    const bool erowok = tid < NEDGE && eiy >= 0 && eiy < H;
+    const int erowo = (ech * H + (erowok ? eiy : 0)) * W;
+    const int eldso = erow * RW + CM_COL0 + 1 + edx;
+    f32x4 pv[2]; float pe;
+    auto fetch = [&](int tx0) {
+#pragma unroll
+        for (int j = 0; j < 2; ++j) {
+            const int ix = tx0 + segx[j];
+            if (vec) {
+                const bool ok = rowok[j] && ix < W;
+                const f32x4 q = *(const f32x4*)(xb + (ok ? rowo[j] + ix : 0));
+                pv[j] = ok ? q : f32x4{0.f, 0.f, 0.f, 0.f};
+            } else {
+#pragma unroll
+                for (int e = 0; e < 4; ++e) {
+                    const bool ok = rowok[j] && ix + e < W;
+                    const float q = xb[ok ? rowo[j] + ix + e : 0];
+                    pv[j][e] = ok ? q : 0.f;
+                }
+            }
+        }
+        const int ex = tx0 + edx;
+        const bool eok = erowok && ex >= 0 && ex < W;
+        const float q = xb[eok ? erowo + ex : 0];
+        pe = eok ? q : 0.f;
+    };
+    auto put = [&](float* buf) {
+        *(f32x4*)(buf + ldso[0]) = pv[0];
+        if (tid < NSEG - 256) *(f32x4*)(buf + ldso[1]) = pv[1];
+        if (tid < NEDGE) buf[eldso] = pe;
+    };
+    fetch(t0 * CM_PIX);
     for (int q = tid; q < 512; q += 256) {
         const int row = q >> 2, ch = q & 3;
         *(bf16x8*)(wlds + row * 64 + ((ch ^ ((row >> 2) & 3)) << 4)) = *(const bf16x8*)(wpk + C * 32 + row * 32 + ch * 8);
@@ -153,120 +198,162 @@
     for (int r = 0; r < 8; ++r) {
         const int k = fq * 8 + r, kk = k < 27 ? k : 0;
         const int ci = kk / 9, ky = (kk - ci * 9) / 3, kx = kk - ci * 9 - ky * 3;
-        offb[r] = ((ci * RH + ky) * RW + kx) * 4;
+        offb[r] = ((ci * RH + ky) * RW + kx + CM_COL0) * 4;
     }
     bf16x8 wh[8];
 #pragma unroll
     for (int i = 0; i < 8; ++i) wh[i] = *(const bf16x8*)(wpk + (i * 16 + fr) * 32 + fq * 8);
     const char* const wlp = wlds + fr * 64 + ((fq ^ ((fr >> 2) & 3)) << 4);
     float piv[8];
-#pragma unroll
-    for (int i = 0; i < 8; ++i) piv[i] = bias[64 * (i >> 2) + 16 * fq + 4 * (i & 3)];
-    float gs[8], gss[8];
-#pragma unroll
-    for (int i = 0; i < 8; ++i) gs[i] = gss[i] = 0.f;
-    int cnt = 0;
+    if constexpr (STATS) {
+#pragma unroll
+        for (int i = 0; i < 8; ++i) piv[i] = bias[64 * (i >> 2) + 16 * fq + 4 * (i & 3)];
+    }
+    float sc[8], sh[8];
+    if constexpr (APPLY != 0) {
+        const float* ssb = scale_shift + ((long long)b * C + (lane & 15) * 8) * 2;
+#pragma unroll
+        for (int i = 0; i < 4; ++i) {
+            const f32x4 q = *(const f32x4*)(ssb + i * 4);
+            sc[2 * i] = q[0]; sh[2 * i] = q[1]; sc[2 * i + 1] = q[2]; sh[2 * i + 1] = q[3];
+        }
+    }
+    put(sin);
     __syncthreads();
     typedef unsigned u32x4 __attribute__((ext_vector_type(4)));
     typedef _Float16 f16x8 __attribute__((ext_vector_type(8)));
-    char* const stg = stgbuf + wave * 4096;
+    char* const stg = stgbuf + (STORE ? wave * 4096 : 0);
     const f32x4 zero4 = {0.f, 0.f, 0.f, 0.f};
+    for (int tk = 0; tk < ntile; ++tk) {
+        const int x0 = (t0 + tk) * CM_PIX, cur = tk & 1;
+        const bool more = tk + 1 < ntile;
+        if (more) fetch(x0 + CM_PIX);
+        const char* const hb = (const char*)(sin + cur * HALO);
+        float gs[8], gss[8];
+#pragma unroll
+        for (int i = 0; i < 8; ++i) gs[i] = gss[i] = 0.f;
+        int cnt = 0;
 #pragma unroll CONV_IN_UNROLL
-    for (int t = 0; t < 8; ++t) {
-        const int p = wave * 128 + t * 16 + fr;
-        const char* pb = (const char*)sin + ((p >> 6) * RW + (p & 63)) * 4;
-        float v[8];
-#pragma unroll
-        for (int r = 0; r < 8; ++r) v[r] = *(const float*)(pb + offb[r]);
-        if (fq == 3) { v[3] = v[4] = v[5] = 1.f; v[6] = v[7] = 0.f; }
-        bf16x8 xh, xl;
-#pragma unroll
-        for (int r = 0; r < 8; ++r) {
-            xh[r] = (bf16_t)v[r];
-            xl[r] = (bf16_t)(v[r] - (float)xh[r]);
-        }
-        const int y = y0 + (p >> 6), xx = x0 + (p & 63);
-        const bool ok = y < H && xx < W;
-        const long long o = (((long long)b * H + y) * W + xx) * C + 16 * fq;
-        f32x4 acc[8];
-#pragma unroll
-        for (int i = 0; i < 8; ++i) acc[i] = __builtin_amdgcn_mfma_f32_16x16x32_bf16(wh[i], xl, zero4, 0, 0, 0);
-#pragma unroll
-        for (int i = 0; i < 8; ++i) acc[i] = __builtin_amdgcn_mfma_f32_16x16x32_bf16(wh[i], xh, acc[i], 0, 0, 0);
-#pragma unroll
-        for (int i = 0; i < 8; ++i)
-            acc[i] = __builtin_amdgcn_mfma_f32_16x16x32_bf16(*(const bf16x8*)(wlp + i * 1024), xh, acc[i], 0, 0, 0);
-        if (ok && o32) {
-#pragma unroll
-            for (int hh = 0; hh < 2; ++hh)
-#pragma unroll
-                for (int i = 0; i < 4; ++i) *(f32x4*)(o32 + o + 64 * hh + 4 * i) = acc[hh * 4 + i];
-        }
-#pragma unroll
-        for (int pass = 0; pass < 2; ++pass) {
-            char* outp = pass == 0 ? (char*)oh : (char*)o16;
-            if (!outp) continue;
-#pragma unroll
-            for (int hh = 0; hh < 2; ++hh)
-#pragma unroll
-                for (int i = 0; i < 4; i += 2) {
-                    char* d = stg + fr * 256 + (((hh * 8 + fq * 2 + (i >> 1)) ^ fr) << 4);
-                    if (pass == 0) {
-                        f16x8 h;
-#pragma unroll
-                        for (int r = 0; r < 4; ++r) { h[r] = (f16_t)acc[hh * 4 + i][r]; h[4 + r] = (f16_t)acc[hh * 4 + i + 1][r]; }
-                        *(f16x8*)d = h;
-                    } else {
-                        bf16x8 h;
-#pragma unroll
-                        for (int r = 0; r < 4; ++r) { h[r] = (bf16_t)acc[hh * 4 + i][r]; h[4 + r] = (bf16_t)acc[hh * 4 + i + 1][r]; }
-                        *(bf16x8*)d = h;
+        for (int t = 0; t < 8; ++t) {
+            const int p = wave * 128 + t * 16 + fr;
+            const char* pb = hb + ((p >> 6) * RW + (p & 63)) * 4;
+            float v[8];
+#pragma unroll
+            for (int r = 0; r < 8; ++r) v[r] = *(const float*)(pb + offb[r]);
+            if (fq == 3) { v[3] = v[4] = v[5] = 1.f; v[6] = v[7] = 0.f; }
+            bf16x8 xh, xl;
+#pragma unroll
+            for (int r = 0; r < 8; ++r) {
+                xh[r] = (bf16_t)v[r];
+                xl[r] = (bf16_t)(v[r] - (float)xh[r]);
+            }
+            const int y = y0 + (p >> 6), xx = x0 + (p & 63);
+            const bool ok = y < H && xx < W;
+            f32x4 acc[8];
+#pragma unroll
+            for (int i = 0; i < 8; ++i) acc[i] = __builtin_amdgcn_mfma_f32_16x16x32_bf16(wh[i], xl, zero4, 0, 0, 0);
+#pragma unroll
+            for (int i = 0; i < 8; ++i) acc[i] = __builtin_amdgcn_mfma_f32_16x16x32_bf16(wh[i], xh, acc[i], 0, 0, 0);
+#pragma unroll
+            for (int i = 0; i < 8; ++i)
+                acc[i] = __builtin_amdgcn_mfma_f32_16x16x32_bf16(*(const bf16x8*)(wlp + i * 1024), xh, acc[i], 0, 0, 0);
+            if constexpr (STORE) {
+                if (ok && o32) {
+                    const long long o = (((long long)b * H + y) * W + xx) * C + 16 * fq;
+#pragma unroll
+                    for (int hh = 0; hh < 2; ++hh)
+#pragma unroll
+                        for (int i = 0; i < 4; ++i) *(f32x4*)(o32 + o + 64 * hh + 4 * i) = acc[hh * 4 + i];
+                }
+                const int p0 = wave * 128 + t * 16;
+                const int ty = y0 + (p0 >> 6), tx = x0 + (p0 & 63);
+#pragma unroll
+                for (int pass = 0; pass < (APPLY != 0 ? 1 : 2); ++pass) {
+                    char* outp = pass == 0 ? (char*)oh : (char*)o16;
+                    if (!outp) continue;
+#pragma unroll
+                    for (int hh = 0; hh < 2; ++hh)
+#pragma unroll
+                        for (int i = 0; i < 4; i += 2) {
+                            char* d = stg + fr * 256 + (((hh * 8 + fq * 2 + (i >> 1)) ^ fr) << 4);
+                            if (pass == 0) {
+                                f16x8 h;
+#pragma unroll
+                                for (int r = 0; r < 4; ++r) { h[r] = (f16_t)acc[hh * 4 + i][r]; h[4 + r] = (f16_t)acc[hh * 4 + i + 1][r]; }
+                                *(f16x8*)d = h;
+                            } else {
+                                bf16x8 h;
+#pragma unroll
+                                for (int r = 0; r < 4; ++r) { h[r] = (bf16_t)acc[hh * 4 + i][r]; h[4 + r] = (bf16_t)acc[hh * 4 + i + 1][r]; }
+                                *(bf16x8*)d = h;
+                            }
+                        }
+                    asm volatile("" ::: "memory");
+#pragma unroll
+                    for (int q = 0; q < 4; ++q) {
+                        const int px = q * 4 + (lane >> 4), ch = lane & 15;
+                        const u32x4 v4 = *(const u32x4*)(stg + px * 256 + ((ch ^ px) << 4));
+                        if (ty < H && tx + px < W) {
+                            const long long ob = ((((long long)b * H + ty) * W + tx + px) * C) * 2 + ch * 16;
+                            if constexpr (APPLY != 0) {
+                                __builtin_nontemporal_store(v4, (u32x4*)(outp + ob));
+                                const f16x8 hx = __builtin_bit_cast(f16x8, v4);
+                                float a[8];
+#pragma unroll
+                                for (int i = 0; i < 8; ++i) a[i] = vt_silu(fmaf((float)hx[i], sc[i], sh[i]));
+                                if constexpr (APPLY == 2) {
+                                    f16x8 oa;
+#pragma unroll
+                                    for (int i = 0; i < 8; ++i) oa[i] = (f16_t)a[i];
+                                    __builtin_nontemporal_store(oa, (f16x8*)((char*)o16 + ob));
+                                } else {
+                                    bf16x8 oa;
+#pragma unroll
+                                    for (int i = 0; i < 8; ++i) oa[i] = (bf16_t)a[i];
+                                    __builtin_nontemporal_store(oa, (bf16x8*)((char*)o16 + ob));
+                                }
+                            } else {
+#ifdef CONV_IN_NT
+                                __builtin_nontemporal_store(v4, (u32x4*)(outp + ob));
+#else
+                                *(u32x4*)(outp + ob) = v4;
+#endif
+                            }
+                        }
                     }
-                }
-            asm volatile("" ::: "memory");
-            const int p0 = wave * 128 + t * 16;
-            const int ty = y0 + (p0 >> 6), tx = x0 + (p0 & 63);
-#pragma unroll
-            for (int q = 0; q < 4; ++q) {
-                const int px = q * 4 + (lane >> 4), ch = lane & 15;
-                const u32x4 v4 = *(const u32x4*)(stg + px * 256 + ((ch ^ px) << 4));
-                if (ty < H && tx + px < W) {
-#ifdef CONV_IN_NT
-                    __builtin_nontemporal_store(v4, (u32x4*)(outp + ((((long long)b * H + ty) * W + tx + px) * C) * 2 + ch * 16));
-#else
-                    *(u32x4*)(outp + ((((long long)b * H + ty) * W + tx + px) * C) * 2 + ch * 16) = v4;
-#endif
+                    asm volatile("" ::: "memory");
                 }
             }
-            asm volatile("" ::: "memory");
-        }
-        if (ok) {
-#pragma unroll
-            for (int i = 0; i < 8; ++i)
-#pragma unroll
-                for (int r = 0; r < 4; ++r) { const float d = acc[i][r] - piv[i]; gs[i] += d; gss[i] = fmaf(d, d, gss[i]); }
-            ++cnt;
-        }
-    }
-    if (gn_partial) {
-        __syncthreads();
-        const float n = vt_row16_sum(4.0f * (float)cnt);
-#pragma unroll
-        for (int i = 0; i < 8; ++i) {
-            const float s1 = vt_row16_sum(gs[i]), s2 = vt_row16_sum(gss[i]);
-            if (fr == 0) {
-                const int g = 16 * (i >> 2) + 4 * fq + (i & 3);
-                const float ms = n > 0.f ? s1 / n : 0.f;
-                red[wave][g][0] = n; red[wave][g][1] = piv[i] + ms; red[wave][g][2] = n > 0.f ? fmaxf(s2 - s1 * ms, 0.f) : 0.f;
+            if (STATS && ok) {
+#pragma unroll
+                for (int i = 0; i < 8; ++i)
+#pragma unroll
+                    for (int r = 0; r < 4; ++r) { const float d = acc[i][r] - piv[i]; gs[i] += d; gss[i] = fmaf(d, d, gss[i]); }
+                ++cnt;
             }
         }
-        __syncthreads();
-        if (tid < 32) {
-            float nn = 0.f, mean = 0.f, m2 = 0.f;
-            for (int w = 0; w < 4; ++w) vt_chan_merge(nn, mean, m2, red[w][tid][0], red[w][tid][1], red[w][tid][2]);
-            const int part = blockIdx.y * gridDim.x + blockIdx.x, nparts = gridDim.x * gridDim.y;
-            float* o = gn_partial + (((long long)b * nparts + part) * 32 + tid) * 3;
-            o[0] = nn; o[1] = mean; o[2] = m2;
+        if (more) put(sin + (cur ^ 1) * HALO);
+        if constexpr (STATS) {
+            const float n = vt_row16_sum(4.0f * (float)cnt);
+#pragma unroll
+            for (int i = 0; i < 8; ++i) {
+                const float s1 = vt_row16_sum(gs[i]), s2 = vt_row16_sum(gss[i]);
+                if (fr == 0) {
+                    const int g = 16 * (i >> 2) + 4 * fq + (i & 3);
+                    const float ms = n > 0.f ? s1 / n : 0.f;
+                    red[cur][wave][g][0] = n; red[cur][wave][g][1] = piv[i] + ms; red[cur][wave][g][2] = n > 0.f ? fmaxf(s2 - s1 * ms, 0.f) : 0.f;
+                }
+            }
+        }
+        if (more || STATS) __syncthreads();
+        if constexpr (STATS) {
+            if (tid < 32) {
+                float nn = 0.f, mean = 0.f, m2 = 0.f;
+                for (int w = 0; w < 4; ++w) vt_chan_merge(nn, mean, m2, red[cur][w][tid][0], red[cur][w][tid][1], red[cur][w][tid][2]);
+                const int part = blockIdx.y * tiles_x + t0 + tk, nparts = tiles_x * gridDim.y;
+                float* o = gn_partial + (((long long)b * nparts + part) * 32 + tid) * 3;
+                o[0] = nn; o[1] = mean; o[2] = m2;
+            }
         }
     }
 }
@@ -450,11 +537,23 @@
 }
 
 hipError_t vt_launch_conv_in_mfma(const float* x, const bf16_t* wpk, const float* bias, float* o32, bf16_t* o16, f16_t* oh,
-                                  float* gn_partial, int* gn_parts, int B, int H, int W, hipStream_t s) {
-    if (!x || !wpk || !bias || (!o32 && !o16 && !oh) || B <= 0 || H <= 0 || W <= 0) return hipErrorInvalidValue;
-    dim3 grid((W + CM_PIX - 1) / CM_PIX, (H + CM_ROWS - 1) / CM_ROWS, B);
-    if (gn_parts) *gn_parts = grid.x * grid.y;
-    hipLaunchKernelGGL(conv_in_mfma_kernel, grid, dim3(256), 0, s, x, wpk, bias, o32, o16, oh, gn_partial, H, W);
+                                  float* gn_partial, int* gn_parts, int B, int H, int W, hipStream_t s,
+                                  const float* scale_shift, int apply) {
+    const bool store = o32 || o16 || oh;
+    if (!x || !wpk || !bias || (!store && !gn_partial) || B <= 0 || H <= 0 || W <= 0 || B > 65535 || 3LL * H * W > 0x7fffffffLL) return hipErrorInvalidValue;
+    if (apply && (apply < 0 || apply > 2 || !scale_shift || !oh || !o16 || o32 || gn_partial)) return hipErrorInvalidValue;
+    const int tiles_x = (W + CM_PIX - 1) / CM_PIX, strip = CONV_IN_STRIP;
+    dim3 grid((tiles_x + strip - 1) / strip, (H + CM_ROWS - 1) / CM_ROWS, B);
+    if (grid.y > 65535) return hipErrorInvalidValue;
+    if (gn_parts) *gn_parts = tiles_x * grid.y;
+#define CONV_IN_MFMA(ST, AP, GN) hipLaunchKernelGGL((conv_in_mfma_kernel<ST, AP, GN>), grid, dim3(256), 0, s, x, wpk, bias, o32, (void*)o16, oh, \
+                                                    gn_partial, scale_shift, H, W, tiles_x, strip)
+    if (apply == 1) CONV_IN_MFMA(true, 1, false);
+    else if (apply == 2) CONV_IN_MFMA(true, 2, false);
+    else if (!store) CONV_IN_MFMA(false, 0, true);
+    else if (gn_partial) CONV_IN_MFMA(true, 0, true);
+    else CONV_IN_MFMA(true, 0, false);
+#undef CONV_IN_MFMA
     return hipGetLastError();
 }
 int vt_conv_in_mfma_parts(int H, int W) { return ((W + CM_PIX - 1) / CM_PIX) * ((H + CM_ROWS - 1) / CM_ROWS); }
diff --git a/vae_tagger_amd/csrc/ops.hip b/vae_tagger_amd/csrc/ops.hip
--- a/vae_tagger_amd/csrc/ops.hip
+++ b/vae_tagger_amd/csrc/ops.hip
@@ -244,6 +244,38 @@
     return VT_OK;
 }
 
+size_t vt_op_conv_in_norm_workspace_bytes(int B, int H, int W) {
+    if (B <= 0 || H <= 0 || W <= 0) return 0;
+    return align_up(2 * 128 * 32 * 2) + align_up((size_t)B * vt_conv_in_mfma_parts(H, W) * 32 * 3 * 4) + align_up((size_t)B * 128 * 2 * 4);
+}
+
+int vt_op_conv_in_norm(vt_context* c, const float* x, const float* w_oihw, const float* bias, const float* gamma, const float* beta, int groups,
+                       float eps, int fused, void* x0_out_f16, void* a1_out_16, int a1_is_f16, int B, int H, int W, void* ws, size_t ws_bytes,
+                       void* stream) {
+    if (!c) return VT_ERR_INVALID;
+    DeviceGuard guard(c);
+    if (!x || !w_oihw || !bias || !gamma || !beta || !x0_out_f16 || !a1_out_16 || !ws) return c->fail(VT_ERR_INVALID, "vt_op_conv_in_norm: null buffer");
+    if (groups != 32) return c->fail(VT_ERR_INVALID, "vt_op_conv_in_norm: the matrix-core conv_in writes partials for 32 groups (got %d)", groups);
+    const size_t need = vt_op_conv_in_norm_workspace_bytes(B, H, W);
+    if (!need || ws_bytes < need) return c->fail(VT_ERR_WORKSPACE, "vt_op_conv_in_norm: workspace %zu < required %zu", ws_bytes, need);
+    if (((uintptr_t)ws) % ALIGN) return c->fail(VT_ERR_INVALID, "vt_op_conv_in_norm: workspace must be 256-B aligned");
+    hipStream_t s = (hipStream_t)stream;
+    std::vector<float> hw(128 * 27), hb(128);
+    HIPCK(c, hipMemcpy(hw.data(), w_oihw, hw.size() * 4, hipMemcpyDeviceToHost), "vt_op_conv_in_norm copy");
+    HIPCK(c, hipMemcpy(hb.data(), bias, 128 * 4, hipMemcpyDeviceToHost), "vt_op_conv_in_norm copy");
+    HIPCK(c, to_device(ws, pack_conv_in_mfma(hw.data(), hb.data())), "vt_op_conv_in_norm copy");
+    const bf16_t* wpk = (const bf16_t*)ws;
+    float* partial = (float*)((char*)ws + align_up(2 * 128 * 32 * 2));
+    float* ss = (float*)((char*)partial + align_up((size_t)B * vt_conv_in_mfma_parts(H, W) * 32 * 3 * 4));
+    f16_t* x0 = (f16_t*)x0_out_f16;
+    int parts = 0;
+    HIPCK(c, vt_launch_conv_in_mfma(x, wpk, bias, nullptr, nullptr, fused ? nullptr : x0, partial, &parts, B, H, W, s), "conv_in_mfma");
+    HIPCK(c, vt_launch_gn_finalize(partial, parts, B, 128, groups, eps, gamma, beta, ss, s), "gn_finalize");
+    if (fused) HIPCK(c, vt_launch_conv_in_mfma(x, wpk, bias, nullptr, (bf16_t*)a1_out_16, x0, nullptr, nullptr, B, H, W, s, ss, a1_is_f16 ? 2 : 1), "conv_in_norm");
+    else HIPCK(c, vt_launch_gn_apply(x0, 2, ss, a1_out_16, B, H * W, 128, 1, s, 0.f, nullptr, a1_is_f16 ? 1 : 0), "gn_apply");
+    return VT_OK;
+}
+
 size_t vt_op_groupnorm_workspace_bytes(int B, int HW, int C) {
     if (B <= 0 || HW <= 0 || C < 8 || (C % 8)) return 0;
     return align_up((size_t)B * vt_gn_max_chunks(HW, C) * 64 * 3 * 4) + align_up((size_t)B * C * 2 * 4);
diff --git a/vae_tagger_amd/csrc/vt_context.h b/vae_tagger_amd/csrc/vt_context.h
--- a/vae_tagger_amd/csrc/vt_context.h
+++ b/vae_tagger_amd/csrc/vt_context.h
@@ -127,6 +127,7 @@
     unsigned rs_ring_next = 0;
     std::map<std::array<int, 4>, std::vector<int>> rs_tables;
     int conv_in_mfma = 1;
+    int conv_in_norm = 1;
     void* op_scratch = nullptr; size_t op_scratch_bytes = 0;
 
     struct ProfRec { hipEvent_t e0, e1; double flops; int cfg; };
@@ -238,7 +239,10 @@
 int run_gn(vt_context* c, const void* x, int xdt, int B, int HW, const NormW& n, int groups, int silu, bf16_t* y, GnState& g, hipStream_t s,
            bool out_fp8 = false, bool out_f16 = false);
 bool conv_f16(const vt_context* c, const ConvW& w, int stride, bool has_sc);
-struct NormConvOpts { const ScFuse* sc = nullptr; bool o16_e4m3 = false, o16_f16 = false, o16_planar = false; };
+struct NormConvOpts {
+    const ScFuse* sc = nullptr; bool o16_e4m3 = false, o16_f16 = false, o16_planar = false;
+    bool act_ready = false;
+};
 int run_norm_conv(vt_context* c, const NormW& n, const ConvW& w, const void* x, int xdt, int B, int H, int W, int groups, bf16_t* act,
                   const void* res, void* oh, bf16_t* o16, GnState& gn, bool want_stats, hipStream_t s, int rdt, const NormConvOpts& nc = NormConvOpts());
 
diff --git a/vae_tagger_amd/csrc/vt_kernels.h b/vae_tagger_amd/csrc/vt_kernels.h
--- a/vae_tagger_amd/csrc/vt_kernels.h
+++ b/vae_tagger_amd/csrc/vt_kernels.h
@@ -276,7 +276,8 @@
                              int B, int H, int W, int Cout, hipStream_t s);
 int vt_conv_in_parts(int H, int W);
 hipError_t vt_launch_conv_in_mfma(const float* x_nchw, const bf16_t* wpk, const float* bias, float* out_f32, bf16_t* out_bf16,
-                                  f16_t* out_f16, float* gn_partial, int* gn_parts, int B, int H, int W, hipStream_t s);
+                                  f16_t* out_f16, float* gn_partial, int* gn_parts, int B, int H, int W, hipStream_t s,
+                                  const float* scale_shift = nullptr, int apply = 0);
 int vt_conv_in_mfma_parts(int H, int W);
 
 hipError_t vt_launch_gn_stats(const void* x, int x_dtype, int B, int HW, int C, int groups,
```

Result: no change. 219.0 (median of 6 runs) (+0.7%).
